# cvxgrp/cvxpygen

Hardware: AMD Instinct MI355X
Metric: QP instances solved/sec (batched MPC QP, OSQP; inputs resident in HBM) (higher is better)
Workload: dtype f64

## Files before the change

cvxpygen_amd/codegen.py:

```python

from __future__ import annotations

import os
import shutil
import subprocess
from typing import List, Optional, Sequence

import numpy as np

from .solve_program import GEN_EXTRA_SLOTS, LANES, RaggedProgram, execution_steps, padded_offsets_fit

CSRC = os.path.join(os.path.dirname(os.path.abspath(__file__)), 'csrc')


class ProgramTooLarge(Exception):
    """the family's solve program cannot be made LDS-resident: no specialised library for it"""


def emit_program_header(rp: RaggedProgram, name: str = 'family', plan=None, depth: int = 2, cross: int = 4,
                        pad_offsets: bool = False, group_offsets: int = 4, batch: int = 1, early: int = 4) -> str:
    out: List[str] = []
    w = out.append
    w(f'// Generated by cvxpygen_amd.codegen for problem family "{name}" -- do not edit.')
    w(f'// solve program: {rp.n_phases} phases, {rp.n_chunks} chunks, {int(rp.ctab[:, 0].sum())} steps, '
# ... 419 lines not shown
            r_of, s_of, nr = list(range(len(idx))), {}, len(idx)
        for k, t in enumerate(idx):
            reg_of[t] = r_of[k]
        for c, sft in s_of.items():
            shift_of[c] = sft
        n_regs_w[v] = nr
    n_regs = max(n_regs_w + [1])
    n_off = max(1, (max([int(sl[t]) + 1 for t in range(T)] + [0]) + 1) // 2)
    n_row = max(1, (max([int(cl[c]) + 1 for c in range(rp.n_chunks)] + [0]) + 1) // 2)
    w(f'// Generated by cvxpygen_amd.codegen for problem family "{name}" -- do not edit.')
    w(f'// team executor ({W} wavefronts per instance): {rp.n_phases} phases, {rp.n_chunks} chunks, {T} steps, {rp.nnz - 1} coefficients;')
    w(f'// steps per wavefront {[int((sw == v).sum()) for v in range(W)]}, coefficient registers {n_regs_w}')
    w('#pragma once')
    w(f'#define {G}_W {W}')
    w(f'#define {G}_NCHUNKS {rp.n_chunks}')
    w(f'#define {G}_NNZ {rp.nnz}')
    w(f'#define {G}_FINGERPRINT {rp.fingerprint()}u')
    w(f'#define {G}_NSTEPS {T}')
    w(f'#define {G}_NSLOTS {rp.n_slots}')
    w(f'#define {G}_NREGS {n_regs}')
    w(f'#define {G}_NOFF {n_off}')
    w(f'#define {G}_NROW {n_row}')
    for k_, v_ in (dims or {}).items():
        w(f'#define {G}_{k_} {int(v_)}')
    w(f'#define {G}_STEPS {{' + ', '.join(f'{{{e}, {cnt}, {reg_of[t]}, {shift_of[c]}}}' for t, (_, c, e, cnt) in enumerate(steps)) + '}')
    w(f'#define {G}_STEP_WAVE {{' + ', '.join(str(int(v)) for v in sw) + '}')
    w(f'#define {G}_STEP_LOCAL {{' + ', '.join(str(int(v)) for v in sl) + '}')
    w(f'#define {G}_CHUNK_SHIFT {{' + ', '.join(str(shift_of[c]) for c in range(rp.n_chunks)) + '}')
    w(f'#define {G}_CHUNK_WAVE {{' + ', '.join(str(int(v)) for v in cw) + '}')
    w(f'#define {G}_CHUNK_LOCAL {{' + ', '.join(str(int(v)) for v in cl) + '}')
    w('namespace cpg {')
    if coef == 'reg':
        w(f'CPG_DEV void {func}(const double (&cf)[{G}_NREGS], const unsigned (&of)[{G}_NOFF], const unsigned (&rw)[{G}_NROW],')
        w('                              CPG_LDS double *w, int wave) {')
    else:
        w(f'CPG_DEV void {func}(const double *vals, const unsigned *off, const unsigned *row, CPG_LDS double *w, int lane, int wave) {{')
    w('    const CPG_LDS char *wb = (const CPG_LDS char *)w;')
    by_phase = {}
    for t, (pi_, c, e, cnt) in enumerate(steps):
        by_phase.setdefault(pi_, []).append((t, c))
    plist = sorted(by_phase)

    def off_expr(t):
        j = int(sl[t])
        base = f'of[{j // 2}]' if coef == 'reg' else f'q{int(sw[t])}_{j // 2}'
        return f'({base} >> 16)' if j & 1 else f'({base} & 0xFFFFu)'

    def row_expr(c):
        j = int(cl[c])
        base = f'rw[{j // 2}]' if coef == 'reg' else f'p{int(cw[c])}_{j // 2}'
        return f'({base} >> 16)' if j & 1 else f'({base} & 0xFFFFu)'
    w('    switch (wave) {')
    for v in range(W):
        w(f'    case {v}: {{')
        mine = [t for t in range(T) if sw[t] == v]
        if coef != 'reg' and mine:
            for k in range((len(mine) + 1) // 2):
                w(f'        const unsigned q{v}_{k} = cpgw::gld(off, {(v * n_off + k) * 64}u + (unsigned)lane);')
            nch_v = len({steps[t][1] for t in mine})
            for k in range((nch_v + 1) // 2):
                w(f'        const unsigned p{v}_{k} = cpgw::gld(row, {(v * n_row + k) * 64}u + (unsigned)lane);')
            for t in mine:
                w(f'        const double c{t} = cpgw::gld(vals, {int(steps[t][2])}u + (unsigned)lane);')
        for pi_ in plist:
            lst = [(t, c) for (t, c) in by_phase[pi_] if sw[t] == v]
            if lst:
                chunks = sorted({c for _, c in lst})
                w(f'        // phase {pi_}')
                for c in chunks:
                    w(f'        const unsigned r{c} = {row_expr(c)};')
                for t, c in lst:
                    w(f'        const double x{t} = *(const CPG_LDS double *)(wb + {off_expr(t)});')
                for c in chunks:
                    if int(rp.ctab[c, 3]) & 2:
                        w(f'        const double o{c} = w[r{c} & CPG_GEN_SLOT_MASK];')
                w('        cpgw::sched_fence();')
                nsteps_c = {}
                for _, c in lst:
                    nsteps_c[c] = nsteps_c.get(c, 0) + 1
                kacc = {c: (1 if (n_ < 6 or not TEAM_SPLIT_SUMS) else (2 if n_ < 12 else 4)) for c, n_ in nsteps_c.items()}
                seen, first = {}, {}
                for t, c in lst:
                    cx = f'cf[{reg_of[t]}]' if coef == 'reg' else f'c{t}'
                    j = seen.get(c, 0) % kacc[c]
                    seen[c] = seen.get(c, 0) + 1
                    nm = f'a{c}' if kacc[c] == 1 else f'a{c}_{j}'
                    if (c, j) not in first:
                        first[(c, j)] = True
                        w(f'        double {nm} = {cx} * x{t};' if coef == 'reg' else f'        double {nm} = fma({cx}, x{t}, 0.0);')
                    else:
                        w(f'        {nm} = fma({cx}, x{t}, {nm});')
                for c in chunks:
                    if kacc[c] == 2:
                        w(f'        const double a{c} = a{c}_0 + a{c}_1;')
                    elif kacc[c] == 4:
                        w(f'        const double a{c} = (a{c}_0 + a{c}_1) + (a{c}_2 + a{c}_3);')
                for c in chunks:
                    lg, kind = int(rp.ctab[c, 1]), int(rp.ctab[c, 3])
                    assert not kind & 4, 'a team executor has no deferred phases (resident_plan: intra phases instead)'
                    red = f'cpgw::seg_sum_first_lit<{lg}>(a{c}, {_mask_literals(stage_masks(rp, c, shift_of[c]))})' if kind & 1 else f'cpgw::group_sum_first<{lg}>(a{c})'
                    acc = f'o{c} + ' if kind & 2 else ''
                    w(f'        w[r{c} & CPG_GEN_SLOT_MASK] = {acc}{red};')
            if sync:
                w('        cpgw::block_sync();')
        w('    } break;')
    w('    default: {')
    if sync:
        for _ in plist:
            w('        cpgw::block_sync();')
    w('    } break;')
    w('    }')
    w('}')
    w('}  // namespace cpg')
    return '\n'.join(out) + '\n' + epilogue


def factor_fingerprint(fac) -> int:
    h = 0x811C9DC5
    ct = np.asarray(fac.ctab, dtype=np.int32).reshape(-1, 4)[:, [0, 1, 3]]
    for arr in (np.ascontiguousarray(ct), np.ascontiguousarray(fac.tlen, dtype=np.uint32)):
        for b in arr.tobytes():
            h = ((h ^ b) * 0x01000193) & 0xFFFFFFFF
    return h


FACTOR_LOOKAHEAD = int(os.environ.get('CPG_FACTOR_LOOKAHEAD', 3))


def emit_factor_program(fac, nnzL: int, N: int, prefix: str = 'GENI', lookahead: Optional[int] = None,
                        preloaded: bool = False, func: str = 'numeric_ldl_gen', zero: Optional[int] = None, body: bool = True,
                        one: Optional[int] = None, inverse_from: Optional[int] = None) -> str:
    G = f'CPG_{prefix}_FAC'
    P = FACTOR_LOOKAHEAD if lookahead is None else lookahead
    ct = np.asarray(fac.ctab, dtype=np.int64).reshape(-1, 4)
    nch = ct.shape[0]
    first = np.concatenate([[0], np.cumsum(ct[:, 0])])
    out = []
    w = out.append
    w(f'#define {G}_NCHUNKS {nch}')
    w(f'#define {G}_NSTEPS {int(first[-1])}')
    w(f'#define {G}_FINGERPRINT {factor_fingerprint(fac)}u')
    w(f'#define {G}_ZERO {nnzL + N if zero is None else int(zero)}')
    if one is not None:
        w(f'#define {G}_ONE {int(one)}')
    inv0 = nch if inverse_from is None else int(inverse_from)
    w(f'#define {G}_CHUNKS {{' + ', '.join(f'{{{int(L)}, {int(last)}, {int(lg)}}}' for L, last, _, lg in ct) + '}')
    if not body:
        return '\n'.join(out) + '\n'
    w(f'#define {G}_GENERATED 1')
    w('namespace cpg {')
    if preloaded:
        w(f'CPG_DEV void {func}(const unsigned long long *tri, const unsigned *dk, double *w, int lane) {{')
    else:
        w(f'CPG_DEV void {func}(const unsigned long long *tri, const unsigned *dk, const double *kct, const double *rinv,')
        w('                             double *w, int lane) {')
    w('    const unsigned ln = (unsigned)cpgw::opaque(lane);     // (table addresses computed here, not hoisted out of the instance loop)')

    def req_dk(c):
        if c < nch:
            w(f'    const unsigned d{c} = cpgw::gld(dk, {c * 64}u + ln);')

    def req_rest(c):
        if c < nch:
            if not preloaded and c < inv0:
                w(f'    const double kc{c} = cpgw::gld(kct, {c * 64}u + ln);')
                w(f'    const double kr{c} = cpgw::gld(rinv, (d{c} >> 16) ? (d{c} >> 16) - 1u : 0u);')
            for s_ in range(int(ct[c, 0])):
                w(f'    const unsigned long long e{int(first[c]) + s_} = cpgw::gld(tri, {(int(first[c]) + s_) * 64}u + ln);')
    for c in range(2 * P):
        req_dk(c)
    for c in range(P):
        req_rest(c)
    for c in range(nch):
        L, last, _, lg = (int(v) for v in ct[c])
        last &= 1
        w(f'    // chunk {c}: {L} step(s), groups of {1 << lg}' + (', level end' if last else ''))
        req_dk(c + 2 * P)
        req_rest(c + P)
        if preloaded and L == 0:
            if last:
                w('    cpgw::lds_order();')
            continue
        w(f'    double a{c} = 0.0;')
        for s_ in range(L):
            e = f'e{int(first[c]) + s_}'
            w(f'    a{c} = fma(w[(unsigned){e} & 0xFFFFu] * w[(unsigned)({e} >> 32)], w[((unsigned){e} >> 16)], a{c});')
        w(f'    a{c} = cpgw::group_sum_first<{lg}>(a{c});')
        w(f'    if ((d{c} & 0xFFFFu) != 0xFFFFu) {{')
        if c >= inv0 and not preloaded:
            w(f'        w[d{c} & 0xFFFFu] = -a{c};')
        elif preloaded:
            w(f'        const double v = w[d{c} & 0xFFFFu] - a{c};')
            w(f'        w[d{c} & 0xFFFFu] = (d{c} >> 16) ? 1.0 / v : v;')
        else:
            w(f'        const double v = (kc{c} - ((d{c} >> 16) ? kr{c} : 0.0)) - a{c};')
            w(f'        w[d{c} & 0xFFFFu] = (d{c} & 0xFFFFu) >= {nnzL}u ? 1.0 / v : v;')
        w('    }')
        if last:
            w('    cpgw::lds_order();')
    w('    cpgw::lds_order();')
    w('}')
    w('}  // namespace cpg')
    return '\n'.join(out) + '\n'


def write_instance_header(rp: RaggedProgram, path: str, name: str = 'family', **opts) -> str:
    text = emit_instance_program(rp, name, **opts)
    if os.path.exists(path) and open(path).read() == text:
        return path
    with open(path, 'w') as f:
        f.write(text)
    return path


def write_program_header(rp: RaggedProgram, path: str, name: str = 'family', plan=None, depth: int = 2, **gen_opts) -> str:
    text = emit_program_header(rp, name, plan, depth, **gen_opts)
    if os.path.exists(path) and open(path).read() == text:
        return path
    with open(path, 'w') as f:
        f.write(text)
    return path


def coefficient_dictionary(rp: RaggedProgram) -> np.ndarray:
    return np.unique(np.ascontiguousarray(rp.vals, dtype=np.float64).view(np.uint64))


def family_library_defs(plan, out_dir: str, name: str = 'family', g_list: Sequence[int] = (1, 2),
                        waves: Optional[dict] = None, extra_flags: Sequence[str] = (), depth: int = 2,
                        compress: Optional[bool] = None, **gen_opts):
    out_dir = os.path.abspath(out_dir)
    os.makedirs(out_dir, exist_ok=True)
    rp = plan.kkt_ragged
    d = plan.desc
    N = d.n_var + d.m
    if 'pad_offsets' not in gen_opts:
        gen_opts = dict(gen_opts, pad_offsets=(compress is not True) and padded_offsets_fit(rp, N))
    pad_offsets = bool(gen_opts['pad_offsets'])
    hdr = write_program_header(rp, os.path.join(out_dir, f'cpg_program_{name}.h'), name, plan=plan, depth=depth, **gen_opts)
    nsx, nsz = -(-d.n_var // 64), -(-d.m // 64)
    nv = max(-(-plan.n_vary_x // 64), -(-plan.n_vary_z // 64), 1)
    nv = nv if nv <= 1 else max(nsx, nsz)
    waves = waves or {1: 8, 2: 4}
    ylist = ' '.join(f'Y({nsx}, {nsz}, {nv}, {g}, {waves[g]})' for g in g_list)
    nnzp = rp.nnz + 64
    n_off = 64 * ((int(rp.ctab[:, 0].sum()) + 3) & ~3) if pad_offsets else nnzp
    plain = 8 * N + 8 * (nnzp + (n_off + 3) // 4 + 16 * ((rp.n_chunks + 3) & ~3))
    n_dict = len(coefficient_dictionary(rp))
    packed = 8 * N + 8 * (n_dict + (nnzp + 1) // 2 + 16 * ((rp.n_chunks + 3) & ~3))
    per_wave = 8 * (rp.n_slots + GEN_EXTRA_SLOTS)
    can_compress = n_dict <= 8192 and per_wave <= 65536 and not pad_offsets
    if compress is None:
        compress = can_compress and (160 * 1024 - plain) // per_wave < 8 and \
            (160 * 1024 - packed) // per_wave > max(0, (160 * 1024 - plain) // per_wave)
    compress = bool(compress and can_compress)
    fixed = packed if compress else plain
    wfit = (160 * 1024 - fixed) // per_wave
    if wfit < 1:
        raise ProgramTooLarge(f'solve program ({fixed} B) + one work vector do not fit the 160 KiB LDS; '
                              'use the table-driven library (program streamed from L2)')
    if 1 in g_list and waves[1] == 8 and wfit >= 10:
        ylist += f' Y({nsx}, {nsz}, {nv}, 1, 12)'
    defs = [f'-DCPG_GEN_HEADER="{hdr}"', '-DCPG_KERNELS(X)=', f'-DCPG_KERNELS_LDS(Y)={ylist}',
            f'-DCPG_KERNELS_REFACTOR(Z)=Z({nsx}, {nsz})']
    if compress:
        defs += ['-DCPG_GEN_COMPRESSED=1', f'-DCPG_GEN_NDICT={n_dict}']
    import scipy.sparse as _sps
    if int(np.diff(_sps.csr_matrix(d.A).indptr).max(initial=0)) > 32:
        defs.append('-DCPG_REFACTOR_ROW_COPY=1')
    if not any('CPG_REFACTOR_WAVES_PER_SIMD' in f for f in extra_flags):
        if nsx + nsz <= 14:
            defs.append('-DCPG_REFACTOR_WAVES_PER_SIMD=4')
        elif nsx + nsz >= 20:
            defs.append('-DCPG_REFACTOR_WAVES_PER_SIMD=2')
            if os.environ.get('CPG_REFACTOR_CR_LDS', '1') != '0':
                defs.append('-DCPG_REFACTOR_CR_LDS=1')
    ih = instance_header(plan, out_dir, name)
    if ih is not None:
        defs.append(f'-DCPG_GENI_HEADER="{ih}"')
    qh = squad_header(plan, out_dir, name)
    if qh is not None:
        defs.append(f'-DCPG_GENQ_HEADER="{qh}"')
    th = team_header(plan, out_dir, name) if team_waves(d) else None
    rh = resident_header(plan, out_dir, name) if th is None else None
    if th is None and rh is None and TEAM_WAVES == -1 and matrix_parameters(d):
        th = team_header(plan, out_dir, name, W=TEAM_AUTO_WAVES)
    if th is not None:
        defs.append(f'-DCPG_GENT_HEADER="{th}"')
    elif rh is not None:
        defs.append(f'-DCPG_GENR_HEADER="{rh}"')
    else:
        sh = stream_header(plan, out_dir, name)
        if sh is not None:
            defs.append(f'-DCPG_GENS_HEADER="{sh}"')
    return hdr, defs


GENS_MAX_STEPS = int(os.environ.get('CPG_GENS_MAX_STEPS', 1200))
GENS_LOOKAHEAD = int(os.environ.get('CPG_GENS_LOOKAHEAD', 16))


def stream_header(plan, out_dir: str, name: str = 'family') -> Optional[str]:
    from . import refactor_plan as _rp
    from .solve_program import execution_steps
    d = plan.desc
    if not matrix_parameters(d) or os.environ.get('CPG_GENS', '0') != '1':
        return None
    rpl = _rp.build_refactor_plan(d.P, d.A, plan.osqp)
    T = len(execution_steps(rpl.sol))
    if T == 0 or T > GENS_MAX_STEPS or any(int(k_) & ~1 for k_ in rpl.sol.ctab[:, 3]):
        return None
    text = emit_instance_program(rpl.sol, name, lookahead=GENS_LOOKAHEAD, prefix='GENS', func='run_program_gens', coef='mem')
    path = os.path.join(os.path.abspath(out_dir), f'cpg_stream_{name}.h')
    if not (os.path.exists(path) and open(path).read() == text):
        with open(path, 'w') as f:
            f.write(text)
    return path


GENI_MAX_REGS = int(os.environ.get('CPG_GENI_MAX_REGS', 64))
GENI_MAX_STEPS = int(os.environ.get('CPG_GENI_MAX_STEPS', 240))
LDS_BYTES = 160 * 1024


SHARED_REG_LDS_REGS = 20


def shared_register_lds_bytes(n: int, m: int, n_steps: int, n_chunks: int, n_slots: int, n_regs: int, waves: int = 8) -> int:
    tab = 2 * (256 * ((n_steps + 3) // 4) + 256 * ((n_chunks + 3) // 4))
    return 8 * (n + m) + tab + 8 * 64 * min(SHARED_REG_LDS_REGS, n_regs) + waves * 8 * (n_slots + GEN_EXTRA_SLOTS)


def instance_program_fits(rpl) -> bool:
    mg = getattr(rpl, 'merged', None)
    rp = mg.sol if mg is not None else rpl.sol
    N = rpl.n + rpl.m
    steps = execution_steps(rp)
    if len(steps) > GENI_MAX_STEPS or rp.n_slots + GEN_EXTRA_SLOTS > 0x1FFF or not np.array_equal(rp.final_pos, np.arange(N)):
        return False
    if pack_step_registers(rp, steps)[2] > GENI_MAX_REGS:
        return False
    tab = 2 * (256 * ((len(steps) + 3) // 4) + 256 * ((rp.n_chunks + 3) // 4))
    per_wave = rp.n_slots + GEN_EXTRA_SLOTS + N + (N & 1)
    fac = rpl.nnzL + N
    if mg is not None:
        fac = mg.fac_len
        if fac >= 0xFFFF:
            return False
    per_wave = max(per_wave, fac + (fac & 1))
    return tab + 8 * 8 * per_wave <= LDS_BYTES


def instance_header(plan, out_dir: str, name: str = 'family') -> Optional[str]:
    from . import refactor_plan as _rp
    d = plan.desc
    o = plan.osqp_shared or plan.osqp
    Ps, As = o.pruned(d.P, d.A)
    rpl = _rp.shared_mode_plan(Ps, As, o)
    if not instance_program_fits(rpl):
        return None
    dims = dict(N=d.n_var, M=d.m, NEQ=d.n_eq)
    mg = rpl.merged
    if mg is None:
        prog, fac = rpl.sol, emit_factor_program(rpl.fac, rpl.nnzL, rpl.n + rpl.m)
    else:
        import types
        dims['NNZX'] = mg.nnzX
        prog = mg.sol
        fac = emit_factor_program(types.SimpleNamespace(ctab=mg.f_ctab, tlen=mg.f_len), rpl.nnzL, rpl.n + rpl.m,
                                  zero=mg.fac_len - 1, one=mg.one_pos, inverse_from=mg.base.fac.n_chunks)
    return write_instance_header(prog, os.path.join(os.path.abspath(out_dir), f'cpg_instance_{name}.h'), name,
                                 row_programs=shared_row_programs(Ps, As), dims=dims, epilogue=fac)


RESIDENT_MAX_REGS = int(os.environ.get('CPG_RESIDENT_MAX_REGS', 160))
RESIDENT_MAX_STEPS = int(os.environ.get('CPG_RESIDENT_MAX_STEPS', 320))
RESIDENT_ACC_BASE = int(os.environ.get('CPG_RESIDENT_ACC_BASE', 32))
RESIDENT_GATHER_BATCH = int(os.environ.get('CPG_RESIDENT_GATHER_BATCH', 12))
RESIDENT_ACC_PAIRS = int(os.environ.get('CPG_RESIDENT_ACC_PAIRS', 112))


def resident_compiler_flags(defs: Sequence[str]) -> List[str]:
    return []


def matrix_parameters(desc) -> bool:
    import scipy.sparse as _sps
    NP = desc.NP
    return any(_sps.csr_matrix(desc.maps[k])[:, :NP].nnz > 0 for k in ('P', 'A'))


def resident_program_fits(rpl, np_var: Optional[int] = None) -> bool:
    rp = rpl.sol
    b = rpl.base
    N = b.n + b.m
    steps = execution_steps(rp)
    if len(steps) > RESIDENT_MAX_STEPS or not np.array_equal(rp.final_pos, np.arange(N)):
        return False
    if pack_step_registers(rp, steps)[2] > RESIDENT_MAX_REGS:
        return False
    tab = 2 * (256 * ((len(steps) + 3) // 4) + 256 * ((rp.n_chunks + 3) // 4))
    np_var = b.nnzP + b.nnzA + N if np_var is None else np_var
    slice_ = max(rpl.fac_len, rpl.w_slots + N, b.nnzA + b.nnzP + max(np_var, N + max(b.n, b.m)))
    slice_ += slice_ & 1
    return 8 * slice_ <= 0xFFFF and tab + 2 * 8 * slice_ <= LDS_BYTES


def resident_four_waves(rpl, np_var: int) -> bool:
    if os.environ.get('CPG_RES_FOUR_WAVES', '0') != '1':
        return False
    b = rpl.base
    N = b.n + b.m
    slice_ = max(rpl.fac_len, rpl.w_slots + b.m, max(b.nnzA + b.nnzP, max(np_var, N + max(b.n, b.m))))
    slice_ += slice_ & 1
    return 4 * 8 * slice_ <= LDS_BYTES


def resident_header(plan, out_dir: str, name: str = 'family') -> Optional[str]:
    from . import resident_plan as _rs
    d = plan.desc
    if not matrix_parameters(d):
        return None
    rpl = _rs.build_resident_plan(d.P, d.A, plan.osqp)
    if not resident_program_fits(rpl, d.NP):
        return None
    b = rpl.base
    dims = dict(N=b.n, M=b.m, NEQ=d.n_eq, NNZA=b.nnzA, NNZP=b.nnzP, NNZL=b.nnzL, NNZX=rpl.nnzX)
    from .solve_program import execution_steps
    rows = ''
    progs = (('GENRA', 'run_rows_a', rpl.rows_A), ('GENRP', 'run_rows_p', rpl.rows_P), ('GENRT', 'run_rows_t', rpl.rows_At))
    if all(len(execution_steps(pr)) > 0 and not any(int(k_) & ~1 for k_ in pr.ctab[:, 3]) for _, _, pr in progs):
        for pre, fn, pr in progs:
            rows += emit_instance_program(pr, name, lookahead=len(execution_steps(pr)) + 4, prefix=pre, func=fn, coef='mem',
                                          lds_typed=True).replace('#pragma once\n', '')
    import types
    if rpl.fac_len < 0xFFFF:
        rows += emit_factor_program(types.SimpleNamespace(ctab=rpl.f_ctab, tlen=rpl.f_len), b.nnzL, b.n + b.m, prefix='GENR',
                                    preloaded=True, func='resident_factor_gen', zero=rpl.fac_len - 1)
    return write_instance_header(rpl.sol, os.path.join(os.path.abspath(out_dir), f'cpg_resident_{name}.h'), name,
                                 prefix='GENR', func='run_program_res', prefetch_next=True, dims=dims,
                                 gather_batch=RESIDENT_GATHER_BATCH, lds_typed=True, epilogue=rows,
                                 tables_global=resident_four_waves(rpl, d.NP))


TEAM_WAVES = int(os.environ.get('CPG_TEAM_WAVES', -1))
TEAM_AUTO_WAVES = 4
TEAM_MAX_GROUP_ROWS = int(os.environ.get('CPG_TEAM_MAX_GROUP_ROWS', 600))
TEAM_SPLIT_SUMS = os.environ.get('CPG_TEAM_SPLIT_SUMS', '0') == '1'
FAC_CODE_BYTES_PER_STEP = 130
INSTRUCTION_CACHE_BYTES = 64 * 1024
TEAM_FAC_GENERATED_MAX = int(os.environ.get('CPG_TEAM_FAC_GENERATED_MAX', (INSTRUCTION_CACHE_BYTES * 5 // 4) // FAC_CODE_BYTES_PER_STEP))


def team_waves(desc=None) -> int:
    return TEAM_WAVES if TEAM_WAVES in (1, 2, 4, 8) else 0


def build_team_plan(desc, osqp, W: Optional[int] = None, max_group_rows: Optional[int] = None, groups=None):
    from . import resident_plan as _rs
    W = team_waves(desc) if W is None else W
    saved = _rs.MAX_GROUP_ROWS
    _rs.MAX_GROUP_ROWS = TEAM_MAX_GROUP_ROWS if max_group_rows is None else int(max_group_rows)
    try:
        return _rs.build_resident_plan(desc.P, desc.A, osqp, team=W, inplace_x=False, groups=groups)
    finally:
        _rs.MAX_GROUP_ROWS = saved


def team_slice_doubles(rpl, np_var: int) -> int:
    b = rpl.base
    N = b.n + b.m
    slice_ = max(rpl.fac_len, rpl.w_slots, b.nnzA + b.nnzP, np_var, N + max(b.n, b.m))
    slice_ += slice_ & 1
    return slice_ + 16 * max(1, int(rpl.team)) + 8


def team_program_fits(rpl, W: int, np_var: Optional[int] = None) -> bool:
    rp = rpl.sol
    b = rpl.base
    N = b.n + b.m
    if rpl.team != W or not np.array_equal(rp.final_pos, np.arange(N)) or rp.n_slots + GEN_EXTRA_SLOTS > 0x1FFF:
        return False
    if any(int(k_) & 4 for k_ in rp.ctab[:, 3]):
# ... 626 lines not shown
```

cvxpygen_amd/csrc/cpg_hip.cpp:

```cpp
#include "../../include/cpg_hip.h"

#include <math.h>
#include <stdio.h>
#include <stdlib.h>
#include <string.h>

#include <algorithm>
#include <string>
#include <type_traits>
#include <vector>

#include "cpg_osqp_kernel.h"
#include "cpg_osqp_refactor.h"
#include "cpg_osqp_resident.h"
#include "cpg_osqp_team.h"
#include "cpg_osqp_squad.h"
#include "cpg_clarabel_kernel.h"

#include <hip/hip_runtime.h>
typedef hipStream_t rt_stream_t;
typedef hipEvent_t rt_event_t;
#define RT_CHECK(expr)                                                                         \
    do {                                                                                       \
        hipError_t e_ = (expr);                                                                \
// ... 281 lines not shown
    const int wave_global = (int)(blockIdx.x * (blockDim.x >> 6) + (threadIdx.x >> 6));
    cpg::osqp_refactor_body<NSX, NSZ, true>(F, R, S, Bt, cpg_lds, wave_global);
}
#ifdef CPG_GENI_NNZX
template <int NSX, int NSZ, int NV>
__global__ void __launch_bounds__(512, 2)
osqp_shared_reg_kernel(cpg::DevFamily F, cpg::DevUpdate U, cpg::DevSettings S, cpg::DevBatch Bt, cpg::DevShRegs RG) {
    extern __shared__ __attribute__((aligned(16))) double cpg_lds[];
    const int wave_global = (int)(blockIdx.x * (blockDim.x >> 6) + (threadIdx.x >> 6));
    cpg::osqp_shared_body<NSX, NSZ, NV, 1, false, cpg::SharedRegExec>(F, U, S, Bt, cpg_lds, wave_global, RG);
}
#endif
#endif
#ifdef CPG_GENR_HEADER
template <int NSX, int NSZ>
__global__ void __launch_bounds__(256)
osqp_resident_kernel(cpg::DevFamily F, cpg::DevRefactor R, cpg::DevResident Rs, cpg::DevSettings S, cpg::DevBatch Bt) {
    extern __shared__ __attribute__((aligned(16))) double cpg_lds[];
    const int wave_global = (int)(blockIdx.x * (blockDim.x >> 6) + (threadIdx.x >> 6));
    cpg::osqp_resident_body<NSX, NSZ>(F, R, Rs, S, Bt, cpg_lds, wave_global);
}
#endif
#ifdef CPG_GENT_HEADER
__global__ void __launch_bounds__(CPG_GENT_W * 64)
osqp_team_kernel(cpg::DevFamily F, cpg::DevRefactor R, cpg::DevResident Rs, cpg::DevSettings S, cpg::DevBatch Bt) {
    extern __shared__ __attribute__((aligned(16))) double cpg_lds[];
    constexpr int NX = (CPG_GENT_N + CPG_GENT_W * 64 - 1) / (CPG_GENT_W * 64), NZ = (CPG_GENT_M + CPG_GENT_W * 64 - 1) / (CPG_GENT_W * 64);
    cpg::osqp_team_body<(NX > 0 ? NX : 1), (NZ > 0 ? NZ : 1)>(F, R, Rs, S, Bt, cpg_lds, (int)blockIdx.x);
}
#endif
#ifdef CPG_GENQ_HEADER
template <int NSX, int NSZ, int NV>
__global__ void __launch_bounds__(CPG_GENQ_W * 64, 2)
osqp_squad_kernel(cpg::DevFamily F, cpg::DevUpdate U, cpg::DevSettings S, cpg::DevBatch Bt) {
    extern __shared__ __attribute__((aligned(16))) double cpg_lds[];
    cpg::osqp_squad_body<NSX, NSZ, NV>(F, U, S, Bt, cpg_lds);
}
#endif
template <int NSX, int NSZ>
__global__ void __launch_bounds__(512, CPG_GRADIENT_WAVES_PER_SIMD)
osqp_gradient_kernel(cpg::DevFamily F, cpg::DevRefactor R, cpg::DevGradient Gd, cpg::DevGradBatch Bt) {
    extern __shared__ __attribute__((aligned(16))) double cpg_lds[];
    const int wave_global = (int)(blockIdx.x * (blockDim.x >> 6) + (threadIdx.x >> 6));
    cpg::osqp_gradient_body<NSX, NSZ>(F, R, Gd, Bt, cpg_lds, wave_global);
}

#ifndef CPG_KERNELS_REFACTOR
#define CPG_KERNELS_REFACTOR(Z) Z(1, 1) Z(4, 4) Z(8, 8) Z(16, 16)
#endif
template <typename Launch>
static bool slot_class(cpg_handle_t h, int &rc, Launch &&launch) {
    const int nsx = (h->F.n + 63) / 64, nsz = (h->F.m + 63) / 64;
#define Z(a, b)                                                                                   \
    if (nsx <= a && nsz <= b) {                                                                   \
        rc = launch(std::integral_constant<int, a>(), std::integral_constant<int, b>());          \
        return true;                                                                              \
    }
    CPG_KERNELS_REFACTOR(Z)
#undef Z
    return false;
}
template <typename Launch>
static int with_slot_class(cpg_handle_t h, Launch &&launch) {
    int rc;
    if (slot_class(h, rc, launch)) return rc;
    set_error("problem family larger than the largest compiled slot class");
    return CPG_E_UNSUPPORTED;
}
static int launch_gradient(cpg_handle_t h, const cpg::DevGradBatch &Bt, int blocks, int waves, size_t lds) {
    return with_slot_class(h, [&](auto NSX, auto NSZ) {
        return launch_kernel(osqp_gradient_kernel<NSX, NSZ>, blocks, waves * 64, lds, h->stream, h->F, h->R, h->Gd, Bt); });
}
static int launch_refactor(cpg_handle_t h, rt_stream_t stream, const cpg::DevSettings &S, const cpg::DevBatch &Bt, int blocks, int waves, size_t lds) {
    return with_slot_class(h, [&](auto NSX, auto NSZ) {
        return launch_kernel(h->R.shared_mats ? osqp_refactor_kernel<NSX, NSZ, true> : osqp_refactor_kernel<NSX, NSZ, false>,
                             blocks, waves * 64, lds, stream, h->F, h->R, S, Bt); });
}

#ifndef CPG_CONIC_WAVES_PER_SIMD
#define CPG_CONIC_WAVES_PER_SIMD 4
#endif
template <bool TABLES_IN_LDS, bool SPECIALISED, bool NONSYM>
__global__ void __launch_bounds__(512, CPG_CONIC_WAVES_PER_SIMD)
clarabel_kernel(cpg::DevConic C, cpg::DevConicSettings S, cpg::DevBatch Bt) {
    extern __shared__ __attribute__((aligned(16))) double cpg_lds[];
    const int wave_global = (int)(blockIdx.x * (blockDim.x >> 6) + (threadIdx.x >> 6));
    cpg::clarabel_body<TABLES_IN_LDS, SPECIALISED, NONSYM>(C, S, Bt, cpg_lds, wave_global);
}
static int launch_conic(cpg_handle_t h, const cpg::DevBatch &Bt, int blocks, int waves, size_t lds, bool tables_in_lds) {
    const bool extended = h->C.n_ns > 0 || h->C.n_psd > 0;
#ifdef CPG_GENC_HEADER
    if (h->conic_specialised && tables_in_lds)
        return launch_kernel(extended ? clarabel_kernel<true, true, true> : clarabel_kernel<true, true, false>,
                             blocks, waves * 64, lds, h->stream, h->C, h->CS, Bt);
#endif
    auto kern = extended ? (tables_in_lds ? clarabel_kernel<true, false, true> : clarabel_kernel<false, false, true>)
                         : (tables_in_lds ? clarabel_kernel<true, false, false> : clarabel_kernel<false, false, false>);
    return launch_kernel(kern, blocks, waves * 64, lds, h->stream, h->C, h->CS, Bt);
}


#ifndef CPG_KERNELS
#define CPG_KERNELS(X)                                                                              \
    X(1, 1, 1, 1) X(1, 1, 1, 2) X(4, 4, 1, 1) X(4, 4, 1, 2) X(4, 4, 4, 1) X(8, 8, 1, 1) X(8, 8, 1, 2)   \
    X(8, 8, 8, 1) X(16, 16, 16, 1)
#endif
#ifndef CPG_KERNELS_LDS
#define CPG_KERNELS_LDS(Y)                                                                          \
    Y(1, 1, 1, 1, 8) Y(1, 1, 1, 1, 16) Y(1, 1, 1, 2, 8) Y(4, 4, 1, 1, 8) Y(4, 4, 1, 1, 16) Y(4, 4, 1, 2, 8)    \
    Y(4, 4, 4, 1, 8) Y(8, 8, 1, 1, 8) Y(8, 8, 1, 1, 12) Y(8, 8, 1, 2, 4) Y(8, 8, 1, 2, 8) Y(8, 8, 8, 1, 8) \
    Y(16, 16, 16, 1, 8)
#endif

static int vary_slots(cpg_handle_t h) {
    const int nvx = (h->n_vary_x + 63) / 64, nvz = (h->n_vary_z + 63) / 64;
    return nvx > nvz ? nvx : nvz;
}
static int launch(cpg_handle_t h, const cpg::DevBatch &Bt, int blocks, int waves, int G, size_t lds, bool in_lds) {
    const int nsx = (h->F.n + 63) / 64, nsz = (h->F.m + 63) / 64, nv = vary_slots(h);
    if (!in_lds) {
#define X(a, b, v, g)                                                                             \
        if (nsx <= a && nsz <= b && (nv <= v || (v >= a && v >= b)) && G == g && waves <= 4)      \
            return launch_kernel(osqp_shared_kernel<a, b, v, g, false, 4>, blocks, waves * 64, lds, h->stream, h->F, h->U, h->S, Bt);
        CPG_KERNELS(X)
#undef X
    } else {
#define Y(a, b, v, g, wm)                                                                         \
        if (nsx <= a && nsz <= b && (nv <= v || (v >= a && v >= b)) && G == g && waves <= wm)     \
            return launch_kernel(osqp_shared_kernel<a, b, v, g, true, wm>, blocks, waves * 64, lds, h->stream, h->F, h->U, h->S, Bt);
        CPG_KERNELS_LDS(Y)
#undef Y
    }
    set_error("no compiled kernel for this family size / launch geometry");
    return CPG_E_UNSUPPORTED;
}

#ifdef CPG_GENQ_HEADER
static int launch_squad(cpg_handle_t h, const cpg::DevBatch &Bt, int blocks, size_t lds) {
    const int nsx = (h->F.n + 63) / 64, nsz = (h->F.m + 63) / 64, nv = vary_slots(h);
#define Y(a, b, v, g, wm)                                                                         \
    if (nsx == a && nsz == b && (nv <= v || (v >= a && v >= b)) && g == 1)                        \
        return launch_kernel(osqp_squad_kernel<a, b, v>, blocks, CPG_GENQ_W * 64, lds, h->stream, h->F, h->U, h->S, Bt);
    CPG_KERNELS_LDS(Y)
#undef Y
    set_error("no compiled squad kernel for this family size");
    return CPG_E_UNSUPPORTED;
}
#endif

#if defined(CPG_GENI_HEADER) && defined(CPG_GENI_NNZX)
static int shared_reg_waves(cpg_handle_t h) { return h->waves_per_block > 0 && h->waves_per_block < 8 ? h->waves_per_block : 8; }
static size_t shared_reg_lds(cpg_handle_t h, int W) {
    const size_t tab = (size_t)(((CPG_GENI_NSTEPS + 3) / 4) * 256 + ((CPG_GENI_NCHUNKS + 3) / 4) * 256) * sizeof(unsigned short);
    return (size_t)(h->F.n + h->F.m) * sizeof(double) + tab + (size_t)cpg::SharedRegExec::nlds * 64 * sizeof(double) +
           (size_t)W * (CPG_GENI_NSLOTS + CPG_GEN_EXTRA_SLOTS) * sizeof(double);
}
static bool shared_reg_usable(cpg_handle_t h) {
    return !h->refactor_mode && !h->conic && h->sreg_ok && h->sreg_rho == h->F.rho && h->sreg_sigma == h->F.sigma &&
           h->inst_per_wave == 1 && shared_reg_lds(h, shared_reg_waves(h)) <= h->lds_limit;
}
static int launch_shared_reg(cpg_handle_t h, const cpg::DevBatch &Bt, int blocks, int waves, size_t lds) {
    const int nsx = (h->F.n + 63) / 64, nsz = (h->F.m + 63) / 64, nv = vary_slots(h);
#define Y(a, b, v, g, wm)                                                                         \
    if (nsx <= a && nsz <= b && (nv <= v || (v >= a && v >= b)) && g == 1)                        \
        return launch_kernel(osqp_shared_reg_kernel<a, b, v>, blocks, waves * 64, lds, h->stream, h->F, h->U, h->S, Bt, h->SRg);
    CPG_KERNELS_LDS(Y)
#undef Y
    set_error("no compiled register-executor kernel for this family size");
    return CPG_E_UNSUPPORTED;
}
#else
static bool shared_reg_usable(cpg_handle_t) { return false; }
#endif

static cpg::DevBatch make_batch(int64_t B, const double *d_theta, const double *d_state_in, double *d_state_out, double *d_prim,
                                double *d_dual, double *d_obj, int32_t *d_iter, int32_t *d_status, double *d_pri, double *d_dua) {
    cpg::DevBatch Bt;
    Bt.scratch = nullptr; Bt.state_in = d_state_in; Bt.state_out = d_state_out;
    Bt.B = B; Bt.theta = d_theta; Bt.prim = d_prim; Bt.dual = d_dual; Bt.obj = d_obj; Bt.pri_res = d_pri;
    Bt.dua_res = d_dua; Bt.iter = d_iter; Bt.status = d_status; Bt.counter = nullptr;
    Bt.ho_list = nullptr; Bt.ho_count = nullptr; Bt.ho_state = nullptr; Bt.list = nullptr; Bt.list_count = nullptr; Bt.resume = 0;
    return Bt;
}

static int launch_per_instance(cpg_handle_t h, rt_stream_t stream, const cpg::DevSettings &S, cpg::DevBatch &Bt) {
    int rc;
    auto scratch = [&](int blocks, int waves, size_t doubles) {
        const int r = ensure(h->scratch, (size_t)blocks * waves * doubles * sizeof(double));
        Bt.scratch = (double *)h->scratch.p;
        return r;
    };
#ifdef CPG_GENT_HEADER
    if (h->Rs.ok == 2 && !h->R.shared_mats && h->program_in_lds != 0 && h->program_in_lds != 2) {
        const size_t lds = ((size_t)CPG_TEAM_SLICE_OFF + (size_t)h->Rs.slice_doubles) * sizeof(double);
        if (lds <= h->lds_limit) {
            long long per_cu = (long long)(h->lds_limit / lds);
            if (per_cu * CPG_GENT_W > 16) per_cu = 16 / CPG_GENT_W;
            if (CPG_GENT_W <= 4 && per_cu * CPG_GENT_W > 4) per_cu = 4 / CPG_GENT_W;
            if (h->blocks_per_cu > 0 && per_cu > h->blocks_per_cu) per_cu = h->blocks_per_cu;
            const int blocks = std::max(1, grid_blocks(h, Bt.B, 1, per_cu));
            if ((rc = scratch(blocks, 1, h->Rs.buf_doubles))) return rc;
            return launch_kernel(osqp_team_kernel, blocks, CPG_GENT_W * 64, lds, stream, h->F, h->R, h->Rs, S, Bt);
        }
    }
#endif
#ifdef CPG_GENR_HEADER
    if (h->Rs.ok && !h->R.shared_mats && h->program_in_lds != 0 && h->program_in_lds != 2) {
#ifdef CPG_GENR_TABLES_GLOBAL
        const size_t tab = 0;
#else
        const size_t tab = (size_t)(((CPG_GENR_NSTEPS + 3) / 4) * 256 + ((CPG_GENR_NCHUNKS + 3) / 4) * 256) * sizeof(unsigned short);
#endif
        const size_t slice = (size_t)h->Rs.slice_doubles * sizeof(double);
        int NW = h->waves_per_block > 0 ? h->waves_per_block : 4;
        if (NW > 4) NW = 4;
        while (NW > 1 && tab + (size_t)NW * slice > h->lds_limit) NW--;
        const size_t lds = tab + (size_t)NW * slice;
        if (lds <= h->lds_limit) {
            const int blocks = grid_blocks(h, Bt.B, NW, 1);
            if ((rc = scratch(blocks, NW, h->Rs.buf_doubles))) return rc;
            if (slot_class(h, rc, [&](auto NSX, auto NSZ) {
                    return launch_kernel(osqp_resident_kernel<NSX, NSZ>, blocks, NW * 64, lds, stream, h->F, h->R, h->Rs, S, Bt); }))
                return rc;
        }
    }
#endif
#ifdef CPG_GENI_HEADER
    if (h->R.gi_ok && h->program_in_lds != 0 && h->program_in_lds != 2) {
        const int W = 8;
        const size_t tab = (size_t)(((CPG_GENI_NSTEPS + 3) / 4) * 256 + ((CPG_GENI_NCHUNKS + 3) / 4) * 256) * sizeof(unsigned short);
        const size_t nq = (size_t)(h->F.n + h->F.m);
        size_t per_wave = (size_t)(CPG_GENI_NSLOTS + CPG_GEN_EXTRA_SLOTS) + nq + (nq & 1);
#ifdef CPG_GENI_FAC_NSTEPS
        const size_t fac = (size_t)CPG_GENI_FAC_ZERO + 1;
#else
        const size_t fac = (size_t)h->R.nnzL + nq;
#endif
        if (per_wave < fac) per_wave = fac + (fac & 1);
        const size_t lds = tab + (size_t)W * per_wave * sizeof(double);
        if (lds <= h->lds_limit) {
            const int blocks = grid_blocks(h, Bt.B, W, 1);
            if ((rc = scratch(blocks, W, h->R.buf_doubles))) return rc;
            if (slot_class(h, rc, [&](auto NSX, auto NSZ) {
                    return launch_kernel(osqp_instance_kernel<NSX, NSZ>, blocks, W * 64, lds, stream, h->F, h->R, S, Bt); }))
                return rc;
        }
    }
#endif
#ifdef CPG_REFACTOR_CR_LDS
    if (!h->R.shared_mats && h->program_in_lds != 0) {
        const int W8 = 8;
        const size_t tab = (((size_t)h->R.sol_nnz + 1) / 2) * sizeof(double);
        const size_t lds8 = tab + (size_t)W8 * h->R.sol_slots * sizeof(double);
        if (lds8 <= h->lds_limit) {
            const int blocks = grid_blocks(h, Bt.B, W8, 1);
            if ((rc = scratch(blocks, W8, h->R.buf_doubles))) return rc;
            if (slot_class(h, rc, [&](auto NSX, auto NSZ) {
                    return launch_kernel(osqp_refactor_crlds_kernel<NSX, NSZ>, blocks, W8 * 64, lds8, stream, h->F, h->R, S, Bt); }))
                return rc;
        }
    }
#endif
    const int W = 4;
#ifdef CPG_GENS_HEADER
    if (!h->R.shared_mats && !h->R.gs_ok) {
        set_error("this library's per-instance substitution program was generated for a different family"); return CPG_E_BADARG; }
    const size_t lds = (size_t)W * (size_t)(h->R.shared_mats ? h->R.sol_slots : h->R.sol_slots + CPG_GEN_EXTRA_SLOTS) * sizeof(double);
#else
    const size_t lds = (size_t)W * h->R.sol_slots * sizeof(double);
#endif
    if (lds > h->lds_limit) { set_error("work vectors do not fit the LDS"); return CPG_E_UNSUPPORTED; }
    int per_cu = h->blocks_per_cu > 0 ? h->blocks_per_cu : CPG_REFACTOR_WAVES_PER_SIMD;
    if (per_cu > CPG_REFACTOR_WAVES_PER_SIMD) per_cu = CPG_REFACTOR_WAVES_PER_SIMD;
    if ((long long)per_cu * (long long)lds > (long long)h->lds_limit) per_cu = (int)(h->lds_limit / lds);
    const int blocks = grid_blocks(h, Bt.B, W, per_cu);
    if ((rc = scratch(blocks, W, h->R.buf_doubles))) return rc;
    return launch_refactor(h, stream, S, Bt, blocks, W, lds);
}

static int begin_solve(cpg_handle_t h) {
    RT_CHECK(hipMemsetAsync(h->d_counter, 0, 4 * sizeof(unsigned), h->stream));
    RT_CHECK(hipEventRecord(h->ev0, h->stream));
    return CPG_OK;
}
static int end_solve(cpg_handle_t h) {
    RT_CHECK(hipEventRecord(h->ev1, h->stream));
    return CPG_OK;
}

static int solve_conic(cpg_handle_t h, const cpg::DevBatch &Bt) {
    const size_t per_wave = (size_t)h->C.lds_doubles * sizeof(double);
    int W = h->waves_per_block > 0 ? (h->waves_per_block > 8 ? 8 : h->waves_per_block) : 8;
    const size_t tab = (size_t)h->C.tab_doubles * sizeof(double);
    const bool tables_in_lds = h->program_in_lds != 0 && tab + per_wave <= h->lds_limit;
    const size_t fixed = tables_in_lds ? tab : 0;
    while (W > 1 && fixed + (size_t)W * per_wave > h->lds_limit) W--;
    if (h->waves_per_block <= 0) {
        int best = W, best_res = 0;
        for (int w2 = W; w2 >= 4; w2--) {
            int pc = (int)(h->lds_limit / (fixed + (size_t)w2 * per_wave));
            if (h->blocks_per_cu > 0 && pc > h->blocks_per_cu) pc = h->blocks_per_cu;
            int res = pc * w2; if (res > 4 * CPG_CONIC_WAVES_PER_SIMD) res = 4 * CPG_CONIC_WAVES_PER_SIMD;
            if (res > best_res) { best_res = res; best = w2; }
        }
        W = best;
    }
    const size_t lds = fixed + (size_t)W * per_wave + (fixed + (size_t)W * per_wave + 128 <= h->lds_limit ? 128 : 0);
// ... 709 lines not shown
    UP(int, prim_idx, f->n_prim); UP(int, dual_idx, f->n_dual);
#undef UP
    TRY(upload_csr(h, own, f->map_P, &C.map_P)); TRY(upload_csr(h, own, f->map_A, &C.map_A));
    TRY(upload_csr(h, own, f->map_q, &C.map_q)); TRY(upload_csr(h, own, f->map_b, &C.map_b));
    TRY(upload_csr(h, own, f->map_d, &C.map_d));
    C.gc_ok = 0; C.sv_pad = 0; C.w_extra = 0; C.gc_ncols = 0; C.gc_nrows = 0; C.gc_cols = nullptr; C.gc_rows = nullptr;
    C.gf_ok = 0;
#ifdef CPG_GENC_FACTOR_HEADER
    C.gf_ok = (conic_factor_words_hash(f) == CPG_GENC_FAC_HASH && !(getenv("CPG_CONIC_FACTOR") && atoi(getenv("CPG_CONIC_FACTOR")) == 0)) ? 1 : 0;
#endif
#ifdef CPG_GENC_HEADER
    if (f->sol_chunks == CPG_GENC_NCHUNKS && f->sol_nnz == CPG_GENC_NNZ && f->sol_slots == CPG_GENC_NSLOTS &&
        program_fingerprint(f->sol_ctab, f->sol_desc, f->sol_cols, f->sol_chunks, f->sol_nnz) == CPG_GENC_FINGERPRINT &&
        !(getenv("CPG_CONIC_GENERATED") && atoi(getenv("CPG_CONIC_GENERATED")) == 0)) {
        static const int steps[][4] = CPG_GENC_STEPS;
        std::vector<unsigned short> gcols, grows;
        if (generated_tables(f->sol_ctab, f->sol_desc, f->sol_cols, f->sol_chunks, f->sol_nnz, f->sol_slots, steps, CPG_GENC_NSTEPS, gcols, grows)) {
            TRY(upload<unsigned short>(h, own, gcols.data(), gcols.size(), &C.gc_cols));
            TRY(upload<unsigned short>(h, own, grows.data(), grows.size(), &C.gc_rows));
            C.gc_ncols = (int)gcols.size(); C.gc_nrows = (int)grows.size();
            C.gc_ok = 1; C.sv_pad = 64; C.w_extra = CPG_GEN_EXTRA_SLOTS;
            cpg::DevConic Cs = C;
            Cs.n_pfull = f->Prp[n]; Cs.fac_triples = f->fac_triples;
            cpg::DevConic Ck = Cs;
            { cpg::DevConic &Cref = Ck; CPG_GENC_SPECIALISE(Cref) }
            h->conic_specialised = conic_dims_equal(Cs, Ck) && !(getenv("CPG_CONIC_SPECIALISED") && atoi(getenv("CPG_CONIC_SPECIALISED")) == 0);
#ifdef CPG_GENC_ROWS
            if (h->conic_specialised && conic_row_words_hash(f) != CPG_GENC_ROWS_HASH) h->conic_specialised = false;
#endif
        }
    }
#endif
    {
        C.fac_triples = f->fac_triples; C.n_pfull = f->Prp[n];
        auto dbl = [](size_t count, size_t elem) { return (count * elem + 7) / 8; };
        size_t t = 0;
        t += 2 * dbl((size_t)f->n_soc, 4) + dbl((size_t)m, 4);
        bool row_words = false;
#ifdef CPG_GENC_ROWS
        row_words = h->conic_specialised;
        if (row_words) t += dbl((size_t)CPG_GENC_ROWS_WORDS, sizeof(cpg::genc_row_word));
#endif
        if (!row_words) {
            t += dbl((size_t)n + 1, 4) + dbl((size_t)f->nnzA, 4) + dbl((size_t)m + 1, 4) + 2 * dbl((size_t)f->nnzA, 4);
            t += dbl((size_t)n + 1, 4) + dbl((size_t)f->nnzP, 4) + dbl((size_t)n + 1, 4) + 2 * dbl((size_t)C.n_pfull, 4);
        }
        t += dbl((size_t)f->nnzL, 4) + 2 * dbl((size_t)f->nnzL + N, 4);
        t += dbl((size_t)f->fac_chunks * 4, 4) + 2 * dbl((size_t)f->fac_chunks * 64, 4) + 3 * dbl((size_t)f->fac_triples, 4);
#ifdef CPG_GENC_HEADER
        t += dbl((size_t)C.gc_ncols, 2) + dbl((size_t)C.gc_nrows, 2);
#else
        t += dbl((size_t)f->sol_chunks * 4, 4) + dbl((size_t)f->sol_chunks * 64, 4) + dbl((size_t)f->sol_nnz, 2);
#endif
        t += 2 * dbl((size_t)f->sol_nnz, 4) + dbl((size_t)N, 2);
        C.tab_doubles = (int)t;
    }
    {
        const long long d = (long long)f->nnzP + f->nnzA + 7LL * n + 14LL * m + 6LL * N + f->nnzL + f->sol_nnz + C.sv_pad + f->sol_slots + C.w_extra + C.psd_doubles;
        C.lds_doubles = (int)((d + 1) & ~1LL);
        if ((size_t)C.lds_doubles * 8 > h->lds_limit) {
            set_error("conic family too large: the interior-point state of one instance does not fit the LDS");
            cpg_hip_destroy(h); return CPG_E_UNSUPPORTED; }
    }
    { void *p = nullptr; TRY(rt_malloc(&p, 64)); h->d_counter = (unsigned *)p; }
    TRY(rt_sync(h));
#undef TRY
    h->have_update = true;
    cpg_hip_set_default_settings(h);
    *out = h;
    return CPG_OK;
}

struct cpg_pipe_s;
static void free_pipe(cpg_pipe_s *p);
static void free_list(std::vector<void *> &v) { for (void *p : v) rt_free(p); v.clear(); }

int cpg_hip_destroy(cpg_handle_t h) {
    if (!h) return CPG_OK;
    rt_set_device(h->device);
    rt_sync(h);
    free_list(h->owned); free_list(h->update_owned); free_list(h->refactor_owned); free_list(h->sreg_owned); free_list(h->resident_owned); free_list(h->gradient_owned);
    free_buf(h->g_theta); free_buf(h->g_x); free_buf(h->g_y); free_buf(h->g_dprim); free_buf(h->g_dtheta);
    if (h->d_counter) rt_free(h->d_counter);
    free_buf(h->scratch);
    free_buf(h->s_theta); h->s_out.free(); free_buf(h->s_state_in); free_buf(h->s_state_out);
    free_buf(h->ho_state); free_buf(h->ho_list);
    free_pipe(h->pipe); h->pipe = nullptr;
    if (h->have_events) { hipEventDestroy(h->ev0); hipEventDestroy(h->ev1); hipEventDestroy(h->ev_mid); }
    if (h->stream) hipStreamDestroy(h->stream);
    delete h;
    return CPG_OK;
}

int cpg_hip_set_update(cpg_handle_t h, const cpg_osqp_update_t *u) {
    if (!h || !u) { set_error("null argument"); return CPG_E_BADARG; }
    if (h && h->conic) { set_error("not available for a conic (interior-point) handle"); return CPG_E_BADARG; }
    if (u->map_q.nnz && u->map_q.rows != h->F.n) { set_error("map_q rows != n"); return CPG_E_BADARG; }
    if (u->map_u.nnz && u->map_u.rows != h->F.m) { set_error("map_u rows != m"); return CPG_E_BADARG; }
    {
        const cpg_csr_t *mp[2] = {&u->map_q, &u->map_u};
        const int lim[2] = {h->n_vary_x, h->n_vary_z};
        for (int k = 0; k < 2; k++)
            if (mp[k]->nnz > 0 && mp[k]->ptr[mp[k]->rows] != mp[k]->ptr[lim[k] < mp[k]->rows ? lim[k] : mp[k]->rows]) {
                set_error("update map touches entries outside the parameter-dependent prefix"); return CPG_E_BADARG; }
    }
    int rc = rt_set_device(h->device);
    if (rc) return rc;
    if ((rc = rt_sync(h))) return rc;
    free_list(h->update_owned);
    cpg::DevUpdate &U = h->U;
    U.np_var = u->np_var; U.d_base = u->d_base;
    if ((rc = upload<double>(h, h->update_owned, u->q_base, h->F.n, &U.q_base))) return rc;
    if ((rc = upload<double>(h, h->update_owned, u->u_base, h->F.m, &U.u_base))) return rc;
    if ((rc = upload_csr(h, h->update_owned, u->map_q, &U.map_q))) return rc;
    if ((rc = upload_csr(h, h->update_owned, u->map_u, &U.map_u))) return rc;
    if ((rc = upload_csr(h, h->update_owned, u->map_d, &U.map_d))) return rc;
    if ((rc = rt_sync(h))) return rc;
    h->have_update = true;
    h->refactor_mode = false;
    return CPG_OK;
}

static bool kkt_constants(cpg_handle_t h, const cpg_osqp_refactor_t *r, std::vector<double> &fkc, std::vector<int> &fkrow) {
    const size_t m = h->F.m, nd = (size_t)r->nnzL + h->F.n + m;
    fkc.assign(nd, 0.0); fkrow.assign(nd, -1);
    for (size_t d = 0; d < nd; d++) {
        const int kind = r->ksrc_kind[d], idx = r->ksrc_idx[d];
        const bool piv = d >= (size_t)r->nnzL;
        if (kind == CPG_K_P) { if (idx < 0 || idx >= r->nnzP) return false; fkc[d] = r->Ps[idx] + (piv ? h->F.sigma : 0.0); }
        else if (kind == CPG_K_A) { if (idx < 0 || idx >= r->nnzA) return false; fkc[d] = r->As[idx]; }
        else if (kind == CPG_K_SIGMA) fkc[d] = h->F.sigma;
        else if (kind == CPG_K_RHO) { if (idx < 0 || (size_t)idx >= m) return false; fkrow[d] = idx; }
        else if (kind != CPG_K_NONE) return false;
    }
    return true;
}

#ifdef CPG_GENI_HEADER
struct InstanceTables {
    int nnzX;
    int sol_chunks, sol_nnz, sol_slots;
    const int32_t *sol_ctab; const uint32_t *sol_desc; const uint16_t *sol_cols; const int32_t *sol_kind, *sol_idx;
    int fac_chunks, fac_triples;
    const int32_t *fac_ctab; const uint32_t *fac_task, *fac_len, *fac_a, *fac_b, *fac_k;
};

static int set_instance_executor(cpg_handle_t h, const cpg_osqp_refactor_t *r, const InstanceTables &g,
                                 const std::vector<double> &fkc, const std::vector<int> &fkrow) {
    std::vector<void *> &own = h->refactor_owned;
    cpg::DevRefactor &R = h->R;
    const size_t n = h->F.n, m = h->F.m, N = n + m;
    int rc = CPG_OK;
    R.gi_ok = 0;
    std::vector<unsigned short> gcols, grows, glcol;
    std::vector<unsigned> gsrc, gdk;
    std::vector<unsigned long long> gtri;
    std::vector<double> gkc;
#ifdef CPG_GENI_N
    const bool geni_dims = h->F.n == CPG_GENI_N && h->F.m == CPG_GENI_M && h->F.n_eq == CPG_GENI_NEQ;
#else
    const bool geni_dims = true;
#endif
#ifdef CPG_GENI_NNZX
    const bool merged_lib = true;
#else
    const bool merged_lib = false;
#endif
    if (!(geni_dims && (g.nnzX > 0) == merged_lib && g.sol_chunks == CPG_GENI_NCHUNKS && g.sol_nnz == CPG_GENI_NNZ && g.sol_slots == CPG_GENI_NSLOTS))
        return CPG_OK;
    const size_t nd = (size_t)r->nnzL + N, nx = (size_t)g.nnzX;
    const unsigned hsh = program_fingerprint(g.sol_ctab, g.sol_desc, g.sol_cols, g.sol_chunks, g.sol_nnz);
    static const int steps[][4] = CPG_GENI_STEPS;
    static const int chunk_shift[] = CPG_GENI_CHUNK_SHIFT;
    bool ok = hsh == CPG_GENI_FINGERPRINT;
    {
        const int nn[3] = {CPG_GENI_AROWS_N, CPG_GENI_PROWS_N, CPG_GENI_ATROWS_N};
        for (int k = 0; ok && k < 3; k++) {
            if ((int)h->rows_hdr[k].size() != 4 * nn[k]) ok = false;
            for (int c2 = 0; ok && c2 < nn[k]; c2++)
                if (h->rows_hdr[k][4 * c2] != cpg::GeniRows::len(k, c2) || h->rows_hdr[k][4 * c2 + 3] != cpg::GeniRows::off(k, c2)) ok = false;
        }
    }
    if (ok) ok = generated_tables(g.sol_ctab, g.sol_desc, g.sol_cols, g.sol_chunks, g.sol_nnz, g.sol_slots, steps, CPG_GENI_NSTEPS, gcols, grows, chunk_shift);
    if (ok) {
        gsrc.assign((size_t)CPG_GENI_NREGS * 64, 0u);
        glcol.assign((size_t)CPG_GENI_NREGS * 64, (unsigned short)0);
        std::vector<char> taken((size_t)CPG_GENI_NREGS * 64, 0);
        for (int t = 0; ok && t < CPG_GENI_NSTEPS; t++) {
            const int e = steps[t][0], cnt = steps[t][1], reg = steps[t][2], sh = steps[t][3];
            if (reg < 0 || reg >= CPG_GENI_NREGS) { ok = false; break; }
            for (int l = 0; l < cnt; l++) {
                int kind = g.sol_kind[e + l], idx = g.sol_idx[e + l];
                if (kind == 4) {
                    if (idx < 0 || (size_t)idx >= nx) { ok = false; break; }
                    kind = 3; idx += (int)N;
                }
                if (kind < 0 || kind > 3 || idx < 0 || idx >= (1 << 28)) { ok = false; break; }
                const size_t at = (size_t)reg * 64 + (size_t)(l + sh);
                if (taken[at]) { ok = false; break; }
                taken[at] = 1;
                gsrc[at] = ((unsigned)kind << 28) | (unsigned)idx;
                if (kind == 2) {
                    if (idx >= r->nnzL || r->Lcol[idx] < 0 || r->Lcol[idx] > 0xFFFF) { ok = false; break; }
                    glcol[at] = (unsigned short)r->Lcol[idx];
                }
            }
        }
    }
#ifdef CPG_GENI_FAC_NSTEPS
    if (ok) {
        static const int fch[][3] = CPG_GENI_FAC_CHUNKS;
        const size_t fac_end = nx ? nd + nx + 2 : nd + 1;
        const size_t one = nd + nx;
        unsigned hsh2 = 0x811C9DC5u;
        auto mix = [&](unsigned v) { for (int k = 0; k < 4; k++) { hsh2 = (hsh2 ^ ((v >> (8 * k)) & 0xFFu)) * 0x01000193u; } };
        ok = g.fac_chunks == CPG_GENI_FAC_NCHUNKS && fac_end - 1 == (size_t)CPG_GENI_FAC_ZERO && fac_end <= 0xFFFFu;
#ifdef CPG_GENI_FAC_ONE
        ok = ok && one == (size_t)CPG_GENI_FAC_ONE;
#endif
        for (int c = 0; ok && c < g.fac_chunks; c++) { mix((unsigned)g.fac_ctab[4 * c]); mix((unsigned)g.fac_ctab[4 * c + 1]); mix((unsigned)g.fac_ctab[4 * c + 3]); }
        for (size_t e = 0; ok && e < (size_t)g.fac_chunks * 64; e++) mix(g.fac_len[e]);
        ok = ok && hsh2 == CPG_GENI_FAC_FINGERPRINT;
        if (ok) {
            const unsigned long long Z = (unsigned long long)(fac_end - 1);
            gtri.assign((size_t)CPG_GENI_FAC_NSTEPS * 64, Z | (Z << 16) | (Z << 32));
            gdk.assign((size_t)g.fac_chunks * 64, 0xFFFFu);
            gkc.assign((size_t)g.fac_chunks * 64, 0.0);
            size_t step = 0;
            for (int c = 0; ok && c < g.fac_chunks; c++) {
                const int L = g.fac_ctab[4 * c];
                size_t base = (size_t)g.fac_ctab[4 * c + 2];
                if (L != fch[c][0]) { ok = false; break; }
                for (int s = 0; ok && s < L; s++, step++) {
                    int cnt = 0;
                    for (int l = 0; l < 64; l++) {
                        const unsigned ln = g.fac_len[(size_t)c * 64 + l];
                        if ((int)(ln & 0xFFFFu) <= s) continue;
                        const size_t e = base + (size_t)l;
                        if (l != cnt || e >= (size_t)g.fac_triples) { ok = false; break; }
                        cnt++;
                        if ((int)(ln >> 16) > s) {
                            const unsigned a = g.fac_a[e], b = g.fac_b[e], k = nx ? g.fac_k[e] : (unsigned)r->nnzL + g.fac_k[e];
                            if (a >= (unsigned)r->nnzL || !(b < (unsigned)r->nnzL || (nx && b >= nd && b <= one)) ||
                                k < (unsigned)r->nnzL || k >= nd) { ok = false; break; }
                            gtri[step * 64 + (size_t)l] = (unsigned long long)a | ((unsigned long long)b << 16) | ((unsigned long long)k << 32);
                        }
                    }
                    base += (size_t)cnt;
                }
                for (int l = 0; ok && l < 64; l++) {
                    const unsigned t0 = g.fac_task[(size_t)c * 64 + l];
                    if (t0 == 0xFFFFFFFFu) continue;
                    const unsigned t = nx ? (t0 & 0x7FFFFFFFu) : t0;
                    if (t >= nd + nx) { ok = false; break; }
                    const int kr = t < nd ? fkrow[t] : -1;
                    gdk[(size_t)c * 64 + l] = t | ((unsigned)(kr + 1) << 16);
                    gkc[(size_t)c * 64 + l] = t < nd ? fkc[t] : 0.0;
                }
            }
            if (ok && step != (size_t)CPG_GENI_FAC_NSTEPS) ok = false;
        }
        if (ok) {
            if ((rc = upload<unsigned long long>(h, own, gtri.data(), gtri.size(), &R.gf_tri))) return rc;
            if ((rc = upload<unsigned>(h, own, gdk.data(), gdk.size(), &R.gf_dk))) return rc;
            if ((rc = upload<double>(h, own, gkc.data(), gkc.size(), &R.gf_kc))) return rc;
        }
    }
#else
    ok = ok && !nx;
#endif
    if (ok) {
        if ((rc = upload<unsigned short>(h, own, glcol.data(), glcol.size(), &R.gi_lcol))) return rc;
        if ((rc = upload<unsigned short>(h, own, gcols.data(), gcols.size(), &R.gi_cols))) return rc;
        if ((rc = upload<unsigned short>(h, own, grows.data(), grows.size(), &R.gi_rows))) return rc;
        if ((rc = upload<unsigned>(h, own, gsrc.data(), gsrc.size(), &R.gi_src))) return rc;
    }
    if ((rc = rt_sync(h))) return rc;
    R.gi_ok = ok ? 1 : 0;
    return CPG_OK;
}
#endif

int cpg_hip_set_refactor(cpg_handle_t h, const cpg_osqp_refactor_t *r) {
    if (h && h->conic) { set_error("not available for a conic (interior-point) handle"); return CPG_E_BADARG; }
    if (!h || !r) { set_error("null argument"); return CPG_E_BADARG; }
    int rc = rt_set_device(h->device);
    if (rc) return rc;
    if ((rc = rt_sync(h))) return rc;
    free_list(h->refactor_owned);
    free_list(h->resident_owned); h->Rs = cpg::DevResident{};
    std::vector<void *> &own = h->refactor_owned;
    cpg::DevRefactor &R = h->R;
    const size_t n = h->F.n, m = h->F.m, N = n + m;
    R.nnzP = r->nnzP; R.nnzA = r->nnzA; R.nnzL = r->nnzL; R.n_eq = h->F.n_eq; R.np_var = r->np_var;
    R.scaling_iters = r->scaling_iters; R.d_base = r->d_base;
    R.fac_chunks = r->fac_chunks; R.sol_nnz = r->sol_nnz; R.sol_slots = r->sol_slots;
#define UP(T, field, count) if ((rc = upload<T>(h, own, (const T *)r->field, (size_t)(count), (const T **)&R.field))) return rc
    UP(int, Ap, n + 1); UP(int, Ai, r->nnzA); UP(int, Arp, m + 1); UP(int, Aent, r->nnzA); UP(int, Acol, r->nnzA);
    UP(int, Pp, n + 1); UP(int, Pi, r->nnzP); UP(int, Prp, n + 1);
    { const int npf = r->Prp[n]; UP(int, Pent, npf); UP(int, Pcol, npf); }
    UP(int, Lcol, r->nnzL); UP(int, ksrc_kind, r->nnzL + N); UP(int, ksrc_idx, r->nnzL + N);
    UP(int, fac_ctab, (size_t)r->fac_chunks * 4); UP(unsigned, fac_task, (size_t)r->fac_chunks * 64);
    UP(unsigned, fac_len, (size_t)r->fac_chunks * 64);
    UP(unsigned, fac_a, r->fac_triples); UP(unsigned, fac_b, r->fac_triples); UP(unsigned, fac_k, r->fac_triples);
    StreamTables stt;
    std::vector<int> kind2, idx2;
    R.gs_cols = nullptr; R.gs_rows = nullptr; R.gs_kind = nullptr; R.gs_idx = nullptr; R.gs_ok = 0; R.gs_nnz = 0;
#ifdef CPG_GENS_HEADER
    std::vector<unsigned short> gscols, gsrows;
    std::vector<int> gskind, gsidx;
    if (!r->shared_mats && r->sol_chunks == CPG_GENS_NCHUNKS && r->sol_nnz == CPG_GENS_NNZ && r->sol_slots == CPG_GENS_NSLOTS &&
        program_fingerprint(r->sol_ctab, r->sol_desc, r->sol_cols, r->sol_chunks, r->sol_nnz) == CPG_GENS_FINGERPRINT) {
        static const int gsteps[][4] = CPG_GENS_STEPS;
        if (generated_tables(r->sol_ctab, r->sol_desc, r->sol_cols, r->sol_chunks, r->sol_nnz, r->sol_slots, gsteps, CPG_GENS_NSTEPS, gscols, gsrows)) {
            gskind.assign((size_t)r->sol_nnz + 64, 0); gsidx.assign((size_t)r->sol_nnz + 64, 0);
            for (int e = 0; e < r->sol_nnz; e++) { gskind[e] = r->sol_kind[e]; gsidx[e] = r->sol_idx[e]; }
            R.gs_nnz = r->sol_nnz + 64;
            if ((rc = upload<unsigned short>(h, own, gscols.data(), gscols.size(), &R.gs_cols))) return rc;
            if ((rc = upload<unsigned short>(h, own, gsrows.data(), gsrows.size(), &R.gs_rows))) return rc;
            if ((rc = upload<int>(h, own, gskind.data(), gskind.size(), &R.gs_kind))) return rc;
            if ((rc = upload<int>(h, own, gsidx.data(), gsidx.size(), &R.gs_idx))) return rc;
            R.gs_ok = 1;
        }
    }
#endif
    {
        if ((rc = build_stream_tables(r->sol_ctab, r->sol_desc, r->sol_cols, r->sol_chunks, r->sol_slots, stt))) return rc;
        kind2.resize(stt.src.size()); idx2.resize(stt.src.size());
        for (size_t e = 0; e < stt.src.size(); e++) {
            kind2[e] = stt.src[e] >= 0 ? r->sol_kind[stt.src[e]] : 0;
            idx2[e] = stt.src[e] >= 0 ? r->sol_idx[stt.src[e]] : 0;
        }
        R.sol_pairs = stt.n_pairs;
        R.sol_nnz = (int)stt.cr.size();
        if ((rc = upload<unsigned>(h, own, stt.st.data(), stt.st.size(), &R.sol_stab))) return rc;
        if ((rc = upload<unsigned>(h, own, stt.cr.data(), stt.cr.size(), &R.sol_cr))) return rc;
        if ((rc = upload<int>(h, own, kind2.data(), kind2.size(), &R.sol_kind))) return rc;
        if ((rc = upload<int>(h, own, idx2.data(), idx2.size(), &R.sol_idx))) return rc;
    }
    UP(unsigned short, sol_fpos, N);
    UP(double, P_base, r->nnzP); UP(double, A_base, r->nnzA); UP(double, q_base, n); UP(double, u_base, m);
    UP(double, q_setup, n);
#undef UP
    if ((rc = upload_csr(h, own, r->map_P, &R.map_P))) return rc;
    if ((rc = upload_csr(h, own, r->map_A, &R.map_A))) return rc;
    if ((rc = upload_csr(h, own, r->map_q, &R.map_q))) return rc;
    if ((rc = upload_csr(h, own, r->map_u, &R.map_u))) return rc;
    if ((rc = upload_csr(h, own, r->map_d, &R.map_d))) return rc;
    R.buf_doubles = (long long)(r->nnzP + 2 * r->nnzA + 3 * n + 4 * m + r->nnzL + 2 * N + std::max(R.sol_nnz, R.gs_nnz) + 64);
    R.shared_mats = r->shared_mats ? 1 : 0; R.cs = 1.0;
    R.Ps = R.As = R.Ars = R.Ds = R.Dinvs = R.Es = R.Einvs = nullptr;
    std::vector<double> ars, dinv, einv;
    if (r->shared_mats) {
        if (!r->Ps || !r->As || !r->D || !r->E || !(r->c > 0.0)) { set_error("shared-matrix mode needs Ps, As, D, E, c"); return CPG_E_BADARG; }
        ars.resize((size_t)r->nnzA); dinv.resize(n); einv.resize(m);
        for (int k = 0; k < r->nnzA; k++) ars[k] = r->As[r->Aent[k]];
        for (size_t i = 0; i < n; i++) dinv[i] = 1.0 / r->D[i];
        for (size_t i = 0; i < m; i++) einv[i] = 1.0 / r->E[i];
        R.cs = r->c;
        if ((rc = upload<double>(h, own, r->Ps, (size_t)r->nnzP, &R.Ps))) return rc;
        if ((rc = upload<double>(h, own, r->As, (size_t)r->nnzA, &R.As))) return rc;
        if ((rc = upload<double>(h, own, ars.data(), ars.size(), &R.Ars))) return rc;
        if ((rc = upload<double>(h, own, r->D, n, &R.Ds))) return rc;
        if ((rc = upload<double>(h, own, dinv.data(), n, &R.Dinvs))) return rc;
        if ((rc = upload<double>(h, own, r->E, m, &R.Es))) return rc;
        if ((rc = upload<double>(h, own, einv.data(), m, &R.Einvs))) return rc;
    }
    R.gf_tri = nullptr; R.gf_dk = nullptr; R.gf_kc = nullptr;
    R.gi_ok = 0; R.gi_cols = R.gi_rows = nullptr; R.gi_src = nullptr; R.gi_lcol = nullptr; R.fac_kc = nullptr; R.fac_krow = nullptr; R.fac_kc_cl = nullptr; R.fac_krow_cl = nullptr; R.fac_kind_cl = nullptr; R.fac_idx_cl = nullptr;
    std::vector<double> fkc, fkc_cl;
    std::vector<int> fkrow, fkrow_cl;

    if (r->shared_mats) {
        if (!kkt_constants(h, r, fkc, fkrow)) { set_error("cpg_hip_set_refactor: KKT source table out of range"); return CPG_E_BADARG; }
        const size_t nd = (size_t)r->nnzL + N;
        fkc_cl.assign((size_t)r->fac_chunks * 64, 0.0); fkrow_cl.assign((size_t)r->fac_chunks * 64, -1);
        for (size_t e = 0; e < fkc_cl.size(); e++) {
            const unsigned t = r->fac_task[e];
            if (t == 0xFFFFFFFFu) continue;
            if (t >= nd) { set_error("cpg_hip_set_refactor: factorisation task out of range"); return CPG_E_BADARG; }
            fkc_cl[e] = fkc[t]; fkrow_cl[e] = fkrow[t];
        }
        if ((rc = upload<double>(h, own, fkc.data(), fkc.size(), &R.fac_kc))) return rc;
        if ((rc = upload<int>(h, own, fkrow.data(), fkrow.size(), &R.fac_krow))) return rc;
        if ((rc = upload<double>(h, own, fkc_cl.data(), fkc_cl.size(), &R.fac_kc_cl))) return rc;
        if ((rc = upload<int>(h, own, fkrow_cl.data(), fkrow_cl.size(), &R.fac_krow_cl))) return rc;
    }
#ifdef CPG_GENI_HEADER
    if (r->shared_mats) {
        const InstanceTables g{0, r->sol_chunks, r->sol_nnz, r->sol_slots, r->sol_ctab, r->sol_desc, r->sol_cols, r->sol_kind, r->sol_idx,
                               r->fac_chunks, r->fac_triples, r->fac_ctab, r->fac_task, r->fac_len, r->fac_a, r->fac_b, r->fac_k};
        if ((rc = set_instance_executor(h, r, g, fkc, fkrow))) return rc;
    }
#endif
    if ((rc = rt_sync(h))) return rc;
    h->refactor_mode = true;
    h->have_update = true;
    return CPG_OK;
}

int cpg_hip_set_refactor_merged(cpg_handle_t h, const cpg_osqp_refactor_t *r, const cpg_osqp_resident_t *mg) {
    if (h && h->conic) { set_error("not available for a conic (interior-point) handle"); return CPG_E_BADARG; }
    if (!h || !r || !mg) { set_error("null argument"); return CPG_E_BADARG; }
    if (!r->shared_mats || mg->nnzX <= 0) { set_error("cpg_hip_set_refactor_merged: needs shared-matrix tables and a merged program"); return CPG_E_BADARG; }
    int rc = cpg_hip_set_refactor(h, r);
    if (rc) return rc;
#ifdef CPG_GENI_NNZX
    if (mg->nnzX == CPG_GENI_NNZX) {
        std::vector<double> fkc;
        std::vector<int> fkrow;
        if (!kkt_constants(h, r, fkc, fkrow)) { set_error("cpg_hip_set_refactor_merged: KKT source table out of range"); return CPG_E_BADARG; }
        const InstanceTables g{mg->nnzX, mg->sol_chunks, mg->sol_nnz, mg->sol_slots, mg->sol_ctab, mg->sol_desc, mg->sol_cols, mg->sol_kind,
                               mg->sol_idx, mg->fac_chunks, mg->fac_triples, mg->f_ctab, mg->f_task, mg->f_len, mg->f_a, mg->f_b, mg->f_k};
        if ((rc = set_instance_executor(h, r, g, fkc, fkrow))) return rc;
    }
#endif
    return CPG_OK;
}

int cpg_hip_set_shared_registers(cpg_handle_t h, const cpg_osqp_resident_t *mg, const double *coef, int32_t n_coef, double rho, double sigma) {
    if (h && h->conic) { set_error("not available for a conic (interior-point) handle"); return CPG_E_BADARG; }
    if (!h || !mg || !coef) { set_error("null argument"); return CPG_E_BADARG; }
    if (h->refactor_mode) { set_error("cpg_hip_set_shared_registers: needs a shared-factor handle"); return CPG_E_BADARG; }
    h->sreg_ok = false;
    h->SRg = cpg::DevShRegs{};
    int rc = rt_sync(h);
    if (rc) return rc;
    free_list(h->sreg_owned);
#if defined(CPG_GENI_HEADER) && defined(CPG_GENI_NNZX)
#ifdef CPG_GENI_N
    const bool geni_dims = h->F.n == CPG_GENI_N && h->F.m == CPG_GENI_M && h->F.n_eq == CPG_GENI_NEQ;
#else
    const bool geni_dims = true;
#endif
    if (!(geni_dims && mg->nnzX == CPG_GENI_NNZX && mg->sol_chunks == CPG_GENI_NCHUNKS && mg->sol_nnz == CPG_GENI_NNZ &&
          mg->sol_slots == CPG_GENI_NSLOTS && n_coef == mg->sol_nnz))
        return CPG_OK;
    if (program_fingerprint(mg->sol_ctab, mg->sol_desc, mg->sol_cols, mg->sol_chunks, mg->sol_nnz) != CPG_GENI_FINGERPRINT) return CPG_OK;
    static const int steps[][4] = CPG_GENI_STEPS;
    static const int chunk_shift[] = CPG_GENI_CHUNK_SHIFT;
    std::vector<unsigned short> gcols, grows;
    if (!generated_tables(mg->sol_ctab, mg->sol_desc, mg->sol_cols, mg->sol_chunks, mg->sol_nnz, mg->sol_slots, steps, CPG_GENI_NSTEPS,
                          gcols, grows, chunk_shift))
        return CPG_OK;
    std::vector<double> cf((size_t)CPG_GENI_NREGS * 64, 0.0);
    std::vector<char> taken(cf.size(), 0);
    for (int t = 0; t < CPG_GENI_NSTEPS; t++) {
        const int e = steps[t][0], cnt = steps[t][1], reg = steps[t][2], sh = steps[t][3];
        if (reg < 0 || reg >= CPG_GENI_NREGS) return CPG_OK;
        for (int l = 0; l < cnt; l++) {
            const size_t at = (size_t)reg * 64 + (size_t)(l + sh);
            if (taken[at]) return CPG_OK;
            taken[at] = 1;
            cf[at] = coef[e + l];
        }
    }
    cpg::DevShRegs T{};
    if ((rc = upload<double>(h, h->sreg_owned, cf.data(), cf.size(), &T.cf))) return rc;
    if ((rc = upload<unsigned short>(h, h->sreg_owned, gcols.data(), gcols.size(), &T.cols))) return rc;
    if ((rc = upload<unsigned short>(h, h->sreg_owned, grows.data(), grows.size(), &T.rows))) return rc;
    if ((rc = rt_sync(h))) return rc;
    h->SRg = T;
    h->sreg_ok = true;
    h->sreg_rho = rho; h->sreg_sigma = sigma;
#else
    (void)n_coef; (void)rho; (void)sigma;
#endif
    return CPG_OK;
}

#if defined(CPG_GENT_HEADER)
#define CPG_RX(x) CPG_GENT_##x
#define CPG_RX_PRESENT 1
#define CPG_RX_FAC 1
#elif defined(CPG_GENR_HEADER)
#define CPG_RX(x) CPG_GENR_##x
#define CPG_RX_PRESENT 1
#ifdef CPG_GENR_FAC_NSTEPS
#define CPG_RX_FAC 1
#endif
#endif
#ifdef CPG_GENT_HEADER
static bool team_tables(const std::vector<unsigned short> &gcols, const std::vector<unsigned short> &grows, int T, int n_chunks,
                        const int *step_wave, const int *step_local, const int *chunk_wave, const int *chunk_local, int W, int n_off, int n_row,
                        int n_slots, std::vector<unsigned> &toff, std::vector<unsigned> &trow) {
    const unsigned zero_off = (unsigned)(n_slots + CPG_GEN_DUMMY_SLOTS) * 8u, dummy = (unsigned)n_slots;
    toff.assign((size_t)W * n_off * 64, zero_off | (zero_off << 16));
    trow.assign((size_t)W * n_row * 64, dummy | (dummy << 16));
    for (int t = 0; t < T; t++) {
        const int wv = step_wave[t], j = step_local[t];
        if (wv < 0 || wv >= W || j < 0 || j / 2 >= n_off) return false;
        for (int l = 0; l < 64; l++) {
            unsigned &wd = toff[((size_t)wv * n_off + (size_t)(j / 2)) * 64 + l];
            const unsigned v = gcols[((size_t)(t / 4) * 64 + l) * 4 + (t % 4)];
            wd = (j & 1) ? ((wd & 0xFFFFu) | (v << 16)) : ((wd & 0xFFFF0000u) | v);
        }
    }
    for (int c = 0; c < n_chunks; c++) {
        const int wv = chunk_wave[c], j = chunk_local[c];
        if (wv < 0 || wv >= W || j < 0 || j / 2 >= n_row) return false;
        for (int l = 0; l < 64; l++) {
            unsigned &wd = trow[((size_t)wv * n_row + (size_t)(j / 2)) * 64 + l];
            const unsigned v = grows[((size_t)(c >> 2) * 64 + l) * 4 + (c & 3)];
            wd = (j & 1) ? ((wd & 0xFFFFu) | (v << 16)) : ((wd & 0xFFFF0000u) | v);
        }
    }
    return true;
}
#endif
int cpg_hip_set_resident(cpg_handle_t h, const cpg_osqp_refactor_t *r, const cpg_osqp_resident_t *rs) {
    int rc = cpg_hip_set_refactor(h, r);
    if (rc) return rc;
    free_list(h->resident_owned);
    h->Rs = cpg::DevResident{};
    if (!rs) { set_error("null argument"); return CPG_E_BADARG; }
#ifdef CPG_RX_PRESENT
    if (r->shared_mats) return CPG_OK;
    std::vector<void *> &own = h->resident_owned;
    cpg::DevResident &Rs = h->Rs;
    const int n = h->F.n, m = h->F.m, N = n + m, nnzL = r->nnzL;
    if (n != CPG_RX(N) || m != CPG_RX(M) || h->F.n_eq != CPG_RX(NEQ) || r->nnzA != CPG_RX(NNZA) || r->nnzP != CPG_RX(NNZP) ||
        nnzL != CPG_RX(NNZL) || rs->nnzX != CPG_RX(NNZX) ||
// ... 703 lines not shown
```

cvxpygen_amd/csrc/cpg_osqp_kernel.h:

```cpp
#pragma once

#include <type_traits>
#include "cpg_wave.h"

namespace cpg {

#define CPG_INFTY 1e30
#define CPG_MIN_SCALING 1e-4
#define CPG_DIV_TOL 1e-30
#define CPG_RHO_MIN 1e-6
#define CPG_RHO_MAX 1e6
#define CPG_NO_ROW 0xFFFF
#ifndef CPG_ILP
#define CPG_ILP 2
#endif
#define CPG_FENCE_EVERY(s) do { if (((s) + 1) % CPG_ILP == 0) cpgw::sched_fence(); } while (0)
#ifndef CPG_LDS_UNROLL
#define CPG_LDS_UNROLL 4
#endif
#ifndef CPG_CHUNK_UNROLL
#define CPG_CHUNK_UNROLL 4
#endif

struct DevProgram {
// ... 261 lines not shown
    }
}

#define CPG_GEN_SLOT_MASK 0x1FFFu
#define CPG_GEN_DUMMY_SLOTS 16
#define CPG_GEN_EXTRA_SLOTS (CPG_GEN_DUMMY_SLOTS + 1)
#ifdef CPG_GEN_HEADER
#define CPG_GEN_ZERO(A) _Pragma("unroll") for (int g_ = 0; g_ < G; g_++) A[g_] = 0.0
#define CPG_GEN_PAD 64
#ifdef CPG_GEN_COMPRESSED
#define CPG_GEN_VB(vals, lane) ((const char *)(vals))
#define CPG_GEN_CB(cols, lane) ((const char *)(cols) + (unsigned)(lane) * 4u)
#define CPG_GEN_LOAD_CV(ID, E) const unsigned wd##ID = *(const unsigned *)(cb + (E) * 4u);
#define CPG_GEN_LOAD_W(ID)                                                                         \
    const double vl##ID = *(const double *)(vb + (wd##ID >> 16));                                  \
    double x##ID[G];                                                                               \
    _Pragma("unroll") for (int g_ = 0; g_ < G; g_++) x##ID[g_] = *(const double *)(wb + (unsigned)g_ * ldwb + (wd##ID & 0xFFFFu));
#else
#define CPG_GEN_VB(vals, lane) ((const char *)(vals) + (unsigned)(lane) * 8u)
#define CPG_GEN_CB(cols, lane) ((const char *)(cols) + (unsigned)(lane) * 2u)
#define CPG_GEN_LOAD_CV(ID, E)                                                                     \
    const double vl##ID = *(const double *)(vb + (E) * 8u);                                        \
    const unsigned co##ID = *(const unsigned short *)(cb + (E) * 2u);
#define CPG_GEN_LOAD_CVP(ID, E, K)                                                                 \
    const double vl##ID = *(const double *)(vb + (E) * 8u);                                        \
    const unsigned co##ID = *(const unsigned short *)(cb + (K) * 128u);
#define CPG_GEN_LOAD_CVP2A(ID, E, K)                                                               \
    const double vl##ID = *(const double *)(vb + (E) * 8u);                                        \
    const unsigned cp##ID = *(const unsigned *)(cb + (unsigned)lane * 2u + ((K) >> 1) * 256u);     \
    const unsigned co##ID = cp##ID & 0xFFFFu;
#define CPG_GEN_LOAD_CVP2B(ID, E, PREV)                                                            \
    const double vl##ID = *(const double *)(vb + (E) * 8u);                                        \
    const unsigned co##ID = cp##PREV >> 16;
#define CPG_GEN_LOAD_CVP4A(ID, E, K)                                                               \
    const double vl##ID = *(const double *)(vb + (E) * 8u);                                        \
    const OffsetQuad cq##ID = *(const OffsetQuad *)(cb + (unsigned)lane * 6u + ((K) >> 2) * 512u);          \
    const unsigned co##ID = cq##ID.a & 0xFFFFu;
#define CPG_GEN_LOAD_CVP4B(ID, E, FIRST, J)                                                        \
    const double vl##ID = *(const double *)(vb + (E) * 8u);                                        \
    const unsigned co##ID = (J) == 1 ? cq##FIRST.a >> 16 : (J) == 2 ? (cq##FIRST.b & 0xFFFFu) : cq##FIRST.b >> 16;
#define CPG_GEN_LOAD_W(ID)                                                                         \
    double x##ID[G];                                                                               \
    _Pragma("unroll") for (int g_ = 0; g_ < G; g_++) x##ID[g_] = *(const double *)(wb + (unsigned)g_ * ldwb + co##ID);
#endif
#define CPG_GEN_FMA_FULL(A, ID)                                                                    \
    _Pragma("unroll") for (int g_ = 0; g_ < G; g_++) A[g_] = fma(vl##ID, x##ID[g_], A[g_]);
#define CPG_GEN_FMA_PART(A, ID, CNT)                                                               \
    {                                                                                              \
        const double v_ = lane < (CNT) ? vl##ID : 0.0;                                             \
        _Pragma("unroll") for (int g_ = 0; g_ < G; g_++) A[g_] = fma(v_, x##ID[g_], A[g_]);        \
    }
#define CPG_GEN_LOAD_ROWS(Q) const OffsetQuad rq##Q = *(const OffsetQuad *)((const char *)rows + (unsigned)lane * 8u + (Q) * 512u);
#define CPG_GEN_ROW(Q, J) ((J) == 0 ? (rq##Q.a & 0xFFFFu) : (J) == 1 ? (rq##Q.a >> 16) : (J) == 2 ? (rq##Q.b & 0xFFFFu) : (rq##Q.b >> 16))
#define CPG_GEN_REDUCE_STORE(A, LG, Q, J)                                                          \
    {                                                                                              \
        const unsigned row_ = CPG_GEN_ROW(Q, J) & CPG_GEN_SLOT_MASK;                               \
        _Pragma("unroll") for (int g_ = 0; g_ < G; g_++)                                           \
            w[(unsigned)(g_ * ldw) + row_] = cpgw::group_sum_first<LG>(A[g_]);                     \
    }
#define CPG_GEN_SEGREDUCE_STORE_LIT(A, S, Q, J, M0, M1, M2)                                       \
    {                                                                                              \
        const unsigned row_ = CPG_GEN_ROW(Q, J) & CPG_GEN_SLOT_MASK;                               \
        _Pragma("unroll") for (int g_ = 0; g_ < G; g_++)                                           \
            w[(unsigned)(g_ * ldw) + row_] = cpgw::seg_sum_first_lit<S>(A[g_], M0, M1, M2);        \
    }
#define CPG_GEN_SEGREDUCE_STORE(A, S, Q, J)                                                        \
    {                                                                                              \
        const unsigned e_ = CPG_GEN_ROW(Q, J);                                                     \
        _Pragma("unroll") for (int g_ = 0; g_ < G; g_++)                                           \
            w[(unsigned)(g_ * ldw) + (e_ & CPG_GEN_SLOT_MASK)] = cpgw::seg_sum_first<S>(A[g_], e_ >> 13); \
    }
}
#include CPG_GEN_HEADER
namespace cpg {
#ifndef CPG_GEN_N
#error "generated program headers must carry the family dimensions (codegen.write_program_header(plan=...))"
#endif
#ifdef CPG_GEN_N
struct GenFam {
    static constexpr unsigned n = CPG_GEN_N, m = CPG_GEN_M;
    static constexpr int n_slots = CPG_GEN_NSLOTS;
    static constexpr int ct(int s) { constexpr signed char t[] = CPG_GEN_CT_INIT; return t[s]; }
    static constexpr int rows_len(int which, int s) {
        constexpr int a[][2] = CPG_GEN_AROWS; constexpr int p[][2] = CPG_GEN_PROWS; constexpr int t[][2] = CPG_GEN_ATROWS;
        return which == 0 ? (s < CPG_GEN_AROWS_N ? a[s < CPG_GEN_AROWS_N ? s : 0][0] : 0)
             : which == 1 ? (s < CPG_GEN_PROWS_N ? p[s < CPG_GEN_PROWS_N ? s : 0][0] : 0)
                          : (s < CPG_GEN_ATROWS_N ? t[s < CPG_GEN_ATROWS_N ? s : 0][0] : 0);
    }
    static constexpr int rows_off(int which, int s) {
        constexpr int a[][2] = CPG_GEN_AROWS; constexpr int p[][2] = CPG_GEN_PROWS; constexpr int t[][2] = CPG_GEN_ATROWS;
        return which == 0 ? a[s < CPG_GEN_AROWS_N ? s : 0][1] : which == 1 ? p[s < CPG_GEN_PROWS_N ? s : 0][1]
                                                                            : t[s < CPG_GEN_ATROWS_N ? s : 0][1];
    }
};
#endif
#endif

CPG_DEV double natural_chunk(const DevProgram &P, int s, const double *w, int lane) {
    double o[1];
    o[0] = 0.0;
    if (s < P.n_chunks) do_chunk<1, false>(P, s, w, 0, lane, o);
    return o[0];
}

#ifndef CPG_ROWS_BATCH
#define CPG_ROWS_BATCH 8
#endif
CPG_DEV double natural_chunk_lit(const DevProgram &P, const int len, const int off, const double *w, int lane_in) {
    const int lane = cpgw::opaque(lane_in);
    const unsigned e0 = (unsigned)off * 64u + (unsigned)lane;
    double acc = 0.0;
#pragma unroll
    for (int t0 = 0; t0 < len; t0 += CPG_ROWS_BATCH) {
        double v[CPG_ROWS_BATCH];
        unsigned c[CPG_ROWS_BATCH];
#pragma unroll
        for (int t = 0; t < CPG_ROWS_BATCH; t++)
            if (t0 + t < len) { v[t] = cpgw::gld(P.vals, e0 + 64u * (unsigned)(t0 + t)); c[t] = cpgw::gld(P.cols, e0 + 64u * (unsigned)(t0 + t)); }
#pragma unroll
        for (int t = 0; t < CPG_ROWS_BATCH; t++)
            if (t0 + t < len) acc = fma(v[t], w[c[t]], acc);
    }
    return acc;
}
#ifdef CPG_GEN_N
#define CPG_NATURAL_ROWS(P, which, s, w, lane) natural_chunk_lit(P, GenFam::rows_len(which, s), GenFam::rows_off(which, s), w, lane)
#else
#define CPG_NATURAL_ROWS(P, which, s, w, lane) natural_chunk(P, s, w, lane)
#endif

template <int NSX, int NSZ, int NV>
struct Inst {
    static const int NVX = MinI<NV, NSX>::v, NVZ = MinI<NV, NSZ>::v;
    double x[NSX], z[NSZ], y[NSZ];
    double qv[NVX], uv[NVZ];
    double dconst;
    long long b;
    int done;
};

struct CheckOut {
    double prim_res, dual_res, obj;
    int status;
};

CPG_DEV double csr_row(const DevCsr &mp, unsigned row, const double *theta, double v) {
    if (mp.nnz > 0) {
        const unsigned s = (unsigned)cpgw::gld(mp.ptr, row), e = (unsigned)cpgw::gld(mp.ptr, row + 1u);
        for (unsigned k = s; k < e; k++) v = fma(cpgw::gld(mp.val, k), cpgw::gld(theta, (unsigned)cpgw::gld(mp.idx, k)), v);
    }
    return v;
}

template <int NSX, int NSZ, int NV>
struct SharedCtx {
    static constexpr bool kTestsFirst = true;
    static constexpr bool kOpaqueLane = true;
    const DevFamily &F;
    const double *sh, *shu;
    const Inst<NSX, NSZ, NV> &I;
    const double *w;
    int lane;
    CPG_DEV double q(int s, unsigned i) const {
        return s < Inst<NSX, NSZ, NV>::NVX ? I.qv[s < Inst<NSX, NSZ, NV>::NVX ? s : 0] : sh[i];
    }
    CPG_DEV double u(int s, unsigned i) const {
        return s < Inst<NSX, NSZ, NV>::NVZ ? I.uv[s < Inst<NSX, NSZ, NV>::NVZ ? s : 0] : shu[i];
    }
    CPG_DEV void products(int) const {}
    CPG_DEV void stage(int) const {}
    CPG_DEV double sE(unsigned i) const { return cpgw::gld(F.E, i); }
    CPG_DEV double sEinv(unsigned i) const { return cpgw::gld(F.Einv, i); }
    CPG_DEV double sD(unsigned i) const { return cpgw::gld(F.D, i); }
    CPG_DEV double sDinv(unsigned i) const { return cpgw::gld(F.Dinv, i); }
    CPG_DEV double ax(int s) const { return CPG_NATURAL_ROWS(F.A_rows, 0, s, w, lane); }
    CPG_DEV double px(int s) const { return CPG_NATURAL_ROWS(F.P_rows, 1, s, w, lane); }
    CPG_DEV double atx(int s) const { return CPG_NATURAL_ROWS(F.At_rows, 2, s, w, lane); }
};

template <int NSX, int NSZ, int NV>
CPG_DEV bool canonicalise(const DevFamily &F, const DevUpdate &U, const double *theta,
                          Inst<NSX, NSZ, NV> &I, int lane) {
    bool bad = false;
#pragma unroll
    for (int s = 0; s < NSX; s++) I.x[s] = 0.0;
#pragma unroll
    for (int s = 0; s < NSZ; s++) { I.z[s] = 0.0; I.y[s] = 0.0; }
#pragma unroll
    for (int s = 0; s < Inst<NSX, NSZ, NV>::NVX; s++) {
        const unsigned i = (unsigned)lane + 64u * (unsigned)s;
        I.qv[s] = (i < (unsigned)F.n) ? csr_row(U.map_q, i, theta, cpgw::gld(U.q_base, i)) : 0.0;
    }
#pragma unroll
    for (int s = 0; s < Inst<NSX, NSZ, NV>::NVZ; s++) {
        const unsigned i = (unsigned)lane + 64u * (unsigned)s;
        I.uv[s] = 0.0;
        if (i < (unsigned)F.m) {
            const double uv = csr_row(U.map_u, i, theta, cpgw::gld(U.u_base, i));
            I.uv[s] = uv;
            const int ctp = (int)cpgw::gld(F.ctype, i);
            bad |= (ctp == 0 && uv > CPG_INFTY * CPG_MIN_SCALING) || (ctp == -1 && !(uv > CPG_INFTY * CPG_MIN_SCALING));
        }
    }
    I.dconst = csr_row(U.map_d, 0, theta, U.d_base);
    return cpgw::wave_any(bad);
}

template <int NS>
struct RegDelta {
    const double (&a)[NS];
    CPG_DEV double operator()(int s, unsigned) const { return a[s]; }
};
struct MemDelta {
    const double *p;
    CPG_DEV double operator()(int, unsigned i) const { return cpgw::gld(p, i); }
};
struct NoDelta {
    CPG_DEV double operator()(int, unsigned) const { return 0.0; }
};

template <int NSX, int NSZ, typename Ctx, typename DY>
CPG_DEV bool primal_infeasible(const DevFamily &F, const Ctx &cx, const signed char (&ct)[NSZ],
                               bool unsc, double eps, double *w, const DY &dy, int lane) {
    cx.stage(1);
    double nrm = 0.0, lhs = 0.0;
    double dyp[NSZ];
#pragma unroll
    for (int s = 0; s < NSZ; s++) {
        const unsigned i = (unsigned)lane + 64u * (unsigned)s;
        dyp[s] = 0.0;
        if (i < (unsigned)F.m) {
            const double uu = cx.u(s, i);
            const bool eq = ct[s] == 1;
            const double ll = eq ? uu : -CPG_INFTY;
            const bool iu = uu > CPG_INFTY * CPG_MIN_SCALING, il = !eq;
            double d = dy(s, i);
            if (iu && il) d = 0.0; else if (iu) d = cpgw::dmin2(d, 0.0); else if (il) d = cpgw::dmax2(d, 0.0);
            dyp[s] = d;
            nrm = cpgw::dmax2(nrm, fabs(unsc ? cx.sE(i) * d : d));
            lhs += uu * cpgw::dmax2(d, 0.0) + ll * cpgw::dmin2(d, 0.0);
        }
        cpgw::sched_fence();
    }
    nrm = cpgw::wave_max_nonneg(nrm);
    if (!(nrm > CPG_DIV_TOL)) return false;
    lhs = cpgw::wave_sum(lhs);
    if (!(lhs < eps * nrm)) return false;
#pragma unroll
    for (int s = 0; s < NSZ; s++) { const unsigned i = (unsigned)lane + 64u * (unsigned)s; if (i < (unsigned)F.m) w[(unsigned)F.n + i] = dyp[s]; }
    cpgw::lds_order();
    cx.products(4);
    double r = 0.0;
#pragma unroll
    for (int s = 0; s < NSX; s++) {
        const unsigned i = (unsigned)lane + 64u * (unsigned)s;
        const double t = cx.atx(s);
        if (i < (unsigned)F.n) r = cpgw::dmax2(r, fabs(unsc ? cx.sDinv(i) * t : t));
        cpgw::sched_fence();
    }
    r = cpgw::wave_max_nonneg(r);
    cpgw::lds_order();
    return r < eps * nrm;
}

template <int NSX, int NSZ, typename Ctx, typename DX>
CPG_DEV bool dual_infeasible(const DevFamily &F, const Ctx &cx, const signed char (&ct)[NSZ],
                             bool unsc, double eps, double *w, const DX &dx, int lane) {
    cx.stage(2);
    double nrm = 0.0, qdx = 0.0;
#pragma unroll
    for (int s = 0; s < NSX; s++) {
        const unsigned i = (unsigned)lane + 64u * (unsigned)s;
        if (i < (unsigned)F.n) {
            const double d = dx(s, i);
            nrm = cpgw::dmax2(nrm, fabs(unsc ? cx.sD(i) * d : d));
            qdx += cx.q(s, i) * d;
        }
    }
    nrm = cpgw::wave_max_nonneg(nrm);
    if (!(nrm > CPG_DIV_TOL)) return false;
    const double cs = unsc ? F.c : 1.0;
    qdx = cpgw::wave_sum(qdx);
    if (!(qdx < -cs * eps * nrm)) return false;
#pragma unroll
    for (int s = 0; s < NSX; s++) { const unsigned i = (unsigned)lane + 64u * (unsigned)s; if (i < (unsigned)F.n) w[i] = dx(s, i); }
    cpgw::lds_order();
    cx.products(2);
    double r = 0.0;
#pragma unroll
    for (int s = 0; s < NSX; s++) {
        const unsigned i = (unsigned)lane + 64u * (unsigned)s;
        const double t = cx.px(s);
        if (i < (unsigned)F.n) r = cpgw::dmax2(r, fabs(unsc ? cx.sDinv(i) * t : t));
        cpgw::sched_fence();
    }
    r = cpgw::wave_max_nonneg(r);
    bool res = false;
    if (r < cs * eps * nrm) {
        cx.products(1);
        bool viol = false;
#pragma unroll
        for (int s = 0; s < NSZ; s++) {
            const unsigned i = (unsigned)lane + 64u * (unsigned)s;
            const double a = cx.ax(s);
            if (i < (unsigned)F.m) {
                const double av = unsc ? cx.sEinv(i) * a : a;
                if ((cx.u(s, i) < CPG_INFTY * CPG_MIN_SCALING && av > eps * nrm) ||
                    (ct[s] == 1 && av < -eps * nrm)) viol = true;
            }
            cpgw::sched_fence();
        }
        res = !cpgw::wave_any(viol);
    }
    cpgw::lds_order();
    return res;
}

struct InfeasVerdict { bool primal, dual; };

template <int NSX, int NSZ, typename Ctx, typename DX, typename DY>
CPG_DEV InfeasVerdict infeasibility_tests(const DevFamily &F, const Ctx &cx, const signed char (&ct)[NSZ],
                                          const DevSettings &S, const DX &dx, const DY &dy,
                                          double *w, int lane_in, bool approximate) {
    const int lane = cpgw::opaque(lane_in);
    cpgw::assume((unsigned)lane < 64u);
    const bool unsc = !S.scaled_termination;
    const double mult = approximate ? 10.0 : 1.0;
    InfeasVerdict v;
    v.primal = F.m != 0 && primal_infeasible<NSX, NSZ, Ctx, DY>(F, cx, ct, unsc, S.eps_prim_inf * mult, w, dy, lane);
    v.dual = dual_infeasible<NSX, NSZ, Ctx, DX>(F, cx, ct, unsc, S.eps_dual_inf * mult, w, dx, lane);
    return v;
}

struct ScaledNorms {
    double prim_res, dual_res;
    double nz, nax, nq, naty, npx;
};

template <int NSX, int NSZ, typename Ctx, typename DX, typename DY>
CPG_DEV CheckOut check(const DevFamily &F, const Ctx &cx, const signed char (&ct)[NSZ],
                       const DevSettings &S, const double (&Ix)[NSX], const double (&Iz)[NSZ],
                       const double (&Iy)[NSZ], const DX &dx, const DY &dy, InfeasVerdict iv,
                       double *w, int lane_in, bool approximate, ScaledNorms *sn = nullptr) {
    const int lane = (Ctx::kTestsFirst || Ctx::kOpaqueLane) ? cpgw::opaque(lane_in) : lane_in;
    cpgw::assume((unsigned)lane < 64u);
    const bool unsc = !S.scaled_termination;
    const double mult = approximate ? 10.0 : 1.0;
    const double ea = S.eps_abs * mult, er = S.eps_rel * mult;
    CheckOut o;
#pragma unroll
    for (int s = 0; s < NSX; s++) { const unsigned i = (unsigned)lane + 64u * (unsigned)s; if (i < (unsigned)F.n) w[i] = Ix[s]; }
#pragma unroll
    for (int s = 0; s < NSZ; s++) { const unsigned i = (unsigned)lane + 64u * (unsigned)s; if (i < (unsigned)F.m) w[(unsigned)F.n + i] = Iy[s]; }
    cpgw::lds_order();
    cx.products(1);
    double rp = 0.0, nz = 0.0, na = 0.0, sup = 0.0;
    double s_rp = 0.0, s_nz = 0.0, s_na = 0.0;
#pragma unroll
    for (int s = 0; s < NSZ; s++) {
        const unsigned i = (unsigned)lane + 64u * (unsigned)s;
        const double ax = cx.ax(s);
        if (i < (unsigned)F.m) {
            const double ei = unsc ? cx.sEinv(i) : 1.0;
            rp = cpgw::dmax2(rp, fabs(ei * (ax - Iz[s])));
            nz = cpgw::dmax2(nz, fabs(ei * Iz[s]));
            na = cpgw::dmax2(na, fabs(ei * ax));
            if (sn) { s_rp = cpgw::dmax2(s_rp, fabs(ax - Iz[s])); s_nz = cpgw::dmax2(s_nz, fabs(Iz[s])); s_na = cpgw::dmax2(s_na, fabs(ax)); }
            if (S.check_dualgap) {
                const double uu = cx.u(s, i), yy = Iy[s];
                if (uu < CPG_INFTY * CPG_MIN_SCALING && yy > 0.0) sup += uu * yy;
                if (ct[s] == 1 && uu > -CPG_INFTY * CPG_MIN_SCALING && yy < 0.0) sup += uu * yy;
            }
        }
        cpgw::sched_fence();
    }
    cx.products(6);
    double rd = 0.0, nq = 0.0, nat = 0.0, npx = 0.0, quad = 0.0, lin = 0.0;
    double s_rd = 0.0, s_nq = 0.0, s_nat = 0.0, s_npx = 0.0;
#pragma unroll
    for (int s = 0; s < NSX; s++) {
        const unsigned i = (unsigned)lane + 64u * (unsigned)s;
        const double px = cx.px(s);
        const double aty = cx.atx(s);
        if (i < (unsigned)F.n) {
            const double di = unsc ? cx.sDinv(i) : 1.0;
            const double qq = cx.q(s, i);
            rd = cpgw::dmax2(rd, fabs(di * (qq + px + aty)));
            nq = cpgw::dmax2(nq, fabs(di * qq));
            nat = cpgw::dmax2(nat, fabs(di * aty));
            npx = cpgw::dmax2(npx, fabs(di * px));
            if (sn) { s_rd = cpgw::dmax2(s_rd, fabs(qq + px + aty)); s_nq = cpgw::dmax2(s_nq, fabs(qq));
                      s_nat = cpgw::dmax2(s_nat, fabs(aty)); s_npx = cpgw::dmax2(s_npx, fabs(px)); }
            quad += Ix[s] * px;
            lin += qq * Ix[s];
        }
        cpgw::sched_fence();
    }
    cpgw::lds_order();
    const double cs = unsc ? F.cinv : 1.0;
    rp = cpgw::wave_max_nonneg(rp); nz = cpgw::wave_max_nonneg(nz); na = cpgw::wave_max_nonneg(na);
    rd = cs * cpgw::wave_max_nonneg(rd);
    const double dn = cs * cpgw::dmax2(cpgw::wave_max_nonneg(nq),
                                       cpgw::dmax2(cpgw::wave_max_nonneg(nat), cpgw::wave_max_nonneg(npx)));
    quad = cpgw::wave_sum(quad); lin = cpgw::wave_sum(lin);
    o.prim_res = rp; o.dual_res = rd; o.obj = (0.5 * quad + lin) * F.cinv;
    if (sn) {
        sn->prim_res = cpgw::wave_max_nonneg(s_rp); sn->nz = cpgw::wave_max_nonneg(s_nz); sn->nax = cpgw::wave_max_nonneg(s_na);
        sn->dual_res = cpgw::wave_max_nonneg(s_rd); sn->nq = cpgw::wave_max_nonneg(s_nq);
        sn->naty = cpgw::wave_max_nonneg(s_nat); sn->npx = cpgw::wave_max_nonneg(s_npx);
    }

    o.status = 11;
    if (rp > CPG_INFTY || rd > CPG_INFTY) { o.status = 9; o.obj = NAN; return o; }
    bool pc = false, dc = false, pic = false, dic = false, gc = true;
    if (F.m == 0) pc = true;
    else if (rp < ea + er * cpgw::dmax2(nz, na)) pc = true;
    else pic = Ctx::kTestsFirst ? iv.primal : primal_infeasible<NSX, NSZ, Ctx, DY>(F, cx, ct, unsc, S.eps_prim_inf * mult, w, dy, lane);
    if (rd < ea + er * dn) dc = true;
    else dic = Ctx::kTestsFirst ? iv.dual : dual_infeasible<NSX, NSZ, Ctx, DX>(F, cx, ct, unsc, S.eps_dual_inf * mult, w, dx, lane);
    if (S.check_dualgap) {
        sup = cpgw::wave_sum(sup);
        const double dual_obj = (-0.5 * quad - sup) * F.cinv, gap = fabs(quad + lin + sup) * F.cinv;
        gc = gap < ea + er * cpgw::dmax2(fabs(o.obj), fabs(dual_obj));
    }
    if (pc && dc && gc) o.status = approximate ? 2 : 1;
    else if (pic) { o.status = approximate ? 4 : 3; o.obj = CPG_INFTY; }
    else if (dic) { o.status = approximate ? 6 : 5; o.obj = -CPG_INFTY; }
    return o;
}

template <int NSX, int NSZ>
CPG_DEV void store_state(const DevFamily &F, double *so, const double (&Ix)[NSX], const double (&Iz)[NSZ],
                         const double (&Iy)[NSZ], bool keep, double rho, int lane) {
#pragma unroll
    for (int s = 0; s < NSX; s++) {
        const unsigned i = (unsigned)lane + 64u * (unsigned)s;
        if (i < (unsigned)F.n) cpgw::gst(so, F.ord ? (unsigned)cpgw::gld(F.ord, i) : i, keep ? Ix[s] : 0.0);
    }
#pragma unroll
    for (int s = 0; s < NSZ; s++) {
        const unsigned i = (unsigned)lane + 64u * (unsigned)s;
        if (i < (unsigned)F.m) {
            const unsigned c = F.ord ? (unsigned)cpgw::gld(F.ord, (unsigned)F.n + i) : i;
            cpgw::gst(so, (unsigned)F.n + c, keep ? Iz[s] : 0.0);
            cpgw::gst(so, (unsigned)(F.n + F.m) + c, keep ? Iy[s] : 0.0);
        }
    }
    if (lane == 0) so[F.n + 2 * F.m] = rho;
}

CPG_DEV double rho_estimate(const ScaledNorms &sn, double rho_settings) {
    const double pr = sn.prim_res / (cpgw::dmax2(sn.nz, sn.nax) + CPG_DIV_TOL);
    const double dr = sn.dual_res / (cpgw::dmax2(sn.nq, cpgw::dmax2(sn.naty, sn.npx)) + CPG_DIV_TOL);
    return cpgw::dmin2(cpgw::dmax2(rho_settings * sqrt(pr / dr), CPG_RHO_MIN), CPG_RHO_MAX);
}

template <int NSX, int NSZ, bool OPAQUE_LANE = true>
CPG_DEV void finalize(const DevFamily &F, const DevBatch &Bt, const double (&Ix)[NSX], const double (&Iz)[NSZ],
                      const double (&Iy)[NSZ], double dconst, long long b, double *w, int lane_in, int iter,
                      const CheckOut &o, double rho) {
    const int lane = OPAQUE_LANE ? cpgw::opaque(lane_in) : lane_in;
    cpgw::assume((unsigned)lane < 64u);
    const bool has_sol = o.status == 1 || o.status == 2 || o.status == 7;
    if (Bt.state_out) store_state<NSX, NSZ>(F, Bt.state_out + (size_t)b * (size_t)(F.n + 2 * F.m + 1), Ix, Iz, Iy, has_sol, rho, lane);
#pragma unroll
    for (int s = 0; s < NSX; s++) { const unsigned i = (unsigned)lane + 64u * (unsigned)s; if (i < (unsigned)F.n) w[i] = has_sol ? cpgw::gld(F.D, i) * Ix[s] : NAN; }
#pragma unroll
    for (int s = 0; s < NSZ; s++) { const unsigned i = (unsigned)lane + 64u * (unsigned)s; if (i < (unsigned)F.m) w[(unsigned)F.n + i] = has_sol ? F.cinv * cpgw::gld(F.E, i) * Iy[s] : NAN; }
    cpgw::lds_order();
    double *pp = Bt.prim + (size_t)b * F.n_prim, *dp = Bt.dual + (size_t)b * F.n_dual;
    for (unsigned k = (unsigned)lane; k < (unsigned)F.n_prim; k += 64u) cpgw::gst(pp, k, w[(unsigned)cpgw::gld(F.prim_idx, k)]);
    for (unsigned k = (unsigned)lane; k < (unsigned)F.n_dual; k += 64u) cpgw::gst(dp, k, w[(unsigned)F.n + (unsigned)cpgw::gld(F.dual_idx, k)]);
    if (lane == 0) {
        double ov = o.obj + dconst;
        if (F.is_max) ov = -ov;
        Bt.obj[b] = ov; Bt.iter[b] = iter; Bt.status[b] = o.status;
        Bt.pri_res[b] = o.prim_res; Bt.dua_res[b] = o.dual_res;
    }
    cpgw::lds_order();
}

template <int NSX, int NSZ>
CPG_DEV void load_state(const DevFamily &F, const double *si, double (&Ix)[NSX], double (&Iz)[NSZ],
                        double (&Iy)[NSZ], int lane) {
#pragma unroll
    for (int s = 0; s < NSX; s++) {
        const unsigned i = (unsigned)lane + 64u * (unsigned)s;
        if (i < (unsigned)F.n) Ix[s] = cpgw::gld(si, F.ord ? (unsigned)cpgw::gld(F.ord, i) : i);
    }
#pragma unroll
    for (int s = 0; s < NSZ; s++) {
        const unsigned i = (unsigned)lane + 64u * (unsigned)s;
        if (i < (unsigned)F.m) {
            const unsigned c = F.ord ? (unsigned)cpgw::gld(F.ord, (unsigned)F.n + i) : i;
            Iz[s] = cpgw::gld(si, (unsigned)F.n + c); Iy[s] = cpgw::gld(si, (unsigned)(F.n + F.m) + c);
        }
    }
}

#define CPG_STATUS_HANDED_OVER (-3)
template <int NSX, int NSZ>
CPG_DEV void hand_over(const DevFamily &F, const DevBatch &Bt, const double (&Ix)[NSX], const double (&Iz)[NSZ],
                       const double (&Iy)[NSZ], long long b, int lane_in, int iter, double rho_new) {
    const int lane = cpgw::opaque(lane_in);
    cpgw::assume((unsigned)lane < 64u);
    if (!Bt.ho_state || !Bt.ho_list) {
        if (lane == 0) { Bt.obj[b] = NAN; Bt.iter[b] = iter; Bt.status[b] = -2; Bt.pri_res[b] = 0.0; Bt.dua_res[b] = 0.0; }
        return;
    }
    store_state<NSX, NSZ>(F, Bt.ho_state + (size_t)b * (size_t)(F.n + 2 * F.m + 1), Ix, Iz, Iy, true, rho_new, lane);
    if (lane == 0) {
        Bt.iter[b] = iter; Bt.status[b] = CPG_STATUS_HANDED_OVER;
        Bt.ho_list[cpgw::atomic_next(Bt.ho_count)] = (int)b;
    }
}

#if defined(CPG_GEN_N)
#define CPG_ROW_CLASS(s) (GenFam::ct(s) != 2 ? GenFam::ct(s) : (int)ct[s])
#else
#define CPG_ROW_CLASS(s) ((int)ct[s])
#endif

struct DevShRegs {
    const double *cf;
    const unsigned short *cols, *rows;
};
struct NoRegExec {
    static constexpr bool active = false;
    static constexpr int nslots = 1;
    CPG_DEV explicit NoRegExec(const DevShRegs &) {}
    CPG_DEV size_t stage(double *) { return 0; }
    CPG_DEV void load(int) {}
    CPG_DEV void run(double *, int) const {}
};

template <int NSX, int NSZ, int NV, int G, bool LDSPROG, typename REG = NoRegExec>
CPG_DEV void osqp_shared_body(const DevFamily &F, const DevUpdate &U, const DevSettings &S,
                              const DevBatch &Bt, double *lds, int wave_global, const DevShRegs &RG = DevShRegs{}) {
    typedef Inst<NSX, NSZ, NV> InstT;
    static_assert(!REG::active || (G == 1 && !LDSPROG), "the register executor serves one instance per wavefront");
    const int lane0 = cpgw::lane_id();
    const int lane = lane0;
#if defined(CPG_GEN_N)
    constexpr unsigned n_c = GenFam::n, m_c = GenFam::m;
    constexpr int ldw = REG::active ? REG::nslots : GenFam::n_slots + CPG_GEN_EXTRA_SLOTS;
    static_assert(!LDSPROG || ((n_c + 63) / 64 == (unsigned)NSX && (m_c + 63) / 64 == (unsigned)NSZ), "slot class of the generated family");
#else
    const unsigned n_c = (unsigned)F.n, m_c = (unsigned)F.m;
    const int ldw = REG::active ? REG::nslots : F.n_slots;
#endif
    const int N = F.n + F.m;
    double *sh = lds;
    for (unsigned t = cpgw::thread_in_block(); t < (unsigned)N; t += cpgw::block_threads())
        sh[t] = t < (unsigned)F.n ? cpgw::gld(U.q_base, t) : cpgw::gld(U.u_base, t - (unsigned)F.n);
    const double *shu = sh + n_c;
    LdsProg LP;
    size_t lds_off = (size_t)N;
    if (LDSPROG) {
        const DevRagged &R = F.kkt_ragged;
#ifdef CPG_GEN_HEADER
        const unsigned nnzp = (unsigned)R.nnz + CPG_GEN_PAD;
#else
        const unsigned nnzp = (unsigned)R.nnz;
#endif
        const unsigned nt = cpgw::block_threads(), t0 = cpgw::thread_in_block();
#ifdef CPG_GEN_COMPRESSED
        double *lv = lds + lds_off;                         lds_off += (size_t)R.n_dict;
        unsigned *lw = (unsigned *)(lds + lds_off);         lds_off += (size_t)((nnzp + 1) / 2);
        for (unsigned t = t0; t < (unsigned)R.n_dict; t += nt) lv[t] = cpgw::gld(R.dict, t);
        for (unsigned t = t0; t < nnzp; t += nt) lw[t] = t < (unsigned)R.nnz ? cpgw::gld(R.words, t) : 0u;
        const unsigned short *lc = (const unsigned short *)lw;
#else
        double *lv = lds + lds_off;                         lds_off += (size_t)nnzp;
#ifdef CPG_GEN_PADDED_OFFSETS
        constexpr unsigned n_off = 64u * ((CPG_GEN_PADDED_OFFSETS + 3u) & ~3u);
        unsigned short *lc = (unsigned short *)(lds + lds_off); lds_off += (size_t)((n_off + 3) / 4);
        for (unsigned t = t0; t < nnzp; t += nt) lv[t] = t < (unsigned)R.nnz ? cpgw::gld(R.vals, t) : 0.0;
        for (unsigned t = t0; t < n_off; t += nt) lc[t] = cpgw::gld(R.cols_padded, t);
#else
        unsigned short *lc = (unsigned short *)(lds + lds_off); lds_off += (size_t)((nnzp + 3) / 4);
        for (unsigned t = t0; t < nnzp; t += nt) {
            const bool in = t < (unsigned)R.nnz;
            lv[t] = in ? cpgw::gld(R.vals, t) : 0.0; lc[t] = in ? cpgw::gld(R.cols, t) : (unsigned short)0;
        }
#endif
#endif
        LP.vals = lv; LP.cols = lc; LP.n_chunks = R.n_chunks; LP.dummy = (unsigned)R.nnz - 1u;
#ifdef CPG_GEN_HEADER
        const unsigned n_rows16 = (((unsigned)R.n_chunks + 3u) & ~3u) * 64u;
        unsigned short *lr = (unsigned short *)(lds + lds_off); lds_off += (size_t)(n_rows16 / 4u);
        for (unsigned t = t0; t < n_rows16; t += nt) lr[t] = cpgw::gld(R.rows_gen, t);
        LP.rows16 = lr; LP.ctab = nullptr; LP.desc = nullptr;
#else
        unsigned *ld = (unsigned *)(lds + lds_off);         lds_off += (size_t)R.n_chunks * 32;
        int *lt = (int *)(lds + lds_off);                   lds_off += (size_t)R.n_chunks * 2;
        for (unsigned t = t0; t < (unsigned)R.n_chunks * 64u; t += nt) ld[t] = cpgw::gld(R.desc, t);
        for (unsigned t = t0; t < (unsigned)R.n_chunks * 4u; t += nt) lt[t] = cpgw::gld(R.ctab, t);
        LP.ctab = lt; LP.desc = ld; LP.rows16 = nullptr;
#endif
    }
    REG rg(RG);
    lds_off += rg.stage(lds + lds_off);
    cpgw::block_sync();
    rg.load(lane);
    double *w = lds + lds_off + (size_t)cpgw::wave_in_block() * G * ldw;
    (void)wave_global;
    const long long ngroups = (Bt.B + G - 1) / G;
    const double rho_eq = 1e3 * F.rho, rho_in = F.rho, rho_fr = 1e-6;
    const double ri_eq = 1.0 / rho_eq, ri_in = 1.0 / rho_in, ri_fr = 1.0 / rho_fr;
    signed char ct_reg[NSZ];
    unsigned short fpx[NSX], fpz[NSZ];
#pragma unroll
    for (int s = 0; s < NSX; s++) {
        const unsigned i = (unsigned)lane + 64u * (unsigned)s;
        fpx[s] = 0;
        if (i < (unsigned)F.n) fpx[s] = !REG::active ? cpgw::gld(F.fpos, i) : (unsigned short)(F.ord ? (unsigned)cpgw::gld(F.ord, i) : i);
    }
#pragma unroll
    for (int s = 0; s < NSZ; s++) {
        const unsigned i = (unsigned)lane + 64u * (unsigned)s;
        ct_reg[s] = (i < (unsigned)F.m) ? cpgw::gld(F.ctype, i) : 0;
        fpz[s] = 0;
        if (i < (unsigned)F.m)
            fpz[s] = !REG::active ? cpgw::gld(F.fpos, (unsigned)F.n + i)
                                  : (unsigned short)((unsigned)F.n + (F.ord ? (unsigned)cpgw::gld(F.ord, (unsigned)F.n + i) : i));
    }

    for (;;) {
        const int lane = cpgw::opaque(lane0);
        cpgw::assume((unsigned)lane < 64u);
        unsigned ig = 0;
        if (lane == 0) ig = cpgw::atomic_next(Bt.counter);
        ig = (unsigned)cpgw::read_first_lane((int)ig);
        if ((long long)ig >= ngroups) break;

        InstT I[G];
        CheckOut co[G];
        int n_open = 0;
#ifdef CPG_GEN_HEADER
        for (unsigned t = (unsigned)lane; t < (unsigned)(G * ldw); t += 64u) w[t] = 0.0;
        cpgw::lds_order();
#endif
#pragma unroll
        for (int g = 0; g < G; g++) {
            const long long b = (long long)ig * G + g;
            I[g].b = b < Bt.B ? b : -1;
            I[g].done = b < Bt.B ? 0 : 1;
            co[g].prim_res = 0; co[g].dual_res = 0; co[g].obj = 0; co[g].status = 11;
            const double *theta = Bt.theta + (size_t)(b < Bt.B ? b : 0) * U.np_var;
            const bool bad = canonicalise<NSX, NSZ, NV>(F, U, theta, I[g], lane);
            if (Bt.state_in && S.warm_starting && b < Bt.B)
                load_state<NSX, NSZ>(F, Bt.state_in + (size_t)b * (size_t)(F.n + 2 * F.m + 1), I[g].x, I[g].z, I[g].y, lane);
            if (Bt.state_in && b < Bt.B && !bad) {
                const double rho_in = cpgw::gld(Bt.state_in + (size_t)b * (size_t)(F.n + 2 * F.m + 1), (unsigned)(F.n + 2 * F.m));
                if (__builtin_expect(cpgw::dmin2(cpgw::dmax2(rho_in, CPG_RHO_MIN), CPG_RHO_MAX) != F.rho, 0)) {
                    hand_over<NSX, NSZ>(F, Bt, I[g].x, I[g].z, I[g].y, b, lane, 0, rho_in);
                    I[g].done = 1;
                }
            }
            if (__builtin_expect(bad && !I[g].done, 0)) {
                if (lane == 0) { Bt.obj[b] = NAN; Bt.iter[b] = 0; Bt.status[b] = -2; Bt.pri_res[b] = 0.0; Bt.dua_res[b] = 0.0; }
                I[g].done = 1;
            }
            n_open += I[g].done ? 0 : 1;
        }

        int iter = 0;
        auto rhs_and_solve = [&]() __attribute__((always_inline)) {
            const int lane_outer = lane;
            const int lane = cpgw::opaque(lane_outer);
            cpgw::assume((unsigned)lane < 64u);
            signed char ct[NSZ];
#pragma unroll
            for (int s = 0; s < NSZ; s++) ct[s] = (signed char)cpgw::opaque((int)ct_reg[s]);
#pragma unroll
            for (int g = 0; g < G; g++) {
                double *wg = w + g * ldw;
#pragma unroll
                for (int s = 0; s < NSX; s++) {
                    const unsigned i = (unsigned)lane + 64u * (unsigned)s;
                    if (i < n_c) wg[REG::active ? (unsigned)fpx[s] : i] = F.sigma * I[g].x[s] - SharedCtx<NSX, NSZ, NV>{F, sh, shu, I[g], wg, lane}.q(s, i);
                    CPG_FENCE_EVERY(s);
                }
#pragma unroll
                for (int s = 0; s < NSZ; s++) {
                    const unsigned i = (unsigned)lane + 64u * (unsigned)s;
                    const int cts = CPG_ROW_CLASS(s);
                    const double ri = cts == 1 ? ri_eq : (cts == 0 ? ri_in : ri_fr);
                    if (i < m_c) wg[REG::active ? (unsigned)fpz[s] : n_c + i] = I[g].z[s] - ri * I[g].y[s];
                    CPG_FENCE_EVERY(s);
                }
            }
            cpgw::lds_order();
            if (REG::active) rg.run(w, lane);
            else
#ifdef CPG_GEN_HEADER
            if (LDSPROG) run_program_gen<G>(LP.vals, LP.cols, LP.rows16, w, ldw, lane);
#else
            if (LDSPROG) run_program_lds<G>(LP, w, ldw, lane);
#endif
            else if (G == 1 && F.kkt_stream.n_pairs > 0) run_program_stream(F.kkt_stream, w, lane);
            else run_program<G>(F.kkt, w, ldw, lane);
        };
        auto update = [&](auto stash_c, double (&dxr)[G][NSX], double (&dyr)[G][NSZ]) __attribute__((always_inline)) {
            constexpr bool STASH = decltype(stash_c)::value;
            const int lane_outer = lane;
            const int lane = cpgw::opaque(lane_outer);
            cpgw::assume((unsigned)lane < 64u);
            signed char ct[NSZ];
#pragma unroll
            for (int s = 0; s < NSZ; s++) ct[s] = (signed char)cpgw::opaque((int)ct_reg[s]);
#pragma unroll
            for (int g = 0; g < G; g++) {
                const double *wg = w + g * ldw;
#pragma unroll
                for (int s = 0; s < NSX; s++) {
                    const unsigned i = (unsigned)lane + 64u * (unsigned)s;
                    if (STASH) dxr[g][s] = 0.0;
                    if (i < n_c) {
                        const double xn = F.alpha * wg[fpx[s]] + (1.0 - F.alpha) * I[g].x[s];
                        if (STASH) dxr[g][s] = xn - I[g].x[s];
                        I[g].x[s] = xn;
                    }
                    CPG_FENCE_EVERY(s);
                }
#pragma unroll
                for (int s = 0; s < NSZ; s++) {
                    const unsigned i = (unsigned)lane + 64u * (unsigned)s;
                    if (STASH) dyr[g][s] = 0.0;
                    if (i < m_c) {
                        const int cts = CPG_ROW_CLASS(s);
                        const double rv = cts == 1 ? rho_eq : (cts == 0 ? rho_in : rho_fr);
                        const double ri = cts == 1 ? ri_eq : (cts == 0 ? ri_in : ri_fr);
                        const double zp = I[g].z[s], yp = I[g].y[s];
                        const double zt = (zp - ri * yp) + ri * wg[fpz[s]];
                        const double zr = F.alpha * zt + (1.0 - F.alpha) * zp;
                        const double uu = SharedCtx<NSX, NSZ, NV>{F, sh, shu, I[g], wg, lane}.u(s, i);
                        const double zn = cts == 1 ? uu : cpgw::dmin2(zr + ri * yp, uu);
                        const double dyv = rv * (zr - zn);
                        I[g].z[s] = zn; I[g].y[s] = yp + dyv;
                        if (STASH) dyr[g][s] = dyv;
                    }
                    CPG_FENCE_EVERY(s);
                }
            }
            cpgw::lds_order();
        };
        const int chk_int = S.check_termination;
        const int ad_int = (S.adaptive_rho && S.adaptive_rho_interval > 0) ? S.adaptive_rho_interval : 0;
#pragma nounroll
        while (n_open > 0) {
            double dxr[G][NSX], dyr[G][NSZ];
            if (iter < S.max_iter) {
                int next_ev = S.max_iter;
                if (chk_int > 0) { const int c = (iter / chk_int + 1) * chk_int; if (c < next_ev) next_ev = c; }
                if (ad_int > 0) { const int c = (iter / ad_int + 1) * ad_int; if (c < next_ev) next_ev = c; }
#pragma nounroll
                for (;;) {
                    iter++;
                    rhs_and_solve();
                    if (iter >= next_ev) break;
                    update(std::false_type{}, dxr, dyr);
                }
                update(std::true_type{}, dxr, dyr);
            } else {
#pragma unroll
                for (int g = 0; g < G; g++) {
#pragma unroll
                    for (int s = 0; s < NSX; s++) dxr[g][s] = 0.0;
#pragma unroll
                    for (int s = 0; s < NSZ; s++) dyr[g][s] = 0.0;
                }
            }
            const bool last = iter >= S.max_iter;
            const bool can_check = last || (chk_int > 0 && iter % chk_int == 0);
            const bool adapt = ad_int > 0 && iter > 0 && iter % ad_int == 0;
            InfeasVerdict iv_exact[G], iv_approx[G];
#pragma unroll
            for (int g = 0; g < G; g++) {
                iv_exact[g] = iv_approx[g] = InfeasVerdict{false, false};
                if (I[g].done || !can_check) continue;
                double *wg = w + g * ldw;
#pragma nounroll
                for (int pass = 0; pass < (last ? 2 : 1); pass++) {
                    const InfeasVerdict v = infeasibility_tests<NSX, NSZ, SharedCtx<NSX, NSZ, NV>, RegDelta<NSX>, RegDelta<NSZ>>(
                        F, SharedCtx<NSX, NSZ, NV>{F, sh, shu, I[g], wg, lane}, ct_reg, S,
                        RegDelta<NSX>{dxr[g]}, RegDelta<NSZ>{dyr[g]}, wg, lane, pass == 1);
                    if (pass == 0) iv_exact[g] = v; else iv_approx[g] = v;
                }
            }
#pragma unroll
            for (int g = 0; g < G; g++) {
                if (I[g].done) continue;
                CheckOut o = co[g];
                if (REG::active) { o.prim_res = 0; o.dual_res = 0; o.obj = 0; o.status = 11; }
                double *wg = w + g * ldw;
                ScaledNorms sn;
                double rho_ws = F.rho;
                bool rho_changed = false;
#pragma nounroll
                for (int pass = 0; pass < 2; pass++) {
                    if (pass == 1 && !(o.status == 11 && last)) break;
                    const CheckOut oc = check<NSX, NSZ, SharedCtx<NSX, NSZ, NV>, NoDelta, NoDelta>(
                        F, SharedCtx<NSX, NSZ, NV>{F, sh, shu, I[g], wg, lane}, ct_reg, S, I[g].x, I[g].z, I[g].y,
                        NoDelta{}, NoDelta{}, pass == 0 ? iv_exact[g] : iv_approx[g], wg, lane, pass == 1,
                        (pass == 0 && adapt) ? &sn : nullptr);
                    if (can_check) o = oc;
                    if (pass == 0 && adapt && o.status == 11) {
                        const double rn = rho_estimate(sn, F.rho);
                        if (rn > F.rho * S.adaptive_rho_tolerance || rn < F.rho / S.adaptive_rho_tolerance) { rho_ws = rn; rho_changed = true; }
                    }
                }
                if (o.status == 11 && last) o.status = 7;
                co[g] = o;
                if (o.status != 11) {
                    finalize<NSX, NSZ>(F, Bt, I[g].x, I[g].z, I[g].y, I[g].dconst, I[g].b, wg, lane, iter, o, rho_ws);
                    I[g].done = 1; n_open--;
                } else if (rho_changed) {
                    hand_over<NSX, NSZ>(F, Bt, I[g].x, I[g].z, I[g].y, I[g].b, lane, iter, rho_ws);
                    I[g].done = 1; n_open--;
                }
            }
        }
    }
}

}
```

cvxpygen_amd/csrc/cpg_osqp_refactor.h:

```cpp
#pragma once

#include "cpg_osqp_kernel.h"

#ifdef CPG_GENI_HEADER
#include CPG_GENI_HEADER
#endif
#ifdef CPG_GENS_HEADER
#include CPG_GENS_HEADER
#define CPG_GENS_ACTIVE(geni, shared, crlds) (!(geni) && !(shared) && !(crlds))
#else
#define CPG_GENS_ACTIVE(geni, shared, crlds) false
#endif

namespace cpg {

#ifdef CPG_GENI_HEADER
struct GeniRows {
    static constexpr int len(int which, int s) {
        constexpr int a[][2] = CPG_GENI_AROWS; constexpr int p[][2] = CPG_GENI_PROWS; constexpr int t[][2] = CPG_GENI_ATROWS;
        return which == 0 ? (s < CPG_GENI_AROWS_N ? a[s < CPG_GENI_AROWS_N ? s : 0][0] : 0)
             : which == 1 ? (s < CPG_GENI_PROWS_N ? p[s < CPG_GENI_PROWS_N ? s : 0][0] : 0)
                          : (s < CPG_GENI_ATROWS_N ? t[s < CPG_GENI_ATROWS_N ? s : 0][0] : 0);
    }
    static constexpr int off(int which, int s) {
        constexpr int a[][2] = CPG_GENI_AROWS; constexpr int p[][2] = CPG_GENI_PROWS; constexpr int t[][2] = CPG_GENI_ATROWS;
        return which == 0 ? a[s < CPG_GENI_AROWS_N ? s : 0][1] : which == 1 ? p[s < CPG_GENI_PROWS_N ? s : 0][1]
                                                                            : t[s < CPG_GENI_ATROWS_N ? s : 0][1];
    }
};
#define CPG_GENI_ROWS(P, which, s, w, lane) natural_chunk_lit(P, GeniRows::len(which, s), GeniRows::off(which, s), w, lane)
#endif

struct DevRefactor {
    int nnzP, nnzA, nnzL, n_eq, np_var, scaling_iters;
    const int *Ap, *Ai, *Arp, *Aent, *Acol, *Pp, *Pi, *Prp, *Pent, *Pcol;
    const int *Lcol, *ksrc_kind, *ksrc_idx;
    const int *fac_ctab;
    const unsigned *fac_task, *fac_len, *fac_a, *fac_b, *fac_k;
    int fac_chunks;
    const int *sol_kind, *sol_idx;
    const unsigned short *sol_fpos;
    int sol_nnz, sol_slots;
    const unsigned *sol_stab;
    const unsigned *sol_cr;
    int sol_pairs;
    const double *P_base, *A_base, *q_base, *u_base;
    const double *q_setup;
    double d_base;
    DevCsr map_P, map_A, map_q, map_u, map_d;
    long long buf_doubles;
    int shared_mats;
    const double *Ps, *As, *Ars, *Ds, *Dinvs, *Es, *Einvs;
    double cs;
    int gi_ok;
    const unsigned short *gi_cols, *gi_rows;
    const unsigned *gi_src;
    const unsigned short *gi_lcol;
    const unsigned long long *gf_tri;
    const unsigned *gf_dk;
    const double *gf_kc;
    const unsigned short *gs_cols, *gs_rows;
    const int *gs_kind, *gs_idx;
    int gs_ok, gs_nnz;
    const double *fac_kc;
    const int *fac_krow;
    const double *fac_kc_cl;
    const int *fac_krow_cl;
    const int *fac_kind_cl, *fac_idx_cl;
};

#define CPG_K_NONE 0
#define CPG_K_P 1
#define CPG_K_A 2
#define CPG_K_SIGMA 3
#define CPG_K_RHO 4

CPG_DEV double lim_scaling(double v) { v = v < 1e-4 ? 1.0 : v; return v > 1e4 ? 1e4 : v; }

struct InstBuf {
    double *P, *A, *D, *Dinv, *E, *Einv, *q, *u, *rinv, *Lx, *Dg, *Dginv, *sv;
    double *Ar;
};
CPG_DEV InstBuf carve(double *b, const DevFamily &F, const DevRefactor &R) {
    InstBuf o;
    const size_t n = (size_t)F.n, m = (size_t)F.m, N = n + m;
    o.P = b; b += R.nnzP; o.A = b; b += R.nnzA;
    o.D = b; b += n; o.Dinv = b; b += n; o.E = b; b += m; o.Einv = b; b += m;
    o.q = b; b += n; o.u = b; b += m; o.rinv = b; b += m;
    o.Lx = b; b += R.nnzL; o.Dg = b; b += N; o.Dginv = b; b += N;
    o.sv = b; b += R.sol_nnz > R.gs_nnz ? R.sol_nnz : R.gs_nnz;
    o.Ar = b; b += R.nnzA;
    return o;
}

#ifndef CPG_ROW_COPY_BATCH
#define CPG_ROW_COPY_BATCH 8
#endif
CPG_DEV void refresh_row_copy(const DevRefactor &R, const InstBuf &B, int lane) {
    cpgw::mem_order();
    for (unsigned k = (unsigned)lane; k < (unsigned)R.nnzA; k += 64u)
        cpgw::gst(B.Ar, k, cpgw::gld((const double *)B.A, (unsigned)cpgw::gld(R.Aent, k)));
    cpgw::mem_order();
}

#ifndef CPG_ROW_WALK_BATCH
#define CPG_ROW_WALK_BATCH 4
#endif
template <bool ENT, int NB = CPG_ROW_WALK_BATCH, class Fn>
CPG_DEV void for_row_entries(const int *ptr, const int *ent, const int *col, const double *val, unsigned r, Fn f) {
    const unsigned a = (unsigned)cpgw::gld(ptr, r), e = (unsigned)cpgw::gld(ptr, r + 1u);
    for (unsigned k = a; k < e; k += (unsigned)NB) {
        unsigned en[NB], co[NB];
#pragma unroll
        for (int t = 0; t < NB; t++) {
            const unsigned kk = k + (unsigned)t < e ? k + (unsigned)t : a;
            en[t] = ENT ? (unsigned)cpgw::gld(ent, kk) : kk;
            co[t] = (unsigned)cpgw::gld(col, kk);
        }
        double av[NB];
#pragma unroll
        for (int t = 0; t < NB; t++) av[t] = cpgw::gld(val, en[t]);
#pragma unroll
        for (int t = 0; t < NB; t++)
            if (k + (unsigned)t < e) f(av[t], co[t]);
    }
}

template <int NSX, int NSZ, bool QUMEM = false>
struct InstCtx {
    static constexpr bool kTestsFirst = false;
    static constexpr bool kOpaqueLane = QUMEM;
    const DevFamily &F;
    const DevRefactor &R;
    const InstBuf &B;
    const double *w;
    int lane;
    const double (&qr)[NSX];
    const double (&ur)[NSZ];
    const double *qm, *um;
    bool rowprog;
    CPG_DEV double rows_gen(const DevProgram &P, int which, int s) const {
#ifdef CPG_GENI_HEADER
        return CPG_GENI_ROWS(P, which, s, w, lane);
#else
        return natural_chunk(P, s, w, lane);
#endif
    }
    CPG_DEV void products(int) const {}
    CPG_DEV void stage(int) const {}
    CPG_DEV double sE(unsigned i) const { return cpgw::gld(F.E, i); }
    CPG_DEV double sEinv(unsigned i) const { return cpgw::gld(F.Einv, i); }
    CPG_DEV double sD(unsigned i) const { return cpgw::gld(F.D, i); }
    CPG_DEV double sDinv(unsigned i) const { return cpgw::gld(F.Dinv, i); }
    CPG_DEV double q(int s, unsigned i) const { return QUMEM ? qm[i] : qr[s]; }
    CPG_DEV double u(int s, unsigned i) const { return QUMEM ? um[i] : ur[s]; }
    template <bool ENT, bool OFFS, int NB = CPG_ROW_WALK_BATCH>
    CPG_DEV double row_dot(const int *ptr, const int *ent, const int *col, const double *val, unsigned r) const {
        double acc = 0.0;
        const double *wv = w + (OFFS ? (unsigned)F.n : 0u);
        for_row_entries<ENT, NB>(ptr, ent, col, val, r, [&](double v, unsigned c) { acc = fma(v, wv[c], acc); });
        return acc;
    }
    CPG_DEV double ax(int s) const {
        if (QUMEM || rowprog) return QUMEM ? rows_gen(F.A_rows, 0, s) : natural_chunk(F.A_rows, s, w, lane);
        const unsigned i = (unsigned)lane + 64u * (unsigned)s;
#ifdef CPG_REFACTOR_ROW_COPY
        return i < (unsigned)F.m ? row_dot<false, false, CPG_ROW_COPY_BATCH>(R.Arp, nullptr, R.Acol, (const double *)B.Ar, i) : 0.0;
#else
        return i < (unsigned)F.m ? row_dot<true, false>(R.Arp, R.Aent, R.Acol, (const double *)B.A, i) : 0.0;
#endif
    }
    CPG_DEV double px(int s) const {
        if (QUMEM || rowprog) return QUMEM ? rows_gen(F.P_rows, 1, s) : natural_chunk(F.P_rows, s, w, lane);
        const unsigned j = (unsigned)lane + 64u * (unsigned)s;
        return j < (unsigned)F.n ? row_dot<true, false>(R.Prp, R.Pent, R.Pcol, (const double *)B.P, j) : 0.0;
    }
    CPG_DEV double atx(int s) const {
        if (QUMEM || rowprog) return QUMEM ? rows_gen(F.At_rows, 2, s) : natural_chunk(F.At_rows, s, w, lane);
        const unsigned j = (unsigned)lane + 64u * (unsigned)s;
        return j < (unsigned)F.n ? row_dot<false, true>(R.Ap, nullptr, R.Ai, (const double *)B.A, j) : 0.0;
    }
};


#ifndef CPG_LDL_BATCH
#define CPG_LDL_BATCH 4
#endif
CPG_DEV void numeric_ldl(const DevRefactor &R, const InstBuf &B, double reg, int lane) {
    int level_start = 0;
#pragma nounroll
    for (int c = 0; c < R.fac_chunks; c++) {
        const int L = cpgw::read_first_lane(cpgw::gld(R.fac_ctab, 4u * (unsigned)c));
        const int last = cpgw::read_first_lane(cpgw::gld(R.fac_ctab, 4u * (unsigned)c + 1u));
        unsigned base = (unsigned)cpgw::read_first_lane(cpgw::gld(R.fac_ctab, 4u * (unsigned)c + 2u));
        const int lg = cpgw::read_first_lane(cpgw::gld(R.fac_ctab, 4u * (unsigned)c + 3u));
        const unsigned task = cpgw::gld(R.fac_task, (unsigned)c * 64u + (unsigned)lane);
        const unsigned lw = cpgw::gld(R.fac_len, (unsigned)c * 64u + (unsigned)lane);
        const int len = (int)(lw & 0xFFFFu), rlen = (int)(lw >> 16);
        double acc = 0.0;
        constexpr int NB = CPG_LDL_BATCH;
        unsigned ia[NB], ib[NB], ik[NB];
        auto load_indices = [&](int s0, unsigned (&xa)[NB], unsigned (&xb)[NB], unsigned (&xk)[NB]) __attribute__((always_inline)) {
#pragma unroll
            for (int t = 0; t < NB; t++) {
                const bool on = s0 + t < len;
                const unsigned e = on ? base + (unsigned)lane : 0u;
                base += cpgw::popc64(cpgw::ballot(on));
                xa[t] = cpgw::gld(R.fac_a, e); xb[t] = cpgw::gld(R.fac_b, e); xk[t] = cpgw::gld(R.fac_k, e);
            }
        };
        load_indices(0, ia, ib, ik);
#pragma nounroll
        for (int s = 0; s < L; s += NB) {
            double la[NB], lb[NB], dk[NB];
#pragma unroll
            for (int t = 0; t < NB; t++) {
                la[t] = cpgw::gld((const double *)B.Lx, ia[t]);
                lb[t] = cpgw::gld((const double *)B.Lx, ib[t]);
                dk[t] = cpgw::gld((const double *)B.Dg, ik[t]);
            }
            unsigned na[NB], nb[NB], nk[NB];
            if (s + NB < L) load_indices(s + NB, na, nb, nk);
#pragma unroll
            for (int t = 0; t < NB; t++)
                if (s + t < rlen) acc = fma(la[t] * dk[t], lb[t], acc);
#pragma unroll
            for (int t = 0; t < NB; t++) { ia[t] = na[t]; ib[t] = nb[t]; ik[t] = nk[t]; }
        }
        acc = cpgw::group_sum_first_dyn(acc, lg);
        if (task != 0xFFFFFFFFu) {
            const int kind = cpgw::gld(R.ksrc_kind, task);
            const unsigned idx = (unsigned)cpgw::gld(R.ksrc_idx, task);
            const bool piv = task >= (unsigned)R.nnzL;
            double kv = 0.0;
            if (kind == CPG_K_P) kv = cpgw::gld((const double *)B.P, idx) + (piv ? reg : 0.0);
            else if (kind == CPG_K_A) kv = cpgw::gld((const double *)B.A, idx);
            else if (kind == CPG_K_SIGMA) kv = reg;
            else if (kind == CPG_K_RHO) kv = -cpgw::gld((const double *)B.rinv, idx);
            const double v = kv - acc;
            if (piv) { cpgw::gst(B.Dg, task - (unsigned)R.nnzL, v); cpgw::gst(B.Dginv, task - (unsigned)R.nnzL, 1.0 / v); }
            else cpgw::gst(B.Lx, task, v);
        }
        if (last) {
            cpgw::mem_order();
#pragma nounroll
            for (int c2 = level_start; c2 <= c; c2++) {
                const unsigned t2 = cpgw::gld(R.fac_task, (unsigned)c2 * 64u + (unsigned)lane);
                if (t2 < (unsigned)R.nnzL)
                    cpgw::gst(B.Lx, t2, cpgw::gld((const double *)B.Lx, t2) * cpgw::gld((const double *)B.Dginv, (unsigned)cpgw::gld(R.Lcol, t2)));
            }
            cpgw::mem_order();
            level_start = c + 1;
        }
    }
}
template <bool MFORM = false, bool GENS = false>
CPG_DEV void substitution_values(const DevRefactor &R, const InstBuf &B, int lane) {
    const int *kinds = GENS ? R.gs_kind : R.sol_kind, *idxs = GENS ? R.gs_idx : R.sol_idx;
    const unsigned cnt = GENS ? (unsigned)R.gs_nnz : (unsigned)R.sol_nnz;
    for (unsigned e = (unsigned)lane; e < cnt; e += 64u) {
        const int kind = cpgw::gld(kinds, e);
        const unsigned idx = (unsigned)cpgw::gld(idxs, e);
        double v = 0.0;
        if (kind == 1) v = 1.0;
        else if (kind == 2) v = MFORM ? -(cpgw::gld((const double *)B.Lx, idx) * cpgw::gld((const double *)B.Dginv, (unsigned)cpgw::gld(R.Lcol, idx)))
                                      : -cpgw::gld((const double *)B.Lx, idx);
        else if (kind == 3) v = cpgw::gld((const double *)B.Dginv, idx);
        cpgw::gst(B.sv, e, v);
    }
    cpgw::mem_order();
}

template <bool LDS, bool KCONST = true>
CPG_DEV void numeric_ldl_m(const DevRefactor &R, double *Ml, double *Dil, const double *rinv, int lane,
                           const double *Pv = nullptr, const double *Av = nullptr, double reg = 0.0) {
    constexpr int NB = CPG_LDL_BATCH;
    struct Hdr { int L, last, lg; unsigned base; };
    struct LaneTab { unsigned task, lw; double kc; int krow; int kind; };
    struct Idx { unsigned a[NB], b[NB], k[NB]; unsigned base; };
    const unsigned *ctab = (const unsigned *)R.fac_ctab;
    const int nch = R.fac_chunks;
    if (nch <= 0) return;
    auto hdr = [&](int c) __attribute__((always_inline)) {
        const unsigned o = 4u * (unsigned)(c < nch ? c : nch - 1);
        return Hdr{(int)cpgw::sld(ctab, o), (int)cpgw::sld(ctab, o + 1u), (int)cpgw::sld(ctab, o + 3u), cpgw::sld(ctab, o + 2u)};
    };
    auto lanetab = [&](int c) __attribute__((always_inline)) {
        const unsigned e = (unsigned)(c < nch ? c : nch - 1) * 64u + (unsigned)lane;
        if (KCONST) return LaneTab{cpgw::gld(R.fac_task, e), cpgw::gld(R.fac_len, e), cpgw::gld(R.fac_kc_cl, e), cpgw::gld(R.fac_krow_cl, e), 0};
        return LaneTab{cpgw::gld(R.fac_task, e), cpgw::gld(R.fac_len, e), 0.0, cpgw::gld(R.fac_idx_cl, e), cpgw::gld(R.fac_kind_cl, e)};
    };
    auto indices = [&](unsigned base, int len, int s0) __attribute__((always_inline)) {
        Idx x;
#pragma unroll
        for (int t = 0; t < NB; t++) {
            const bool on = s0 + t < len;
            const unsigned e = on ? base + (unsigned)lane : 0u;
            base += cpgw::popc64(cpgw::ballot(on));
            x.a[t] = cpgw::gld(R.fac_a, e); x.b[t] = cpgw::gld(R.fac_b, e); x.k[t] = cpgw::gld(R.fac_k, e);
        }
        x.base = base;
        return x;
    };
    Hdr h0 = hdr(0), h1 = hdr(1);
    LaneTab t0 = lanetab(0), t1 = lanetab(1);
    Idx i0 = indices(h0.base, (int)(t0.lw & 0xFFFFu), 0);
#pragma nounroll
    for (int c = 0; c < nch; c++) {
        const Hdr h2 = hdr(c + 2);
        const LaneTab t2 = lanetab(c + 2);
        const Idx i1 = indices(h1.base, (int)(t1.lw & 0xFFFFu), 0);
        const bool has = t0.task != 0xFFFFFFFFu;
        double kr = 0.0, kc = t0.kc;
        if (KCONST) { if (has && t0.krow >= 0) kr = cpgw::gld(rinv, (unsigned)t0.krow); }
        else if (has) {
            const bool piv = t0.task >= (unsigned)R.nnzL;
            if (t0.kind == CPG_K_P) kc = cpgw::gld(Pv, (unsigned)t0.krow) + (piv ? reg : 0.0);
            else if (t0.kind == CPG_K_A) kc = cpgw::gld(Av, (unsigned)t0.krow);
            else if (t0.kind == CPG_K_SIGMA) kc = reg;
            else if (t0.kind == CPG_K_RHO) kr = cpgw::gld(rinv, (unsigned)t0.krow);
        }
        const int L = cpgw::read_first_lane(h0.L), len = (int)(t0.lw & 0xFFFFu), rlen = (int)(t0.lw >> 16);
        double acc = 0.0;
        Idx cur = i0;
#pragma nounroll
        for (int s = 0; s < L; s += NB) {
            double la[NB], lb[NB], dk[NB];
#pragma unroll
            for (int t = 0; t < NB; t++) { la[t] = cpgw::gld((const double *)Ml, cur.a[t]); lb[t] = cpgw::gld((const double *)Ml, cur.b[t]); dk[t] = cpgw::gld((const double *)Dil, cur.k[t]); }
            Idx nxt = cur;
            if (s + NB < L) nxt = indices(cur.base, len, s + NB);
#pragma unroll
            for (int t = 0; t < NB; t++)
                if (s + t < rlen) acc = fma(la[t] * dk[t], lb[t], acc);
            cur = nxt;
        }
        acc = cpgw::group_sum_first_dyn(acc, cpgw::read_first_lane(h0.lg));
        if (has) {
            const double v = (kc - kr) - acc;
            if (t0.task >= (unsigned)R.nnzL) cpgw::gst(Dil, t0.task - (unsigned)R.nnzL, 1.0 / v);
            else cpgw::gst(Ml, t0.task, v);
        }
        if (cpgw::read_first_lane(h0.last)) { if (LDS) cpgw::lds_order(); else cpgw::mem_order(); }
        h0 = h1; h1 = h2; t0 = t1; t1 = t2; i0 = i1;
    }
    if (LDS) cpgw::lds_order(); else cpgw::mem_order();
}

#ifdef CPG_GENI_HEADER
CPG_DEV void load_instance_coefficients(const DevRefactor &R, const double *Ml, const double *Dil, double (&cf)[CPG_GENI_NREGS], int lane) {
    const unsigned ln = (unsigned)cpgw::opaque(lane);
#pragma unroll
    for (int t = 0; t < CPG_GENI_NREGS; t++) {
        const unsigned code = cpgw::gld(R.gi_src, (unsigned)t * 64u + ln);
        const unsigned col = (unsigned)cpgw::opaque((int)cpgw::gld(R.gi_lcol, (unsigned)t * 64u + ln));
        const unsigned kind = code >> 28, idx = code & 0x0FFFFFFFu;
        const double a = kind == 3u ? Dil[idx] : Ml[kind == 2u ? idx : 0u], b = Dil[kind == 2u ? col : 0u];
        cf[t] = kind == 2u ? -(a * b) : (kind == 3u ? a : (kind == 1u ? 1.0 : 0.0));
    }
}

#ifdef CPG_GENI_NNZX
#ifndef CPG_SREG_LDS_REGS
#define CPG_SREG_LDS_REGS 20
#endif
struct SharedRegExec {
    static constexpr bool active = true;
    static constexpr int nslots = CPG_GENI_NSLOTS + CPG_GEN_EXTRA_SLOTS;
    static constexpr unsigned ncols = ((CPG_GENI_NSTEPS + 3u) / 4u) * 256u, nrows = ((CPG_GENI_NCHUNKS + 3u) / 4u) * 256u;
    static constexpr int nlds = CPG_SREG_LDS_REGS < CPG_GENI_NREGS ? CPG_SREG_LDS_REGS : CPG_GENI_NREGS;
    static constexpr int nreg = CPG_GENI_NREGS - nlds;
    const double *gcf;
    const unsigned short *gcols, *grows, *lc = nullptr, *lr = nullptr;
    const double *lcf = nullptr;
    double cf[nreg > 0 ? nreg : 1];
    CPG_DEV explicit SharedRegExec(const DevShRegs &t) : gcf(t.cf), gcols(t.cols), grows(t.rows) {}
    CPG_DEV size_t stage(double *lds) {
        unsigned short *c = (unsigned short *)lds, *r = c + ncols;
        double *v = lds + (ncols + nrows) / 4u;
        const unsigned t0 = cpgw::thread_in_block(), nt = cpgw::block_threads();
        for (unsigned t = t0; t < ncols; t += nt) c[t] = cpgw::gld(gcols, t);
        for (unsigned t = t0; t < nrows; t += nt) r[t] = cpgw::gld(grows, t);
        for (unsigned t = t0; t < 64u * (unsigned)nlds; t += nt) v[t] = cpgw::gld(gcf, 64u * (unsigned)nreg + t);
        lc = c; lr = r; lcf = v;
        return (ncols + nrows) / 4u + 64u * (unsigned)nlds;
    }
    CPG_DEV void load(int lane) {
#pragma unroll
        for (int t = 0; t < nreg; t++) cf[t] = cpgw::gld(gcf, (unsigned)t * 64u + (unsigned)lane);
    }
    CPG_DEV void run(double *w, int lane) const {
        double c[CPG_GENI_NREGS];
#pragma unroll
        for (int t = 0; t < CPG_GENI_NREGS; t++) c[t] = t < nreg ? cf[t < nreg ? t : 0] : lcf[(unsigned)(t - nreg) * 64u + (unsigned)lane];
        run_program_inst(c, lc, lr, w, lane);
    }
};
#endif
#endif

CPG_DEV double uniform_double(double v) {
    int w2[2];
    __builtin_memcpy(w2, &v, 8);
    w2[0] = cpgw::read_first_lane(w2[0]); w2[1] = cpgw::read_first_lane(w2[1]);
    __builtin_memcpy(&v, w2, 8);
    return v;
}

template <int NSX, int NSZ, bool GENI = false, bool SHARED = GENI, bool CRLDS = false>
CPG_DEV void osqp_refactor_body(const DevFamily &F0, const DevRefactor &R, const DevSettings &S,
                                const DevBatch &Bt, double *lds, int wave_global) {
    const int lane = cpgw::lane_id();
#if defined(CPG_GENI_HEADER) && defined(CPG_GENI_N)
    const unsigned n = GENI ? (unsigned)CPG_GENI_N : (unsigned)F0.n, m = GENI ? (unsigned)CPG_GENI_M : (unsigned)F0.m, N = n + m;
    const unsigned n_eq = GENI ? (unsigned)CPG_GENI_NEQ : (unsigned)R.n_eq;
#else
    const unsigned n = (unsigned)F0.n, m = (unsigned)F0.m, N = n + m, n_eq = (unsigned)R.n_eq;
#endif
    const unsigned *cr_tab = R.sol_cr;
    if (CRLDS) {
        unsigned *lc = (unsigned *)lds;
        const unsigned ncr = (unsigned)R.sol_nnz;
        for (unsigned t = cpgw::thread_in_block(); t < ncr; t += cpgw::block_threads()) lc[t] = cpgw::gld(R.sol_cr, t);
        cpgw::block_sync();
        cr_tab = lc;
        lds += (ncr + 1u) / 2u;
    }
#ifdef CPG_GENI_HEADER
    const int ldw = GENI ? CPG_GENI_NSLOTS + CPG_GEN_EXTRA_SLOTS : (CPG_GENS_ACTIVE(GENI, SHARED, CRLDS) ? R.sol_slots + CPG_GEN_EXTRA_SLOTS : R.sol_slots);
    constexpr unsigned gi_ncols = ((CPG_GENI_NSTEPS + 3u) / 4u) * 256u, gi_nrows = ((CPG_GENI_NCHUNKS + 3u) / 4u) * 256u;
    const unsigned short *gi_lc = nullptr, *gi_lr = nullptr;
    if (GENI) {
        unsigned short *lc = (unsigned short *)lds, *lr = lc + gi_ncols;
        for (unsigned t = cpgw::thread_in_block(); t < gi_ncols; t += cpgw::block_threads()) lc[t] = cpgw::gld(R.gi_cols, t);
        for (unsigned t = cpgw::thread_in_block(); t < gi_nrows; t += cpgw::block_threads()) lr[t] = cpgw::gld(R.gi_rows, t);
        cpgw::block_sync();
        gi_lc = lc; gi_lr = lr;
        lds += (gi_ncols + gi_nrows) / 4u;
    }
#else
    const int ldw = CPG_GENS_ACTIVE(GENI, SHARED, CRLDS) ? R.sol_slots + CPG_GEN_EXTRA_SLOTS : R.sol_slots;
#endif
    size_t per_wave = (size_t)ldw + (GENI ? (size_t)(N + (N & 1u)) : 0u);
#ifdef CPG_GENI_FAC_NSTEPS
    const size_t fac_doubles = (size_t)CPG_GENI_FAC_ZERO + 1u;
#else
    const size_t fac_doubles = (size_t)R.nnzL + N;
#endif
    if (GENI && per_wave < fac_doubles) per_wave = fac_doubles + (fac_doubles & 1u);
    double *w = lds + (size_t)cpgw::wave_in_block() * per_wave;
    double *qs = w + ldw, *us = qs + n;
    constexpr bool shared = SHARED || GENI;
#ifdef CPG_GENS_HEADER
    constexpr bool GENS = !shared && !CRLDS;
#else
    constexpr bool GENS = false;
#endif
    InstBuf B = carve(Bt.scratch + (size_t)wave_global * (size_t)R.buf_doubles, F0, R);
    const double rho_fr = CPG_RHO_MIN, ri_fr = 1.0 / rho_fr;
    const size_t state_len = (size_t)n + 2u * (size_t)m + 1u;
    unsigned short fpx[NSX], fpz[NSZ];
#pragma unroll
    for (int s = 0; s < NSX; s++) { const unsigned i = (unsigned)lane + 64u * (unsigned)s; fpx[s] = i < n ? cpgw::gld(R.sol_fpos, i) : 0; }
#pragma unroll
    for (int s = 0; s < NSZ; s++) { const unsigned i = (unsigned)lane + 64u * (unsigned)s; fpz[s] = i < m ? cpgw::gld(R.sol_fpos, n + i) : 0; }

    const unsigned n_work = Bt.list_count ? cpgw::sld(Bt.list_count, 0u) : 0u;
    if (shared) {
        B.P = const_cast<double *>(R.Ps); B.A = const_cast<double *>(R.As); B.Ar = const_cast<double *>(R.Ars);
        B.D = const_cast<double *>(R.Ds); B.Dinv = const_cast<double *>(R.Dinvs);
        B.E = const_cast<double *>(R.Es); B.Einv = const_cast<double *>(R.Einvs);
    }

    for (;;) {
        unsigned ig = 0;
        if (lane == 0) ig = cpgw::atomic_next(Bt.counter);
        ig = (unsigned)cpgw::read_first_lane((int)ig);
        long long b = (long long)ig;
        if (Bt.list) {
            if (ig >= n_work) break;
            b = (long long)cpgw::read_first_lane(cpgw::gld(Bt.list, ig));
        } else if (b >= Bt.B) break;
        const double *theta = Bt.theta + (size_t)b * R.np_var;
        const double *state_in = (Bt.state_in && (S.warm_starting || Bt.resume)) ? Bt.state_in + (size_t)b * state_len : nullptr;
        double rho = Bt.state_in ? cpgw::gld(Bt.state_in + (size_t)b * state_len, n + 2u * m) : F0.rho;
        rho = cpgw::dmin2(cpgw::dmax2(rho, CPG_RHO_MIN), CPG_RHO_MAX);
        if (GENI) rho = uniform_double(rho);
        double rho_stg = F0.rho;
        double rho_eq = 1e3 * rho, rho_in = rho, ri_eq = 1.0 / rho_eq, ri_in = 1.0 / rho_in;

        const bool probe = GENI && __builtin_expect(S.debug_stage == 20, 0);
        unsigned long long ts[8];
        int n_ts = 0;
#define CPG_INST_PROBE() do { if (GENI && probe && n_ts < 8) ts[n_ts++] = cpgw::clock100(); } while (0)
        CPG_INST_PROBE();
        if (!shared) {
            for (unsigned k = (unsigned)lane; k < (unsigned)R.nnzA; k += 64u) cpgw::gst(B.A, k, csr_row(R.map_A, k, theta, cpgw::gld(R.A_base, k)));
            for (unsigned k = (unsigned)lane; k < (unsigned)R.nnzP; k += 64u) cpgw::gst(B.P, k, csr_row(R.map_P, k, theta, cpgw::gld(R.P_base, k)));
        }
        for (unsigned i = (unsigned)lane; i < n; i += 64u) cpgw::gst(B.q, i, csr_row(R.map_q, i, theta, cpgw::gld(R.q_base, i)));
        for (unsigned i = (unsigned)lane; i < m; i += 64u) cpgw::gst(B.u, i, csr_row(R.map_u, i, theta, cpgw::gld(R.u_base, i)));
        const double dconst = csr_row(R.map_d, 0, theta, R.d_base);
        cpgw::mem_order();
        double cs = shared ? R.cs : 1.0;
        if (!shared) {
#ifdef CPG_REFACTOR_ROW_COPY
            refresh_row_copy(R, B, lane);
#endif

            for (unsigned i = (unsigned)lane; i < N; i += 64u) w[i] = 1.0;
            cpgw::lds_order();
#pragma nounroll
            for (int it = 0; it < R.scaling_iters; it++) {
                double dn[NSX], en[NSZ];
#pragma unroll
                for (int s = 0; s < NSX; s++) {
                    const unsigned j = (unsigned)lane + 64u * (unsigned)s;
                    double acc = 0.0;
                    if (j < n) {
                        const double dj = w[j];
                        for_row_entries<true>(R.Prp, R.Pent, R.Pcol, (const double *)B.P, j,
                                              [&](double v, unsigned c) { acc = cpgw::dmax2(acc, fabs(cs * dj * v * w[c])); });
                        for_row_entries<false>(R.Ap, nullptr, R.Ai, (const double *)B.A, j,
                                               [&](double v, unsigned c) { acc = cpgw::dmax2(acc, fabs(w[n + c] * v * dj)); });
                    }
                    dn[s] = acc;
                }
#pragma unroll
                for (int s = 0; s < NSZ; s++) {
                    const unsigned i = (unsigned)lane + 64u * (unsigned)s;
                    double acc = 0.0;
                    if (i < m) {
                        const double ei = w[n + i];
#ifdef CPG_REFACTOR_ROW_COPY
                        for_row_entries<false, CPG_ROW_COPY_BATCH>(R.Arp, nullptr, R.Acol, (const double *)B.Ar, i,
#else
                        for_row_entries<true>(R.Arp, R.Aent, R.Acol, (const double *)B.A, i,
#endif
                                              [&](double v, unsigned c) { acc = cpgw::dmax2(acc, fabs(ei * v * w[c])); });
                    }
                    en[s] = acc;
                }
                cpgw::lds_order();
#pragma unroll
                for (int s = 0; s < NSX; s++) { const unsigned j = (unsigned)lane + 64u * (unsigned)s; if (j < n) w[j] = w[j] * (1.0 / sqrt(lim_scaling(dn[s]))); }
#pragma unroll
                for (int s = 0; s < NSZ; s++) { const unsigned i = (unsigned)lane + 64u * (unsigned)s; if (i < m) w[n + i] = w[n + i] * (1.0 / sqrt(lim_scaling(en[s]))); }
                cpgw::lds_order();
                double psum = 0.0, qn = 0.0;
#pragma unroll
                for (int s = 0; s < NSX; s++) {
                    const unsigned j = (unsigned)lane + 64u * (unsigned)s;
                    if (j < n) {
                        const double dj = w[j];
                        double acc = 0.0;
                        for_row_entries<true>(R.Prp, R.Pent, R.Pcol, (const double *)B.P, j,
                                              [&](double v, unsigned c) { acc = cpgw::dmax2(acc, fabs(cs * dj * v * w[c])); });
                        psum += acc;
                        qn = cpgw::dmax2(qn, fabs(cs * dj * cpgw::gld(R.q_setup, j)));
                    }
                }
                psum = cpgw::wave_sum(psum);
                qn = lim_scaling(cpgw::wave_max_nonneg(qn));
                const double cm = n ? psum / (double)n : 0.0;
                cs = cs * (1.0 / lim_scaling(cpgw::dmax2(cm, qn)));
            }
            for (unsigned j = (unsigned)lane; j < n; j += 64u) {
                const double dj = w[j];
                cpgw::gst(B.D, j, dj); cpgw::gst(B.Dinv, j, 1.0 / dj);
                cpgw::gst(B.q, j, cs * dj * cpgw::gld((const double *)B.q, j));
                unsigned a = (unsigned)cpgw::gld(R.Ap, j), e = (unsigned)cpgw::gld(R.Ap, j + 1u);
                for (unsigned k = a; k < e; k++) cpgw::gst(B.A, k, w[n + (unsigned)cpgw::gld(R.Ai, k)] * cpgw::gld((const double *)B.A, k) * dj);
                a = (unsigned)cpgw::gld(R.Pp, j); e = (unsigned)cpgw::gld(R.Pp, j + 1u);
                for (unsigned k = a; k < e; k++) cpgw::gst(B.P, k, cs * w[(unsigned)cpgw::gld(R.Pi, k)] * cpgw::gld((const double *)B.P, k) * dj);
            }
#ifdef CPG_REFACTOR_ROW_COPY
            refresh_row_copy(R, B, lane);
#endif
        }
        if (__builtin_expect(S.debug_stage == 1, 0)) { if (lane == 0) { Bt.status[b] = 11; Bt.iter[b] = 0; } continue; }
        signed char ct[NSZ];
        const int lane_rc = GENI ? cpgw::opaque(lane) : lane;
#pragma unroll
        for (int s = 0; s < NSZ; s++) {
            const unsigned i = (unsigned)lane_rc + 64u * (unsigned)s;
            const unsigned ic = (unsigned)lane + 64u * (unsigned)s;
            ct[s] = 0;
            if (ic < m) {
                double uu = cpgw::gld((const double *)B.u, i);
                if (!shared) {
                    const double ei = w[n + i];
                    uu = ei * uu;
                    cpgw::gst(B.E, i, ei); cpgw::gst(B.Einv, i, 1.0 / ei); cpgw::gst(B.u, i, uu);
                }
                ct[s] = ic < n_eq ? 1 : (uu > CPG_INFTY * CPG_MIN_SCALING ? -1 : 0);
                cpgw::gst(B.rinv, i, ct[s] == 1 ? ri_eq : (ct[s] == 0 ? ri_in : ri_fr));
            }
        }
        cpgw::lds_order();
        cpgw::mem_order();
        double rvv[NSZ], riv[NSZ];
        auto set_steps = [&]() __attribute__((always_inline)) {
#pragma unroll
            for (int s = 0; s < NSZ; s++) {
                rvv[s] = ct[s] == 1 ? rho_eq : (ct[s] == 0 ? rho_in : rho_fr);
                riv[s] = ct[s] == 1 ? ri_eq : (ct[s] == 0 ? ri_in : ri_fr);
            }
        };
        if (GENI) set_steps();

        auto factor_generic = [&]() __attribute__((always_inline)) {
            if (shared) {
                cpgw::mem_order();
                numeric_ldl_m<false>(R, B.Lx, B.Dginv, (const double *)B.rinv, lane);
                substitution_values<true>(R, B, lane);
            } else {
                numeric_ldl(R, B, F0.sigma, lane);
                substitution_values<false, GENS>(R, B, lane);
            }
        };
#ifdef CPG_GENI_HEADER
        double cf[CPG_GENI_NREGS];
        auto factor_in_lds = [&]() __attribute__((always_inline)) {
            cpgw::mem_order();
#ifdef CPG_GENI_FAC_NSTEPS
            if (lane == 0) w[CPG_GENI_FAC_ZERO] = 0.0;
#ifdef CPG_GENI_FAC_ONE
            if (lane == 0) w[CPG_GENI_FAC_ONE] = 1.0;
#endif
            cpgw::lds_order();
            numeric_ldl_gen(R.gf_tri, R.gf_dk, R.gf_kc, (const double *)B.rinv, w, lane);
#else
            numeric_ldl_m<true>(R, w, w + R.nnzL, (const double *)B.rinv, lane);
#endif
            load_instance_coefficients(R, w, w + R.nnzL, cf, lane);
            cpgw::lds_order();
            for (unsigned t = (unsigned)lane; t < (unsigned)ldw; t += 64u) w[t] = 0.0;
            for (unsigned i = (unsigned)lane; i < n; i += 64u) qs[i] = cpgw::gld((const double *)B.q, i);
            for (unsigned i = (unsigned)lane; i < m; i += 64u) us[i] = cpgw::gld((const double *)B.u, i);
            cpgw::lds_order();
        };
        if (__builtin_expect(S.debug_stage == 2, 0)) { if (lane == 0) { Bt.status[b] = 11; Bt.iter[b] = 0; } continue; }
        CPG_INST_PROBE();
        if (GENI) factor_in_lds();
        else
#endif
        factor_generic();
        if (__builtin_expect(S.debug_stage == 3, 0)) { if (lane == 0) { Bt.status[b] = 11; Bt.iter[b] = 0; } continue; }
        CPG_INST_PROBE();

#ifdef CPG_GENS_HEADER
        if (GENS) {
            if (lane == 0) w[CPG_GENS_NSLOTS + CPG_GEN_DUMMY_SLOTS] = 0.0;
            cpgw::lds_order();
        }
#endif
        DevFamily F = F0;
        F.D = B.D; F.Dinv = B.Dinv; F.E = B.E; F.Einv = B.Einv; F.c = cs; F.cinv = 1.0 / cs;
        StreamProg ST;
        ST.stab = R.sol_stab; ST.cr = cr_tab; ST.vals = B.sv;
        ST.n_pairs = R.sol_pairs; ST.dummy = (unsigned)R.sol_nnz / 2u - 1u;
        typedef InstCtx<NSX, NSZ, GENI> CtxT;
        double qr[NSX], ur[NSZ];
#pragma unroll
        for (int s = 0; s < NSX; s++) {
            const unsigned i = (unsigned)lane + 64u * (unsigned)s;
            qr[s] = i < n ? cpgw::gld((const double *)B.q, i) : 0.0;
        }
#pragma unroll
        for (int s = 0; s < NSZ; s++) {
            const unsigned i = (unsigned)lane + 64u * (unsigned)s;
            ur[s] = i < m ? cpgw::gld((const double *)B.u, i) : 0.0;
        }
        const CtxT cx{F, R, B, w, lane, qr, ur, qs, us, shared && F.A_rows.n_chunks > 0};
        double x[NSX], z[NSZ], y[NSZ];
#pragma unroll
        for (int s = 0; s < NSX; s++) x[s] = 0.0;
#pragma unroll
        for (int s = 0; s < NSZ; s++) { z[s] = 0.0; y[s] = 0.0; }
        if (state_in) load_state<NSX, NSZ>(F, state_in, x, z, y, lane);
        CheckOut o;
        o.prim_res = 0; o.dual_res = 0; o.obj = 0; o.status = 11;
        int iter = Bt.resume ? cpgw::read_first_lane(cpgw::gld((const int *)Bt.iter, (unsigned)b)) : 0;
        if (iter > 0) rho_stg = rho;
        double dxr[NSX], dyr[NSZ];
#pragma unroll
        for (int s = 0; s < NSX; s++) dxr[s] = 0.0;
#pragma unroll
        for (int s = 0; s < NSZ; s++) dyr[s] = 0.0;
        auto admm_iteration = [&](const bool chk) __attribute__((always_inline)) {
#pragma unroll
            for (int s = 0; s < NSX; s++) { const unsigned i = (unsigned)lane + 64u * (unsigned)s; if (i < n) w[i] = F.sigma * x[s] - cx.q(s, i); }
#pragma unroll
            for (int s = 0; s < NSZ; s++) {
                const unsigned i = (unsigned)lane + 64u * (unsigned)s;
                const bool ceq = GENI && 64u * (unsigned)(s + 1) <= n_eq;
                const double ri = !GENI ? (ct[s] == 1 ? ri_eq : (ct[s] == 0 ? ri_in : ri_fr)) : (ceq ? ri_eq : riv[s]);
                if (i < m) w[n + i] = z[s] - ri * y[s];
            }
            cpgw::lds_order();
#ifdef CPG_GENI_HEADER
            if (GENI) run_program_inst(cf, gi_lc, gi_lr, w, lane);
            else
#endif
#ifdef CPG_GENS_HEADER
            if (GENS) run_program_gens((const double *)B.sv, R.gs_cols, R.gs_rows, w, lane);
            else
#endif
            run_program_stream(ST, w, lane);
#pragma unroll
            for (int s = 0; s < NSX; s++) {
                const unsigned i = (unsigned)lane + 64u * (unsigned)s;
                if (chk) dxr[s] = 0.0;
                if (i < n) {
                    const double xn = F.alpha * w[GENI ? i : (unsigned)fpx[s]] + (1.0 - F.alpha) * x[s];
                    if (chk) dxr[s] = xn - x[s];
                    x[s] = xn;
                }
            }
#pragma unroll
            for (int s = 0; s < NSZ; s++) {
                const unsigned i = (unsigned)lane + 64u * (unsigned)s;
                if (chk) dyr[s] = 0.0;
                if (i < m) {
                    const bool ceq = GENI && 64u * (unsigned)(s + 1) <= n_eq;
                    const double rv = !GENI ? (ct[s] == 1 ? rho_eq : (ct[s] == 0 ? rho_in : rho_fr)) : (ceq ? rho_eq : rvv[s]);
                    const double ri = !GENI ? (ct[s] == 1 ? ri_eq : (ct[s] == 0 ? ri_in : ri_fr)) : (ceq ? ri_eq : riv[s]);
                    const double zp = z[s], yp = y[s];
                    const double zt = (zp - ri * yp) + ri * w[GENI ? n + i : (unsigned)fpz[s]];
                    const double zr = F.alpha * zt + (1.0 - F.alpha) * zp;
                    const double uu = cx.u(s, i);
                    const double zc = cpgw::dmin2(zr + ri * yp, uu);
                    const double zn = ceq ? uu : (ct[s] == 1 ? uu : zc);
                    const double dyv = rv * (zr - zn);
                    z[s] = zn; y[s] = yp + dyv;
                    if (chk) dyr[s] = dyv;
                }
            }
            cpgw::lds_order();
        };
        const int chk_int = S.check_termination, ad_int = S.adaptive_rho ? S.adaptive_rho_interval : 0;
        CPG_INST_PROBE();
#pragma nounroll
        while (o.status == 11) {
            if (iter < S.max_iter) {
                int next_ev = S.max_iter;
                if (chk_int > 0) { const int c = (iter / chk_int + 1) * chk_int; if (c < next_ev) next_ev = c; }
                if (ad_int > 0) { const int c = (iter / ad_int + 1) * ad_int; if (c < next_ev) next_ev = c; }
#pragma nounroll
                for (; iter < next_ev - 1; iter++) admm_iteration(false);
                iter++;
                admm_iteration(true);
            }
            CPG_INST_PROBE();
            const bool can_check = chk_int > 0 && iter > 0 && iter % chk_int == 0;
            const bool adapt = ad_int > 0 && iter > 0 && iter % ad_int == 0;
            const bool last = iter >= S.max_iter;
            ScaledNorms sn;
            bool have_info = false;
            if (can_check) {
                o = check<NSX, NSZ, CtxT, RegDelta<NSX>, RegDelta<NSZ>>(F, cx, ct, S, x, z, y, RegDelta<NSX>{dxr}, RegDelta<NSZ>{dyr}, InfeasVerdict{false, false}, w, lane, false, &sn);
                have_info = true;
                CPG_INST_PROBE();
                if (o.status != 11) break;
            }
            if (adapt) {
                if (!have_info) (void)check<NSX, NSZ, CtxT, RegDelta<NSX>, RegDelta<NSZ>>(F, cx, ct, S, x, z, y, RegDelta<NSX>{dxr}, RegDelta<NSZ>{dyr}, InfeasVerdict{false, false}, w, lane, false, &sn);
                const double rn = GENI ? uniform_double(rho_estimate(sn, rho_stg)) : rho_estimate(sn, rho_stg);
                if (rn > rho_stg * S.adaptive_rho_tolerance || rn < rho_stg / S.adaptive_rho_tolerance) {
                    rho = rn; rho_stg = rn; rho_eq = 1e3 * rho; rho_in = rho; ri_eq = 1.0 / rho_eq; ri_in = 1.0 / rho_in;
                    if (GENI) set_steps();
#pragma unroll
                    for (int s = 0; s < NSZ; s++) {
                        const unsigned i = (unsigned)lane + 64u * (unsigned)s;
                        if (i < m) cpgw::gst(B.rinv, i, ct[s] == 1 ? ri_eq : (ct[s] == 0 ? ri_in : ri_fr));
                    }
                    cpgw::mem_order();
#ifdef CPG_GENI_HEADER
                    if (GENI) factor_in_lds();
                    else
#endif
                    factor_generic();
                }
            }
            if (last) {
                if (!can_check) o = check<NSX, NSZ, CtxT, RegDelta<NSX>, RegDelta<NSZ>>(F, cx, ct, S, x, z, y, RegDelta<NSX>{dxr}, RegDelta<NSZ>{dyr}, InfeasVerdict{false, false}, w, lane, false);
                if (o.status == 11) o = check<NSX, NSZ, CtxT, RegDelta<NSX>, RegDelta<NSZ>>(F, cx, ct, S, x, z, y, RegDelta<NSX>{dxr}, RegDelta<NSZ>{dyr}, InfeasVerdict{false, false}, w, lane, true);
                if (o.status == 11) o.status = 7;
            }
        }
        finalize<NSX, NSZ, GENI>(F, Bt, x, z, y, dconst, b, w, lane, iter, o, rho);
        if (GENI && probe) {
            CPG_INST_PROBE();
            if (lane == 0) for (int k = 0; k < n_ts && k < F0.n_prim; k++) Bt.prim[(size_t)b * F0.n_prim + k] = (double)(ts[k] - ts[0]);
            if (lane == 0 && n_ts < F0.n_prim) Bt.prim[(size_t)b * F0.n_prim + n_ts] = -1.0;
        }
    }
}

}

namespace cpg {

struct DevGradient {
    const int *Pcolidx, *Acolidx;
    const int *tptr, *tkind, *tidx;
    const double *tcoef;
    int NP;
};
struct DevGradBatch {
    long long B;
    const double *theta, *sol_x, *sol_y, *dx;
    double *dtheta;
    unsigned *counter;
    double *scratch;
};
#define CPG_G_Q 0
#define CPG_G_L 1
#define CPG_G_U 2
#define CPG_G_P 3
#define CPG_G_A 4

template <int NSX, int NSZ>
CPG_DEV void osqp_gradient_body(const DevFamily &F, const DevRefactor &R, const DevGradient &Gd,
                                const DevGradBatch &Bt, double *lds, int wave_global) {
    const int lane = cpgw::lane_id();
    const unsigned n = (unsigned)F.n, m = (unsigned)F.m, N = n + m;
    const int ldw = R.sol_slots;
    const size_t per_wave = (size_t)ldw + N + n + m + n + m;
    double *w = lds + (size_t)cpgw::wave_in_block() * per_wave;
    double *rr = w + ldw, *xs = rr + N, *ys = xs + n, *dxs = ys + m, *act = dxs + n;
    const InstBuf B = carve(Bt.scratch + (size_t)wave_global * (size_t)R.buf_doubles, F, R);
    const double eps = 1e-6;
    StreamProg ST;
    ST.stab = R.sol_stab; ST.cr = R.sol_cr; ST.vals = B.sv;
    ST.n_pairs = R.sol_pairs; ST.dummy = (unsigned)R.sol_nnz / 2u - 1u;

    for (;;) {
        unsigned ig = 0;
        if (lane == 0) ig = cpgw::atomic_next(Bt.counter);
        ig = (unsigned)cpgw::read_first_lane((int)ig);
        if ((long long)ig >= Bt.B) break;
        const size_t b = (size_t)ig;
        const double *theta = Bt.theta + b * (size_t)R.np_var;
        for (unsigned i = (unsigned)lane; i < n; i += 64u) { xs[i] = cpgw::gld(Bt.sol_x + b * n, i); dxs[i] = cpgw::gld(Bt.dx + b * n, i); }
        for (unsigned i = (unsigned)lane; i < m; i += 64u) {
            const double yi = cpgw::gld(Bt.sol_y + b * m, i);
            ys[i] = yi;
            const double a = yi < -1e-12 ? -1.0 : (yi > 1e-12 ? 1.0 : 0.0);
            act[i] = a;
            cpgw::gst(B.rinv, i, a != 0.0 ? eps : 1.0);
        }
        cpgw::lds_order();
        for (unsigned k = (unsigned)lane; k < (unsigned)R.nnzA; k += 64u) {
            const double v = csr_row(R.map_A, k, theta, cpgw::gld(R.A_base, k));
            cpgw::gst(B.A, k, act[(unsigned)cpgw::gld(R.Ai, k)] != 0.0 ? v : 0.0);
        }
        for (unsigned k = (unsigned)lane; k < (unsigned)R.nnzP; k += 64u) cpgw::gst(B.P, k, csr_row(R.map_P, k, theta, cpgw::gld(R.P_base, k)));
        cpgw::lds_order();
        cpgw::mem_order();
        numeric_ldl(R, B, eps, lane);
        substitution_values(R, B, lane);
#pragma nounroll
        for (int sweep = 0; sweep < 4; sweep++) {
            if (sweep == 0) {
                for (unsigned i = (unsigned)lane; i < n; i += 64u) w[i] = dxs[i];
                for (unsigned i = (unsigned)lane; i < m; i += 64u) w[n + i] = 0.0;
            } else {
                for (unsigned j = (unsigned)lane; j < n; j += 64u) {
                    double d = dxs[j];
                    for_row_entries<true>(R.Prp, R.Pent, R.Pcol, (const double *)B.P, j, [&](double v, unsigned c) { d -= v * rr[c]; });
                    for_row_entries<false>(R.Ap, nullptr, R.Ai, (const double *)B.A, j, [&](double v, unsigned c) { d -= v * rr[n + c]; });
                    w[j] = d;
                }
                for (unsigned i = (unsigned)lane; i < m; i += 64u) {
                    double d = 0.0;
                    if (act[i] != 0.0) {
                        for_row_entries<true>(R.Arp, R.Aent, R.Acol, (const double *)B.A, i, [&](double v, unsigned c) { d -= v * rr[c]; });
                    }
                    w[n + i] = d;
                }
            }
            cpgw::lds_order();
            run_program_stream(ST, w, lane);
            for (unsigned i = (unsigned)lane; i < N; i += 64u) {
                const double v = w[(unsigned)cpgw::gld(R.sol_fpos, i)];
                rr[i] = sweep == 0 ? v : rr[i] + v;
            }
            cpgw::lds_order();
        }
        double *out = Bt.dtheta + b * (size_t)Gd.NP;
        for (unsigned c = (unsigned)lane; c < (unsigned)Gd.NP; c += 64u) {
            const unsigned a0 = (unsigned)cpgw::gld(Gd.tptr, c), e0 = (unsigned)cpgw::gld(Gd.tptr, c + 1u);
            double acc = 0.0;
            for (unsigned t = a0; t < e0; t++) {
                const int kind = cpgw::gld(Gd.tkind, t);
                const unsigned idx = (unsigned)cpgw::gld(Gd.tidx, t);
                double d = 0.0;
                if (kind == CPG_G_Q) d = -rr[idx];
                else if (kind == CPG_G_L) d = act[idx] == -1.0 ? rr[n + idx] : 0.0;
                else if (kind == CPG_G_U) d = act[idx] == 1.0 ? rr[n + idx] : 0.0;
                else if (kind == CPG_G_P) {
                    const unsigned i = (unsigned)cpgw::gld(R.Pi, idx), j = (unsigned)cpgw::gld(Gd.Pcolidx, idx);
                    d = -0.5 * (rr[i] * xs[j] + xs[i] * rr[j]);
                } else {
                    const unsigned i = (unsigned)cpgw::gld(R.Ai, idx), j = (unsigned)cpgw::gld(Gd.Acolidx, idx);
                    d = act[i] != 0.0 ? -(rr[n + i] * xs[j] + ys[i] * rr[j]) : 0.0;
                }
                acc = fma(cpgw::gld(Gd.tcoef, t), d, acc);
            }
            cpgw::gst(out, c, acc);
        }
        cpgw::lds_order();
    }
}

}
```

Before: 5.346 million.

## Keep scaling vectors in LDS and drop global rinv/q/u round-trips in refactor

In the shared-register path, the D, Dinv, E and Einv scaling vectors are staged in LDS, and the LDS budget grows to three times n+m to hold them. The instance-mode refactor keeps the updated q and u in registers instead of writing them to global memory and reading them back. The LDL factorisation now computes rho-inverse per row from register ballot masks through a functor instead of loading a global rinv array. The Lcol table is packed into the high bits of the 64-bit source table, which removes one upload and one load stream. It also adds clock-based probe instrumentation and a hand-over path that writes state at permuted positions. The cost is a larger LDS footprint, which can lower occupancy or stop some families from fitting.

```diff
diff --git a/cvxpygen_amd/codegen.py b/cvxpygen_amd/codegen.py
--- a/cvxpygen_amd/codegen.py
+++ b/cvxpygen_amd/codegen.py
@@ -595,7 +595,8 @@
     if preloaded:
         w(f'CPG_DEV void {func}(const unsigned long long *tri, const unsigned *dk, double *w, int lane) {{')
     else:
-        w(f'CPG_DEV void {func}(const unsigned long long *tri, const unsigned *dk, const double *kct, const double *rinv,')
+        w('template <class RhoOfRow>')
+        w(f'CPG_DEV void {func}(const unsigned long long *tri, const unsigned *dk, const double *kct, const RhoOfRow &rinv,')
         w('                             double *w, int lane) {')
     w('    const unsigned ln = (unsigned)cpgw::opaque(lane);     // (table addresses computed here, not hoisted out of the instance loop)')
 
@@ -607,7 +608,7 @@
         if c < nch:
             if not preloaded and c < inv0:
                 w(f'    const double kc{c} = cpgw::gld(kct, {c * 64}u + ln);')
-                w(f'    const double kr{c} = cpgw::gld(rinv, (d{c} >> 16) ? (d{c} >> 16) - 1u : 0u);')
+                w(f'    const double kr{c} = rinv((d{c} >> 16) ? (d{c} >> 16) - 1u : 0u);')
             for s_ in range(int(ct[c, 0])):
                 w(f'    const unsigned long long e{int(first[c]) + s_} = cpgw::gld(tri, {(int(first[c]) + s_) * 64}u + ln);')
     for c in range(2 * P):
@@ -771,7 +772,7 @@
 
 def shared_register_lds_bytes(n: int, m: int, n_steps: int, n_chunks: int, n_slots: int, n_regs: int, waves: int = 8) -> int:
     tab = 2 * (256 * ((n_steps + 3) // 4) + 256 * ((n_chunks + 3) // 4))
-    return 8 * (n + m) + tab + 8 * 64 * min(SHARED_REG_LDS_REGS, n_regs) + waves * 8 * (n_slots + GEN_EXTRA_SLOTS)
+    return 3 * 8 * (n + m) + tab + 8 * 64 * min(SHARED_REG_LDS_REGS, n_regs) + waves * 8 * (n_slots + GEN_EXTRA_SLOTS)
 
 
 def instance_program_fits(rpl) -> bool:
diff --git a/cvxpygen_amd/csrc/cpg_hip.cpp b/cvxpygen_amd/csrc/cpg_hip.cpp
--- a/cvxpygen_amd/csrc/cpg_hip.cpp
+++ b/cvxpygen_amd/csrc/cpg_hip.cpp
@@ -457,7 +457,7 @@
 static int shared_reg_waves(cpg_handle_t h) { return h->waves_per_block > 0 && h->waves_per_block < 8 ? h->waves_per_block : 8; }
 static size_t shared_reg_lds(cpg_handle_t h, int W) {
     const size_t tab = (size_t)(((CPG_GENI_NSTEPS + 3) / 4) * 256 + ((CPG_GENI_NCHUNKS + 3) / 4) * 256) * sizeof(unsigned short);
-    return (size_t)(h->F.n + h->F.m) * sizeof(double) + tab + (size_t)cpg::SharedRegExec::nlds * 64 * sizeof(double) +
+    return (size_t)3 * (size_t)(h->F.n + h->F.m) * sizeof(double) + tab + (size_t)cpg::SharedRegExec::nlds * 64 * sizeof(double) +
            (size_t)W * (CPG_GENI_NSLOTS + CPG_GEN_EXTRA_SLOTS) * sizeof(double);
 }
 static bool shared_reg_usable(cpg_handle_t h) {
@@ -1473,9 +1473,9 @@
     const size_t n = h->F.n, m = h->F.m, N = n + m;
     int rc = CPG_OK;
     R.gi_ok = 0;
-    std::vector<unsigned short> gcols, grows, glcol;
-    std::vector<unsigned> gsrc, gdk;
-    std::vector<unsigned long long> gtri;
+    std::vector<unsigned short> gcols, grows;
+    std::vector<unsigned> gdk;
+    std::vector<unsigned long long> gtri, gsrc;
     std::vector<double> gkc;
 #ifdef CPG_GENI_N
     const bool geni_dims = h->F.n == CPG_GENI_N && h->F.m == CPG_GENI_M && h->F.n_eq == CPG_GENI_NEQ;
@@ -1504,8 +1504,7 @@
     }
     if (ok) ok = generated_tables(g.sol_ctab, g.sol_desc, g.sol_cols, g.sol_chunks, g.sol_nnz, g.sol_slots, steps, CPG_GENI_NSTEPS, gcols, grows, chunk_shift);
     if (ok) {
-        gsrc.assign((size_t)CPG_GENI_NREGS * 64, 0u);
-        glcol.assign((size_t)CPG_GENI_NREGS * 64, (unsigned short)0);
+        gsrc.assign((size_t)CPG_GENI_NREGS * 64, 0ull);
         std::vector<char> taken((size_t)CPG_GENI_NREGS * 64, 0);
         for (int t = 0; ok && t < CPG_GENI_NSTEPS; t++) {
             const int e = steps[t][0], cnt = steps[t][1], reg = steps[t][2], sh = steps[t][3];
@@ -1523,7 +1522,7 @@
                 gsrc[at] = ((unsigned)kind << 28) | (unsigned)idx;
                 if (kind == 2) {
                     if (idx >= r->nnzL || r->Lcol[idx] < 0 || r->Lcol[idx] > 0xFFFF) { ok = false; break; }
-                    glcol[at] = (unsigned short)r->Lcol[idx];
+                    gsrc[at] |= (unsigned long long)r->Lcol[idx] << 32;
                 }
             }
         }
@@ -1591,10 +1590,9 @@
     ok = ok && !nx;
 #endif
     if (ok) {
-        if ((rc = upload<unsigned short>(h, own, glcol.data(), glcol.size(), &R.gi_lcol))) return rc;
         if ((rc = upload<unsigned short>(h, own, gcols.data(), gcols.size(), &R.gi_cols))) return rc;
         if ((rc = upload<unsigned short>(h, own, grows.data(), grows.size(), &R.gi_rows))) return rc;
-        if ((rc = upload<unsigned>(h, own, gsrc.data(), gsrc.size(), &R.gi_src))) return rc;
+        if ((rc = upload<unsigned long long>(h, own, gsrc.data(), gsrc.size(), &R.gi_src))) return rc;
     }
     if ((rc = rt_sync(h))) return rc;
     R.gi_ok = ok ? 1 : 0;
@@ -1688,7 +1686,7 @@
         if ((rc = upload<double>(h, own, einv.data(), m, &R.Einvs))) return rc;
     }
     R.gf_tri = nullptr; R.gf_dk = nullptr; R.gf_kc = nullptr;
-    R.gi_ok = 0; R.gi_cols = R.gi_rows = nullptr; R.gi_src = nullptr; R.gi_lcol = nullptr; R.fac_kc = nullptr; R.fac_krow = nullptr; R.fac_kc_cl = nullptr; R.fac_krow_cl = nullptr; R.fac_kind_cl = nullptr; R.fac_idx_cl = nullptr;
+    R.gi_ok = 0; R.gi_cols = R.gi_rows = nullptr; R.gi_src = nullptr; R.fac_kc = nullptr; R.fac_krow = nullptr; R.fac_kc_cl = nullptr; R.fac_krow_cl = nullptr; R.fac_kind_cl = nullptr; R.fac_idx_cl = nullptr;
     std::vector<double> fkc, fkc_cl;
     std::vector<int> fkrow, fkrow_cl;
 
diff --git a/cvxpygen_amd/csrc/cpg_osqp_kernel.h b/cvxpygen_amd/csrc/cpg_osqp_kernel.h
--- a/cvxpygen_amd/csrc/cpg_osqp_kernel.h
+++ b/cvxpygen_amd/csrc/cpg_osqp_kernel.h
@@ -437,7 +437,7 @@
     return v;
 }
 
-template <int NSX, int NSZ, int NV>
+template <int NSX, int NSZ, int NV, bool SCL = false>
 struct SharedCtx {
     static constexpr bool kTestsFirst = true;
     static constexpr bool kOpaqueLane = true;
@@ -446,6 +446,7 @@
     const Inst<NSX, NSZ, NV> &I;
     const double *w;
     int lane;
+    const double *sc = nullptr;
     CPG_DEV double q(int s, unsigned i) const {
         return s < Inst<NSX, NSZ, NV>::NVX ? I.qv[s < Inst<NSX, NSZ, NV>::NVX ? s : 0] : sh[i];
     }
@@ -454,10 +455,10 @@
     }
     CPG_DEV void products(int) const {}
     CPG_DEV void stage(int) const {}
-    CPG_DEV double sE(unsigned i) const { return cpgw::gld(F.E, i); }
-    CPG_DEV double sEinv(unsigned i) const { return cpgw::gld(F.Einv, i); }
-    CPG_DEV double sD(unsigned i) const { return cpgw::gld(F.D, i); }
-    CPG_DEV double sDinv(unsigned i) const { return cpgw::gld(F.Dinv, i); }
+    CPG_DEV double sE(unsigned i) const { return SCL ? sc[2u * (unsigned)F.n + i] : cpgw::gld(F.E, i); }
+    CPG_DEV double sEinv(unsigned i) const { return SCL ? sc[2u * (unsigned)F.n + (unsigned)F.m + i] : cpgw::gld(F.Einv, i); }
+    CPG_DEV double sD(unsigned i) const { return SCL ? sc[i] : cpgw::gld(F.D, i); }
+    CPG_DEV double sDinv(unsigned i) const { return SCL ? sc[(unsigned)F.n + i] : cpgw::gld(F.Dinv, i); }
     CPG_DEV double ax(int s) const { return CPG_NATURAL_ROWS(F.A_rows, 0, s, w, lane); }
     CPG_DEV double px(int s) const { return CPG_NATURAL_ROWS(F.P_rows, 1, s, w, lane); }
     CPG_DEV double atx(int s) const { return CPG_NATURAL_ROWS(F.At_rows, 2, s, w, lane); }
@@ -734,6 +735,23 @@
     if (lane == 0) so[F.n + 2 * F.m] = rho;
 }
 
+template <int NSX, int NSZ>
+CPG_DEV void store_state_at(const DevFamily &F, double *so, const double (&Ix)[NSX], const double (&Iz)[NSZ],
+                            const double (&Iy)[NSZ], const unsigned short (&px)[NSX], const unsigned short (&pz)[NSZ],
+                            double rho, int lane) {
+#pragma unroll
+    for (int s = 0; s < NSX; s++) {
+        const unsigned i = (unsigned)lane + 64u * (unsigned)s;
+        if (i < (unsigned)F.n) cpgw::gst(so, (unsigned)px[s], Ix[s]);
+    }
+#pragma unroll
+    for (int s = 0; s < NSZ; s++) {
+        const unsigned i = (unsigned)lane + 64u * (unsigned)s;
+        if (i < (unsigned)F.m) { cpgw::gst(so, (unsigned)pz[s], Iz[s]); cpgw::gst(so, (unsigned)F.m + (unsigned)pz[s], Iy[s]); }
+    }
+    if (lane == 0) so[F.n + 2 * F.m] = rho;
+}
+
 CPG_DEV double rho_estimate(const ScaledNorms &sn, double rho_settings) {
     const double pr = sn.prim_res / (cpgw::dmax2(sn.nz, sn.nax) + CPG_DIV_TOL);
     const double dr = sn.dual_res / (cpgw::dmax2(sn.nq, cpgw::dmax2(sn.naty, sn.npx)) + CPG_DIV_TOL);
@@ -784,20 +802,30 @@
 }
 
 #define CPG_STATUS_HANDED_OVER (-3)
-template <int NSX, int NSZ>
-CPG_DEV void hand_over(const DevFamily &F, const DevBatch &Bt, const double (&Ix)[NSX], const double (&Iz)[NSZ],
-                       const double (&Iy)[NSZ], long long b, int lane_in, int iter, double rho_new) {
+template <int NSX, int NSZ, bool POS>
+CPG_DEV void hand_over_impl(const DevFamily &F, const DevBatch &Bt, const double (&Ix)[NSX], const double (&Iz)[NSZ],
+                       const double (&Iy)[NSZ], long long b, int lane_in, int iter, double rho_new,
+                       const unsigned short (&px)[NSX], const unsigned short (&pz)[NSZ]) {
     const int lane = cpgw::opaque(lane_in);
     cpgw::assume((unsigned)lane < 64u);
     if (!Bt.ho_state || !Bt.ho_list) {
         if (lane == 0) { Bt.obj[b] = NAN; Bt.iter[b] = iter; Bt.status[b] = -2; Bt.pri_res[b] = 0.0; Bt.dua_res[b] = 0.0; }
         return;
     }
-    store_state<NSX, NSZ>(F, Bt.ho_state + (size_t)b * (size_t)(F.n + 2 * F.m + 1), Ix, Iz, Iy, true, rho_new, lane);
+    double *so = Bt.ho_state + (size_t)b * (size_t)(F.n + 2 * F.m + 1);
+    if (POS) store_state_at<NSX, NSZ>(F, so, Ix, Iz, Iy, px, pz, rho_new, lane);
+    else store_state<NSX, NSZ>(F, so, Ix, Iz, Iy, true, rho_new, lane);
     if (lane == 0) {
         Bt.iter[b] = iter; Bt.status[b] = CPG_STATUS_HANDED_OVER;
         Bt.ho_list[cpgw::atomic_next(Bt.ho_count)] = (int)b;
     }
+}
+
+template <int NSX, int NSZ>
+CPG_DEV void hand_over(const DevFamily &F, const DevBatch &Bt, const double (&Ix)[NSX], const double (&Iz)[NSZ],
+                       const double (&Iy)[NSZ], long long b, int lane_in, int iter, double rho_new) {
+    const unsigned short px[NSX] = {}, pz[NSZ] = {};
+    hand_over_impl<NSX, NSZ, false>(F, Bt, Ix, Iz, Iy, b, lane_in, iter, rho_new, px, pz);
 }
 
 #if defined(CPG_GEN_N)
@@ -839,8 +867,16 @@
     for (unsigned t = cpgw::thread_in_block(); t < (unsigned)N; t += cpgw::block_threads())
         sh[t] = t < (unsigned)F.n ? cpgw::gld(U.q_base, t) : cpgw::gld(U.u_base, t - (unsigned)F.n);
     const double *shu = sh + n_c;
+    typedef SharedCtx<NSX, NSZ, NV, REG::active> CtxS;
+    double *sc = lds + N;
+    if (REG::active) {
+        for (unsigned t = cpgw::thread_in_block(); t < (unsigned)F.n; t += cpgw::block_threads()) { sc[t] = cpgw::gld(F.D, t); sc[(unsigned)F.n + t] = cpgw::gld(F.Dinv, t); }
+        for (unsigned t = cpgw::thread_in_block(); t < (unsigned)F.m; t += cpgw::block_threads()) {
+            sc[2u * (unsigned)F.n + t] = cpgw::gld(F.E, t); sc[2u * (unsigned)F.n + (unsigned)F.m + t] = cpgw::gld(F.Einv, t);
+        }
+    }
     LdsProg LP;
-    size_t lds_off = (size_t)N;
+    size_t lds_off = (size_t)N + (REG::active ? 2u * (size_t)N : 0u);
     if (LDSPROG) {
         const DevRagged &R = F.kkt_ragged;
 #ifdef CPG_GEN_HEADER
@@ -919,6 +955,14 @@
         ig = (unsigned)cpgw::read_first_lane((int)ig);
         if ((long long)ig >= ngroups) break;
 
+        const bool probe = REG::active && __builtin_expect(S.debug_stage == 20, 0);
+        unsigned long long pr_last = 0;
+        int pr_k = 0;
+        double *pr_out = nullptr;
+#define CPG_SHARED_PROBE() do { if (REG::active && probe) { const unsigned long long t_ = cpgw::clock100();                \
+            if (lane == 0 && pr_out) pr_out[pr_k] = (double)(t_ - pr_last) + (pr_k == 5 ? pr_out[5] : 0.0);                \
+            pr_last = t_; if (pr_k < 5) pr_k++; } } while (0)
+        if (REG::active && probe) pr_last = cpgw::clock100();
         InstT I[G];
         CheckOut co[G];
         int n_open = 0;
@@ -939,7 +983,7 @@
             if (Bt.state_in && b < Bt.B && !bad) {
                 const double rho_in = cpgw::gld(Bt.state_in + (size_t)b * (size_t)(F.n + 2 * F.m + 1), (unsigned)(F.n + 2 * F.m));
                 if (__builtin_expect(cpgw::dmin2(cpgw::dmax2(rho_in, CPG_RHO_MIN), CPG_RHO_MAX) != F.rho, 0)) {
-                    hand_over<NSX, NSZ>(F, Bt, I[g].x, I[g].z, I[g].y, b, lane, 0, rho_in);
+                    hand_over_impl<NSX, NSZ, REG::active>(F, Bt, I[g].x, I[g].z, I[g].y, b, lane, 0, rho_in, fpx, fpz);
                     I[g].done = 1;
                 }
             }
@@ -949,6 +993,11 @@
             }
             n_open += I[g].done ? 0 : 1;
         }
+        if (REG::active && probe) {
+            if (I[0].b >= 0 && F.n_prim >= 16) pr_out = Bt.prim + (size_t)I[0].b * F.n_prim + 9;
+            if (lane == 0 && pr_out) for (int k = 0; k < 7; k++) pr_out[k] = 0.0;
+            CPG_SHARED_PROBE();
+        }
 
         int iter = 0;
         auto rhs_and_solve = [&]() __attribute__((always_inline)) {
@@ -964,7 +1013,7 @@
 #pragma unroll
                 for (int s = 0; s < NSX; s++) {
                     const unsigned i = (unsigned)lane + 64u * (unsigned)s;
-                    if (i < n_c) wg[REG::active ? (unsigned)fpx[s] : i] = F.sigma * I[g].x[s] - SharedCtx<NSX, NSZ, NV>{F, sh, shu, I[g], wg, lane}.q(s, i);
+                    if (i < n_c) wg[REG::active ? (unsigned)fpx[s] : i] = F.sigma * I[g].x[s] - CtxS{F, sh, shu, I[g], wg, lane, sc}.q(s, i);
                     CPG_FENCE_EVERY(s);
                 }
 #pragma unroll
@@ -1020,7 +1069,7 @@
                         const double zp = I[g].z[s], yp = I[g].y[s];
                         const double zt = (zp - ri * yp) + ri * wg[fpz[s]];
                         const double zr = F.alpha * zt + (1.0 - F.alpha) * zp;
-                        const double uu = SharedCtx<NSX, NSZ, NV>{F, sh, shu, I[g], wg, lane}.u(s, i);
+                        const double uu = CtxS{F, sh, shu, I[g], wg, lane, sc}.u(s, i);
                         const double zn = cts == 1 ? uu : cpgw::dmin2(zr + ri * yp, uu);
                         const double dyv = rv * (zr - zn);
                         I[g].z[s] = zn; I[g].y[s] = yp + dyv;
@@ -1057,6 +1106,7 @@
                     for (int s = 0; s < NSZ; s++) dyr[g][s] = 0.0;
                 }
             }
+            CPG_SHARED_PROBE();
             const bool last = iter >= S.max_iter;
             const bool can_check = last || (chk_int > 0 && iter % chk_int == 0);
             const bool adapt = ad_int > 0 && iter > 0 && iter % ad_int == 0;
@@ -1068,8 +1118,8 @@
                 double *wg = w + g * ldw;
 #pragma nounroll
                 for (int pass = 0; pass < (last ? 2 : 1); pass++) {
-                    const InfeasVerdict v = infeasibility_tests<NSX, NSZ, SharedCtx<NSX, NSZ, NV>, RegDelta<NSX>, RegDelta<NSZ>>(
-                        F, SharedCtx<NSX, NSZ, NV>{F, sh, shu, I[g], wg, lane}, ct_reg, S,
+                    const InfeasVerdict v = infeasibility_tests<NSX, NSZ, CtxS, RegDelta<NSX>, RegDelta<NSZ>>(
+                        F, CtxS{F, sh, shu, I[g], wg, lane, sc}, ct_reg, S,
                         RegDelta<NSX>{dxr[g]}, RegDelta<NSZ>{dyr[g]}, wg, lane, pass == 1);
                     if (pass == 0) iv_exact[g] = v; else iv_approx[g] = v;
                 }
@@ -1086,8 +1136,8 @@
 #pragma nounroll
                 for (int pass = 0; pass < 2; pass++) {
                     if (pass == 1 && !(o.status == 11 && last)) break;
-                    const CheckOut oc = check<NSX, NSZ, SharedCtx<NSX, NSZ, NV>, NoDelta, NoDelta>(
-                        F, SharedCtx<NSX, NSZ, NV>{F, sh, shu, I[g], wg, lane}, ct_reg, S, I[g].x, I[g].z, I[g].y,
+                    const CheckOut oc = check<NSX, NSZ, CtxS, NoDelta, NoDelta>(
+                        F, CtxS{F, sh, shu, I[g], wg, lane, sc}, ct_reg, S, I[g].x, I[g].z, I[g].y,
                         NoDelta{}, NoDelta{}, pass == 0 ? iv_exact[g] : iv_approx[g], wg, lane, pass == 1,
                         (pass == 0 && adapt) ? &sn : nullptr);
                     if (can_check) o = oc;
@@ -1098,16 +1148,24 @@
                 }
                 if (o.status == 11 && last) o.status = 7;
                 co[g] = o;
+                CPG_SHARED_PROBE();
+                double pr_keep[6];
+                if (REG::active && probe && lane == 0 && pr_out && o.status != 11) for (int k = 0; k < 6; k++) pr_keep[k] = pr_out[k];
                 if (o.status != 11) {
                     finalize<NSX, NSZ>(F, Bt, I[g].x, I[g].z, I[g].y, I[g].dconst, I[g].b, wg, lane, iter, o, rho_ws);
                     I[g].done = 1; n_open--;
                 } else if (rho_changed) {
-                    hand_over<NSX, NSZ>(F, Bt, I[g].x, I[g].z, I[g].y, I[g].b, lane, iter, rho_ws);
+                    hand_over_impl<NSX, NSZ, REG::active>(F, Bt, I[g].x, I[g].z, I[g].y, I[g].b, lane, iter, rho_ws, fpx, fpz);
                     I[g].done = 1; n_open--;
                 }
+                if (REG::active && probe && I[g].done && lane == 0 && pr_out) {
+                    if (o.status != 11) for (int k = 0; k < 6; k++) pr_out[k] = pr_keep[k];
+                    pr_out[6] = (double)(cpgw::clock100() - pr_last);
+                }
             }
         }
-    }
-}
-
-}
+#undef CPG_SHARED_PROBE
+    }
+}
+
+}
diff --git a/cvxpygen_amd/csrc/cpg_osqp_refactor.h b/cvxpygen_amd/csrc/cpg_osqp_refactor.h
--- a/cvxpygen_amd/csrc/cpg_osqp_refactor.h
+++ b/cvxpygen_amd/csrc/cpg_osqp_refactor.h
@@ -54,8 +54,7 @@
     double cs;
     int gi_ok;
     const unsigned short *gi_cols, *gi_rows;
-    const unsigned *gi_src;
-    const unsigned short *gi_lcol;
+    const unsigned long long *gi_src;
     const unsigned long long *gf_tri;
     const unsigned *gf_dk;
     const double *gf_kc;
@@ -352,8 +351,8 @@
     const unsigned ln = (unsigned)cpgw::opaque(lane);
 #pragma unroll
     for (int t = 0; t < CPG_GENI_NREGS; t++) {
-        const unsigned code = cpgw::gld(R.gi_src, (unsigned)t * 64u + ln);
-        const unsigned col = (unsigned)cpgw::opaque((int)cpgw::gld(R.gi_lcol, (unsigned)t * 64u + ln));
+        const unsigned long long sw = cpgw::gld(R.gi_src, (unsigned)t * 64u + ln);
+        const unsigned code = (unsigned)sw, col = (unsigned)(sw >> 32);
         const unsigned kind = code >> 28, idx = code & 0x0FFFFFFFu;
         const double a = kind == 3u ? Dil[idx] : Ml[kind == 2u ? idx : 0u], b = Dil[kind == 2u ? col : 0u];
         cf[t] = kind == 2u ? -(a * b) : (kind == 3u ? a : (kind == 1u ? 1.0 : 0.0));
@@ -407,6 +406,22 @@
     return v;
 }
 
+#if defined(CPG_GENI_HEADER) && defined(CPG_GENI_N)
+template <int NSZ>
+struct RhoRows {
+    static constexpr int S0 = CPG_GENI_NEQ / 64;
+    double ri_eq, ri_in, ri_fr;
+    unsigned long long fr[NSZ];
+    CPG_DEV double operator()(unsigned r) const {
+        unsigned long long mk = fr[S0 < NSZ ? S0 : 0];
+#pragma unroll
+        for (int s = S0 + 1; s < NSZ; s++) mk = (r >> 6) == (unsigned)s ? fr[s] : mk;
+        const bool is_fr = ((mk >> (r & 63u)) & 1ull) != 0ull;
+        return r < (unsigned)CPG_GENI_NEQ ? ri_eq : (is_fr ? ri_fr : ri_in);
+    }
+};
+#endif
+
 template <int NSX, int NSZ, bool GENI = false, bool SHARED = GENI, bool CRLDS = false>
 CPG_DEV void osqp_refactor_body(const DevFamily &F0, const DevRefactor &R, const DevSettings &S,
                                 const DevBatch &Bt, double *lds, int wave_global) {
@@ -498,10 +513,18 @@
             for (unsigned k = (unsigned)lane; k < (unsigned)R.nnzA; k += 64u) cpgw::gst(B.A, k, csr_row(R.map_A, k, theta, cpgw::gld(R.A_base, k)));
             for (unsigned k = (unsigned)lane; k < (unsigned)R.nnzP; k += 64u) cpgw::gst(B.P, k, csr_row(R.map_P, k, theta, cpgw::gld(R.P_base, k)));
         }
-        for (unsigned i = (unsigned)lane; i < n; i += 64u) cpgw::gst(B.q, i, csr_row(R.map_q, i, theta, cpgw::gld(R.q_base, i)));
-        for (unsigned i = (unsigned)lane; i < m; i += 64u) cpgw::gst(B.u, i, csr_row(R.map_u, i, theta, cpgw::gld(R.u_base, i)));
+        double qk[NSX], uk[NSZ];
+        if (GENI) {
+#pragma unroll
+            for (int s = 0; s < NSX; s++) { const unsigned i = (unsigned)lane + 64u * (unsigned)s; qk[s] = i < n ? csr_row(R.map_q, i, theta, cpgw::gld(R.q_base, i)) : 0.0; }
+#pragma unroll
+            for (int s = 0; s < NSZ; s++) { const unsigned i = (unsigned)lane + 64u * (unsigned)s; uk[s] = i < m ? csr_row(R.map_u, i, theta, cpgw::gld(R.u_base, i)) : 0.0; }
+        } else {
+            for (unsigned i = (unsigned)lane; i < n; i += 64u) cpgw::gst(B.q, i, csr_row(R.map_q, i, theta, cpgw::gld(R.q_base, i)));
+            for (unsigned i = (unsigned)lane; i < m; i += 64u) cpgw::gst(B.u, i, csr_row(R.map_u, i, theta, cpgw::gld(R.u_base, i)));
+        }
         const double dconst = csr_row(R.map_d, 0, theta, R.d_base);
-        cpgw::mem_order();
+        if (!GENI) cpgw::mem_order();
         double cs = shared ? R.cs : 1.0;
         if (!shared) {
 #ifdef CPG_REFACTOR_ROW_COPY
@@ -587,18 +610,18 @@
             const unsigned ic = (unsigned)lane + 64u * (unsigned)s;
             ct[s] = 0;
             if (ic < m) {
-                double uu = cpgw::gld((const double *)B.u, i);
+                double uu = GENI ? uk[s] : cpgw::gld((const double *)B.u, i);
                 if (!shared) {
                     const double ei = w[n + i];
                     uu = ei * uu;
                     cpgw::gst(B.E, i, ei); cpgw::gst(B.Einv, i, 1.0 / ei); cpgw::gst(B.u, i, uu);
                 }
                 ct[s] = ic < n_eq ? 1 : (uu > CPG_INFTY * CPG_MIN_SCALING ? -1 : 0);
-                cpgw::gst(B.rinv, i, ct[s] == 1 ? ri_eq : (ct[s] == 0 ? ri_in : ri_fr));
+                if (!GENI) cpgw::gst(B.rinv, i, ct[s] == 1 ? ri_eq : (ct[s] == 0 ? ri_in : ri_fr));
             }
         }
         cpgw::lds_order();
-        cpgw::mem_order();
+        if (!GENI) cpgw::mem_order();
         double rvv[NSZ], riv[NSZ];
         auto set_steps = [&]() __attribute__((always_inline)) {
 #pragma unroll
@@ -621,23 +644,42 @@
         };
 #ifdef CPG_GENI_HEADER
         double cf[CPG_GENI_NREGS];
+        auto store_rinv = [&]() __attribute__((always_inline)) {
+#pragma unroll
+            for (int s = 0; s < NSZ; s++) {
+                const unsigned i = (unsigned)lane + 64u * (unsigned)s;
+                if (i < m) cpgw::gst(B.rinv, i, ct[s] == 1 ? ri_eq : (ct[s] == 0 ? ri_in : ri_fr));
+            }
+            cpgw::mem_order();
+        };
         auto factor_in_lds = [&]() __attribute__((always_inline)) {
-            cpgw::mem_order();
 #ifdef CPG_GENI_FAC_NSTEPS
             if (lane == 0) w[CPG_GENI_FAC_ZERO] = 0.0;
 #ifdef CPG_GENI_FAC_ONE
             if (lane == 0) w[CPG_GENI_FAC_ONE] = 1.0;
 #endif
             cpgw::lds_order();
-            numeric_ldl_gen(R.gf_tri, R.gf_dk, R.gf_kc, (const double *)B.rinv, w, lane);
+#ifdef CPG_GENI_N
+            RhoRows<NSZ> rr;
+            rr.ri_eq = ri_eq; rr.ri_in = ri_in; rr.ri_fr = ri_fr;
+#pragma unroll
+            for (int s = 0; s < NSZ; s++) rr.fr[s] = cpgw::ballot(ct[s] == -1);
+            numeric_ldl_gen(R.gf_tri, R.gf_dk, R.gf_kc, rr, w, lane);
 #else
+            store_rinv();
+            numeric_ldl_gen(R.gf_tri, R.gf_dk, R.gf_kc, [&](unsigned r) { return cpgw::gld((const double *)B.rinv, r); }, w, lane);
+#endif
+#else
+            store_rinv();
             numeric_ldl_m<true>(R, w, w + R.nnzL, (const double *)B.rinv, lane);
 #endif
             load_instance_coefficients(R, w, w + R.nnzL, cf, lane);
             cpgw::lds_order();
             for (unsigned t = (unsigned)lane; t < (unsigned)ldw; t += 64u) w[t] = 0.0;
-            for (unsigned i = (unsigned)lane; i < n; i += 64u) qs[i] = cpgw::gld((const double *)B.q, i);
-            for (unsigned i = (unsigned)lane; i < m; i += 64u) us[i] = cpgw::gld((const double *)B.u, i);
+#pragma unroll
+            for (int s = 0; s < NSX; s++) { const unsigned i = (unsigned)lane + 64u * (unsigned)s; if (i < n) qs[i] = qk[s]; }
+#pragma unroll
+            for (int s = 0; s < NSZ; s++) { const unsigned i = (unsigned)lane + 64u * (unsigned)s; if (i < m) us[i] = uk[s]; }
             cpgw::lds_order();
         };
         if (__builtin_expect(S.debug_stage == 2, 0)) { if (lane == 0) { Bt.status[b] = 11; Bt.iter[b] = 0; } continue; }
@@ -665,12 +707,12 @@
 #pragma unroll
         for (int s = 0; s < NSX; s++) {
             const unsigned i = (unsigned)lane + 64u * (unsigned)s;
-            qr[s] = i < n ? cpgw::gld((const double *)B.q, i) : 0.0;
+            qr[s] = (!GENI && i < n) ? cpgw::gld((const double *)B.q, i) : 0.0;
         }
 #pragma unroll
         for (int s = 0; s < NSZ; s++) {
             const unsigned i = (unsigned)lane + 64u * (unsigned)s;
-            ur[s] = i < m ? cpgw::gld((const double *)B.u, i) : 0.0;
+            ur[s] = (!GENI && i < m) ? cpgw::gld((const double *)B.u, i) : 0.0;
         }
         const CtxT cx{F, R, B, w, lane, qr, ur, qs, us, shared && F.A_rows.n_chunks > 0};
         double x[NSX], z[NSZ], y[NSZ];
@@ -770,15 +812,23 @@
                 if (rn > rho_stg * S.adaptive_rho_tolerance || rn < rho_stg / S.adaptive_rho_tolerance) {
                     rho = rn; rho_stg = rn; rho_eq = 1e3 * rho; rho_in = rho; ri_eq = 1.0 / rho_eq; ri_in = 1.0 / rho_in;
                     if (GENI) set_steps();
-#pragma unroll
-                    for (int s = 0; s < NSZ; s++) {
-                        const unsigned i = (unsigned)lane + 64u * (unsigned)s;
-                        if (i < m) cpgw::gst(B.rinv, i, ct[s] == 1 ? ri_eq : (ct[s] == 0 ? ri_in : ri_fr));
+                    if (!GENI) {
+#pragma unroll
+                        for (int s = 0; s < NSZ; s++) {
+                            const unsigned i = (unsigned)lane + 64u * (unsigned)s;
+                            if (i < m) cpgw::gst(B.rinv, i, ct[s] == 1 ? ri_eq : (ct[s] == 0 ? ri_in : ri_fr));
+                        }
+                        cpgw::mem_order();
                     }
-                    cpgw::mem_order();
 #ifdef CPG_GENI_HEADER
-                    if (GENI) factor_in_lds();
-                    else
+                    if (GENI) {
+#pragma unroll
+                        for (int s = 0; s < NSX; s++) { const unsigned i = (unsigned)lane + 64u * (unsigned)s; qk[s] = i < n ? qs[i] : 0.0; }
+#pragma unroll
+                        for (int s = 0; s < NSZ; s++) { const unsigned i = (unsigned)lane + 64u * (unsigned)s; uk[s] = i < m ? us[i] : 0.0; }
+                        cpgw::lds_order();
+                        factor_in_lds();
+                    } else
 #endif
                     factor_generic();
                 }
@@ -789,8 +839,12 @@
                 if (o.status == 11) o.status = 7;
             }
         }
+        double sh_ts[7];
+        if (GENI && probe && Bt.resume && F0.n_prim >= 16)
+            for (int k = 0; k < 7; k++) sh_ts[k] = Bt.prim[(size_t)b * F0.n_prim + 9 + k];
         finalize<NSX, NSZ, GENI>(F, Bt, x, z, y, dconst, b, w, lane, iter, o, rho);
         if (GENI && probe) {
+            if (lane == 0 && Bt.resume && F0.n_prim >= 16) for (int k = 0; k < 7; k++) Bt.prim[(size_t)b * F0.n_prim + 9 + k] = sh_ts[k];
             CPG_INST_PROBE();
             if (lane == 0) for (int k = 0; k < n_ts && k < F0.n_prim; k++) Bt.prim[(size_t)b * F0.n_prim + k] = (double)(ts[k] - ts[0]);
             if (lane == 0 && n_ts < F0.n_prim) Bt.prim[(size_t)b * F0.n_prim + n_ts] = -1.0;
```

Result: slower. 5.141 million (-3.8%).
